# zju3dv/NeuralRecon-W

Hardware: AMD Instinct MI355X
Metric: ray-samples/sec (train step) at 1024 rays x 128 samples (higher is better)
Workload: dtype f16; 1 GPU; brandenburg_gate config (BASELINE.json configs[1]): 1024 rays/GPU x (64 coarse + 64 fine) samples, SDF 8x256 + colour 4x256 + bg NeRF 8x256, 4 outside samples, up_sample_steps 2, render+loss+backward+allreduce+clip+Adam; rays_per_gpu=1024, samples_per_ray=128, global_rays=1024, parallelism=dp1, world_size=1, submission=eager, streams=2, skipped_steps=0

## Files before the change

include/neuconw_hip.h:

```cpp
#ifndef NEUCONW_HIP_H
#define NEUCONW_HIP_H
#include <stdint.h>

#ifdef __cplusplus
extern "C" {
#endif

#define NCW_PREC_F32 0
#define NCW_PREC_BF16 1
#define NCW_PREC_F16 2
#define NCW_MAX_LAYERS 12
#define NCW_MAX_SEGS 4

#define NCW_E_BADARG (-1)
#define NCW_E_UNSUPPORTED (-2)

int ncw_abi_version(void);
const char* ncw_source_hash(void);
int ncw_device_info(char* buf, int buflen);

typedef struct NcwSeg {
    int32_t col0;
    int32_t ncols;
    int32_t dcol0;
// ... 23 lines not shown
                     void* stream);

typedef struct NcwUnpackDesc {
    const float* dw;
    const float* db;
    const float* src;
    const float* g;
    float* d_src;
    float* d_g;
    float* d_bias;
    int32_t ld, ldw;
    int32_t row0, nrows, drow0;
    float scale;
    float grad_mul;
    int32_t accumulate;
    int32_t nseg;
    NcwSeg seg[NCW_MAX_SEGS];
    const float* grad_mul_dev;
} NcwUnpackDesc;
int ncw_unpack_grads(const NcwUnpackDesc* descs, const int32_t* row_prefix, int n, int total_rows,
                     void* stream);

typedef struct NcwSdfNet {
    const void* w[NCW_MAX_LAYERS];
    const float* b[NCW_MAX_LAYERS];
    const void* wt[NCW_MAX_LAYERS];
    const void* w_feat;
    const float* b_feat;
    const void* wt_feat;
    int32_t n_layers;
    int32_t skip_layer;
    int32_t rb;
    int32_t multires;
    float scale;
    int32_t adj_mode;
    const void* w_lo[NCW_MAX_LAYERS];
    const void* wt_lo[NCW_MAX_LAYERS];
} NcwSdfNet;

int ncw_sdf_infer(const NcwSdfNet* net, int prec, const float* x, int64_t n, float* sdf, void* stream);

int ncw_sdf_infer_rays(const NcwSdfNet* net, int prec, const float* rays_o, const float* rays_d, const float* z,
                       int R, int n, float* sdf, void* stream);

typedef struct NcwPoints {
    const float* x;
    const float* rays_o;
    const float* rays_d;
    const float* z;
    const float* sample_dist;
    int32_t per_ray;
    int32_t mode;
    float gmin[3], gmax[3], gorigin[3], gradius;
    int32_t gdim;
    int32_t _gpad;
    int64_t gstart;
    const int32_t* idx;
    const int32_t* count;
} NcwPoints;

int ncw_sdf_infer_points(const NcwSdfNet* net, int prec, const NcwPoints* pts, int64_t count, float* sdf, void* stream);


typedef struct NcwSdfStash {
    void* gamma;
    void* h[NCW_MAX_LAYERS];
    void* s[NCW_MAX_LAYERS];
    void* t[NCW_MAX_LAYERS];
    void* feat;
    void* dfeat;
    void* qbar[NCW_MAX_LAYERS];
    void* zbar[NCW_MAX_LAYERS];
    void* zsdf;
    void* one;
} NcwSdfStash;

int ncw_sdf_fwd(const NcwSdfNet* net, int prec, const NcwPoints* pts, int64_t n, float* sdf, float* grad,
                const NcwSdfStash* stash, void* stream);
int ncw_sdf_bwd(const NcwSdfNet* net, int prec, const NcwPoints* pts, int64_t n, const float* d_sdf,
                const float* d_grad, const NcwSdfStash* stash, void* stream);

typedef struct NcwColorNet {
    const void* w_f; const void* wt_f; const float* b_f;
    const void* w_e[4]; const void* wt_e[4]; const float* b_e[4];
    const void* w_l[8]; const void* wt_l[8]; const float* b_l[8];
    int32_t n_head;
    int32_t n_lin;
    int32_t rbf, rbh, rbc, n_a;
    const void* w_f_lo; const void* w_e_lo[4]; const void* w_l_lo[8];
    int32_t act_split;
    int32_t _pad;
} NcwColorNet;

typedef struct NcwColorStash {
    void* aux1;
    void* aux2;
    void* f;
    void* e[4];
    void* x[8];
    void* zf;
    void* ze[4];
    void* zx[8];
    void* zo;
    const float* aux_bias;
} NcwColorStash;

int ncw_color_fwd(const NcwColorNet* net, int prec, const NcwPoints* pts, int64_t n, const float* normals,
                  const float* a, const void* feat_stash, float* rgb, const NcwColorStash* stash, void* stream);
int ncw_color_bwd(const NcwColorNet* net, int prec, const NcwPoints* pts, int64_t n, const float* rgb,
                  const float* d_rgb, float* d_grad, float* d_a, float* d_a_rows, void* dfeat_stash,
                  const NcwColorStash* stash, void* stream);

typedef struct NcwNerfNet {
    const void* w_p[8]; const void* wt_p[8]; const float* b_p[8];
    const void* w_alpha; const void* wt_alpha; const float* b_alpha;
    const void* w_feat; const void* wt_feat; const float* b_feat;
    const void* w_a[4]; const void* wt_a[4]; const float* b_a[4];
    const void* w_rgb; const void* wt_rgb; const float* b_rgb;
    int32_t D;
    int32_t skip;
    int32_t rbn, rbh, n_head, n_a;
    const void* w_p_lo[8]; const void* w_alpha_lo; const void* w_feat_lo; const void* w_a_lo[4]; const void* w_rgb_lo;
} NcwNerfNet;

typedef struct NcwNerfStash {
    void* gp;
    void* aux1;
    void* h[9];
    void* featn;
    void* e[4];
    void* zp[8];
    void* zalpha;
    void* zfeat;
    void* ze[4];
    void* zrgb;
    const float* aux_bias;
} NcwNerfStash;

int ncw_nerf_fwd(const NcwNerfNet* net, int prec, const NcwPoints* pts, const float* x4, int64_t n, const float* a,
                 float* density, float* rgb, const NcwNerfStash* stash, void* stream);
int ncw_nerf_bwd(const NcwNerfNet* net, int prec, const NcwPoints* pts, int64_t n, const float* d_density,
                 const float* d_rgb, float* d_a, float* d_a_rows, const NcwNerfStash* stash, void* stream);
int ncw_nerf_refine(const NcwNerfNet* net, int prec, const NcwPoints* pts, int64_t n, const float* aux_bias, float* density,
                    float* rgb, void* stream);
int ncw_batch_assemble(const float* all_rays, int ncols, const float* all_rgbs, const int64_t* idx, int64_t n_rows,
                       int64_t B, int with_semantics, float* rays, int64_t* ts, int64_t* label, float* rgbs,
                       const int* mask_ids, int n_ids, uint8_t* keep, void* stream);
int ncw_aux_ray_bias(const float* w, int ldw, int col0, int n_out, const float* rays_d, const float* a, int n_a, int64_t R,
                     float* out, int ldo, void* stream);
int ncw_ray_prologue(const float* rays, int ncols, int64_t R, const float* origin_host, float radius, float* rays_o,
                     float* rays_d, float* near, float* far, float* depth_gt, float* depth_weight, void* stream);
int ncw_inv_s_fwd(const float* variance, float* inv_s, float* s_val, void* stream);
int ncw_inv_s_bwd(const float* d_inv_s_rays, int64_t R, const float* inv_s, float* d_variance, void* stream);
int ncw_loss_fwd(const float* color, const float* rgbs, int64_t R, const float* gradient_error, const float* mask_error,
                 int64_t n_mask, const float* sfm, int64_t n_sfm, float coef, float igr_w, float mask_w, float depth_w,
                 float* loss, void* stream);
int ncw_loss_bwd(const float* d_loss, const float* color, const float* rgbs, int64_t R, int64_t n_mask, int64_t n_sfm,
                 float coef, float igr_w, float mask_w, float depth_w, float* d_color, float* d_gradient_error,
                 float* d_mask_error, float* d_sfm, void* stream);
int ncw_scatter_add_rows(const float* rows, const int64_t* idx, int64_t R, int n_cols, int64_t n_out, float* out,
                         void* stream);
int ncw_ray_sum_rows(const float* rows, int64_t R, int per_ray, int n_cols, float* out, int accumulate, void* stream);

typedef struct NcwWgradDesc {
    const void* x;
    const void* y;
    float* dense;
    float* dbias;
    int32_t rbx, rby, ld;
    int32_t ksplit;
    int64_t n_points;
    const int32_t* n_points_dev;
} NcwWgradDesc;
int ncw_wgrad(const NcwWgradDesc* descs, const int32_t* wg_prefix, int n_desc, int total_wgs, int ksplit,
              int prec, int64_t n_points, void* stream);
int64_t ncw_wgrad_ordered_scratch_floats(int total_wgs);
int ncw_wgrad_ordered(const NcwWgradDesc* descs, const int32_t* wg_prefix, int n_desc, int total_wgs, int ksplit,
                      int prec, int64_t n_points, float* partials, void* stream);
int ncw_wgrad_tiled(const NcwWgradDesc* descs, const int32_t* wg_prefix, int n_desc, int total_wgs, int ksplit,
                    int tile, int64_t n_points, void* stream);
int ncw_wgrad_tiled_f16(const NcwWgradDesc* descs, const int32_t* wg_prefix, int n_desc, int total_wgs, int ksplit,
                        int tile, int64_t n_points, void* stream);

int ncw_adam_step(float* param, float* grad, float* exp_avg, float* exp_avg_sq, int64_t n, float step_size,
                  float beta1, float beta2, float eps, float bias_correction2_sqrt, const float* total_norm,
                  float max_norm, void* stream);

int64_t ncw_grad_norm_scratch_floats(void);
int ncw_grad_norm(const float* grad, int64_t n, float* scratch, float* norm, void* stream);

typedef struct NcwAdamState {
    int32_t step;
    int32_t good;
    int32_t skipped;
    int32_t skip_now;
    float coef, step_size, bc2_sqrt, last_norm;
} NcwAdamState;
int ncw_adam_step_dev(float* param, float* grad, float* exp_avg, float* exp_avg_sq, int64_t n, NcwAdamState* state,
                      const float* total_norm, float lr, const float* lr_dev, float beta1, float beta2, float eps,
                      float max_norm, float* loss_scale, int growth_interval, float scale_min, float scale_max,
                      void* stream);

int ncw_stash_from_rows(int prec, const float* rows, int64_t n, int F, int rb, void* stash, void* stream);
int ncw_stash_to_rows(int prec, const void* stash, int64_t n, int F, int rb, float* rows, void* stream);

int ncw_sample_coarse(const float* near, const float* far, const float* s_near, const float* s_far, int R,
                      int n_samples, int n_outside, const float* rand_shift, const float* rand_out,
                      float* z, float* z_out, float* sample_dist, void* stream);
int ncw_upsample(const float* rays_o, const float* rays_d, const float* z, const float* sdf, int R, int n,
                 float inv_s, int n_new, float* z_new, void* stream);
int ncw_sort_merge(const float* a, int na, const float* b, int nb, const float* pa, const float* pb, int R,
                   float* out, float* pout, void* stream);
int ncw_boundary(const float* near, const float* far, const float* z, int n, int R, int nb, float* zb,
                 void* stream);

int ncw_voxel_build(const float* pts_normalised, int64_t n, int level, uint32_t* occ, uint32_t* brick, void* stream);
int ncw_ray_voxel_near_far(const float* rays_o_sfm, const float* rays_d, int R, const float* scene_origin_host,
                           float scale, int level, const uint32_t* occ, const uint32_t* brick, float* near_sfm,
                           float* far_sfm, void* stream);
int ncw_ray_voxel_trace(const float* rays_o_norm, const float* rays_d, int R, int level, const uint32_t* occ,
                        const uint32_t* brick, const int32_t* offsets, int32_t* counts, int32_t* nug_ray,
                        int32_t* nug_voxel, float* nug_depth, void* stream);

typedef struct NcwCompositeIn {
    const float* rays_o;
    const float* rays_d;
    const float* z;
    const float* z_feed;
    const float* sample_dist;
    const float* sdf;
    const float* grad;
    const float* rgb;
    const float* density;
    const float* bg_rgb;
    const float* inv_s;
    const float* background_rgb;
    const float* cos_anneal_dev;
    float cos_anneal;
    int32_t R, S, O, has_bg, trim_sphere;
} NcwCompositeIn;

typedef struct NcwCompositeOut {
    float* color;
    float* color_sphere;
    float* color_bg;
    float* weights;
    float* weights_sum;
    float* cdf;
    float* inside;
    float* depth;
    float* normals;
    float* eik;
    float* mid_z;
    float* dists;
    float* bg_alpha;
    float* weights_max;
} NcwCompositeOut;

typedef struct NcwCompositeGrad {
    const float* d_color;
    const float* d_weights_sum;
    const float* d_depth;
    const float* d_eik_num;
    float* d_sdf;
    float* d_grad;
    float* d_rgb;
    float* d_density;
    float* d_bg_rgb;
    float* d_inv_s;
    float grad_scale;
    const float* grad_scale_dev;
    const float* d_normals;
} NcwCompositeGrad;

int ncw_bg_select(const float* rays_o, const float* rays_d, const float* z, const float* sample_dist, int R, int S,
                  int O, int32_t* idx, int32_t* ray_offsets, int32_t* count, void* stream);

int ncw_composite_fwd(const NcwCompositeIn* in, const NcwCompositeOut* out, void* stream);
int ncw_composite_bwd(const NcwCompositeIn* in, const NcwCompositeGrad* g, void* stream);

int ncw_ray_tail_fwd(const float* weights_sum, const int64_t* label, const int* mask_ids, int n_ids,
                     const float* depth, const float* depth_gt, const float* depth_weight, const float* eik_num,
                     const float* eik_den, int R, float* mask_error, float* sfm_depth_loss, float* scalars,
                     void* stream);
int ncw_ray_tail_bwd(const float* weights_sum, const int64_t* label, const int* mask_ids, int n_ids,
                     const float* depth, const float* depth_gt, const float* depth_weight, int R,
                     const float* scalars, const float* d_mask_error, const float* d_sfm_depth_loss,
                     const float* d_gradient_error, float* d_weights_sum, float* d_depth, float* d_eik_num,
                     void* stream);

int ncw_ray_floor_fwd(const float* normals, const int64_t* label, const int* floor_ids, int n_ids, const float n_gt[3],
                      const float* rays_o, const float* rays_d, const float* depth, int R, int scaled,
                      float* floor_error , float* scalars , void* stream);
int ncw_ray_floor_bwd(const float* normals, const int64_t* label, const int* floor_ids, int n_ids, const float n_gt[3],
                      int R, int scaled, const float* scalars, const float* d_floor_error ,
                      float* d_normals , void* stream);

int ncw_mc_count(const float* sdf, const uint8_t* mask, int Dx, int Dy, int Dz, float level, const int32_t* ntri,
                 int32_t* counts, void* stream);
int ncw_mc_emit(const float* sdf, const uint8_t* mask, int Dx, int Dy, int Dz, float level, const int8_t* tri,
                const int32_t* ntri, const int32_t* edges, const int64_t* offsets, float* tri_pos, int64_t* tri_key,
                void* stream);

int ncw_mcs_neighbors(const int32_t* bricks, int64_t n, int G, int32_t* nbr, void* stream);
int ncw_mcs_count(const float* values, int64_t n_values, const int32_t* bricks, const int32_t* nbr, int64_t n, int up, int G,
                  float level, const int32_t* ntri, uint8_t* counts, void* stream);
int ncw_mcs_cube_ids(const int32_t* bricks, int64_t n, int up, int G, const int64_t* sub, int64_t M, int64_t* ids, void* stream);
int ncw_mcs_emit(const float* values, int64_t n_values, const int32_t* bricks, const int32_t* nbr, int64_t n, int up, int G,
                 float level, const int8_t* tri, const int32_t* ntri, const int32_t* edges, const int64_t* sub,
                 const int64_t* offsets, int64_t M, int64_t T, float* tri_pos, int64_t* tri_key, void* stream);


typedef struct NcwNnGrid {
    float lo[3];
    float h, inv_h;
    int32_t dim[3];
} NcwNnGrid;

int ncw_nn_cell_keys(const float* pts, int64_t n, const NcwNnGrid* grid, int32_t* keys, void* stream);
int ncw_nn_cell_ranges(const float* pts, const int32_t* sorted_keys, const int64_t* order, int64_t m, int32_t* cell_range,
                       float* pts_sorted, void* stream);
int ncw_nn_query(const float* pts_sorted, const int32_t* cell_range, const float* q, const int64_t* q_order, int64_t n,
                 const NcwNnGrid* grid, int max_shell, float margin, float* dist, int64_t* idx, int32_t* escaped,
                 int32_t* n_escaped, void* stream);
int ncw_nn_brute(const float* pts_sorted, int64_t m, const float* q, const int32_t* escaped, int64_t n_esc, uint64_t* scratch,
                 float* dist, int64_t* idx, void* stream);
int ncw_nn_coarse(const int32_t* cell_range, const NcwNnGrid* grid, int B, int32_t* coarse, void* stream);
int ncw_nn_query_within(const float* pts_sorted, const int32_t* cell_range, const int32_t* coarse, int B, const float* q,
                        const int64_t* q_order, int64_t n, const NcwNnGrid* grid, float margin, float max_dist, float* dist,
                        int64_t* idx, void* stream);


int ncw_knn_query(const float* pts_sorted, const int32_t* cell_range, const int32_t* coarse, int B, const float* q,
                  const int64_t* q_order, const int32_t* exclude, int64_t n, const NcwNnGrid* grid, float margin, float max_dist,
                  int k, int wg, int32_t* idx, float* dist, int32_t* count, int32_t* work, void* stream);
int ncw_knn_pca(const float* pts, const float* ref, int64_t m, const int32_t* idx, const int32_t* count, int64_t n, int k,
                int with_query, const float* toward, float* normal, double* eig, float* curvature, uint8_t* valid, void* stream);


typedef struct NcwRasterView {
    float view[12];
    float fx, fy, cx, cy;
    float znear, zfar;
    int32_t height, width;
    int32_t cull;
    int32_t small_max;
} NcwRasterView;

int ncw_raster_small(const float* verts, int64_t n_verts, const int32_t* faces, int64_t n_faces, const NcwRasterView* view,
                     uint64_t* zbuf, int32_t* large, int32_t* n_large, void* stream);
int ncw_raster_large(const float* verts, int64_t n_verts, const int32_t* faces, const NcwRasterView* view, const int32_t* large,
                     const int32_t* n_large, int64_t max_large, uint64_t* zbuf, void* stream);
int ncw_raster_resolve(const uint64_t* zbuf, int64_t n_pix, float* depth, int32_t* face, void* stream);
int ncw_raster_backproject(const float* depth, const int64_t* pix, int64_t n, int32_t width, const float* M, float* pts,
                           void* stream);
int ncw_raster_mark(const float* dist, const int64_t* idx, int64_t n, float thr, int64_t m, uint8_t* flags, void* stream);


typedef struct NcwViewCamera {
    float fx, fy, cx, cy;
    float c2w[12];
    int32_t width, height;
    float near, far;
} NcwViewCamera;

// ... 200 lines not shown
```

neuralrecon-w_amd/appfit.py:

```python
import ctypes as C
import json
import os

import numpy as np
import torch

from . import lib as L
from . import rayops
from .neuconw import points_struct
from .packing import pack_many
from .stash import StashArena, StashCache

DEFAULT_STEPS = 200
DEFAULT_LR = 0.02
DEFAULT_N_RAYS = 8192


def half_pixel_indices(width, height):
    width, height = int(width), int(height)
    idx = np.arange(width * height, dtype=np.int64).reshape(height, width)
    return idx[:, : width // 2].reshape(-1), idx[:, width // 2:].reshape(-1)


def ray_subset(width, height, n_rays, seed=0):
    left, _ = half_pixel_indices(width, height)
    if n_rays is None or int(n_rays) >= left.size:
        return left
    pick = np.random.default_rng(int(seed)).choice(left.size, int(n_rays), replace=False)
    return left[np.sort(pick)]


def held_out_rows(root_dir):
    from . import colmap

    _, rows = colmap.split_rows(root_dir)
    return [r["filename"] for r in rows if r.get("split") == "test"]


class FrozenRays:

    def release(self):
        StashCache.release(self.__dict__.pop("sdf_lease", None))

    def __del__(self):
        try:
            self.release()
        except Exception:
            pass


def _use_bg(rdr):
    return bool(rdr.render_bg and rdr.n_outside > 0)


def _bg_choice(rdr, z, n_out):
    select = refine = None
    if rdr.trim_sphere:
        refine = (z, n_out)
        if not rdr.bg_dense:
            select = refine
    return select, refine


@torch.no_grad()
def freeze_rays(rdr, rays, background_rgb=None, chunk=1024, cos_anneal_ratio=0.0, far_override=None):
    if not (torch.is_tensor(rays) and rays.is_cuda):
        raise L.NeuconwHipError("appfit.freeze_rays: rays are not on a GPU; the hot path has no CPU fallback")
    dev, prec, lib = rays.device, rdr.prec, L.get_lib()
    neuconw, nerf = rdr.neuconw, rdr.nerf
    if rdr.origin.device != dev:
        rdr.origin = rdr.origin.to(dev).float()
        rdr.sfm_to_gt = rdr.sfm_to_gt.to(dev).float()
    use_bg = _use_bg(rdr)
    if rdr.__dict__.get("sampler_prec") is None:
        pack_many([(m, m.plan(prec)) for m in [neuconw.sdf_net, neuconw.color_net] + ([nerf] if use_bg else [])])
    origin = (C.c_float * 3)(*[float(v) for v in rdr.origin.reshape(-1).tolist()])
    n_a = int(neuconw.color_net.n_a)
    bgc = None
    if background_rgb is not None:
        if background_rgb.numel() != 3:
            raise ValueError("background_rgb must hold ONE colour (3 values): got shape %s" % (tuple(background_rgb.shape),))
        bgc = background_rgb.detach().to(dev).reshape(3).float().contiguous()
    variance = neuconw.deviation_network.variance
    inv_s, s_val = torch.empty(1, device=dev), torch.empty(1, device=dev)
    L.check(lib.ncw_inv_s_fwd(L.ptr(variance.detach().reshape(1).float().contiguous()), L.ptr(inv_s), L.ptr(s_val),
                              L.stream_ptr(dev)), "ncw_inv_s_fwd")
    rays = rays.contiguous().float()
    out = []
    for r0 in range(0, rays.shape[0], max(1, int(chunk))):
        rc = rays[r0:r0 + max(1, int(chunk))].contiguous()
        R = rc.shape[0]
        rays_o, rays_d = torch.empty(R, 3, device=dev), torch.empty(R, 3, device=dev)
        near, far = torch.empty(R, 1, device=dev), torch.empty(R, 1, device=dev)
        dgt, dw = torch.empty(R, device=dev), torch.empty(R, device=dev)
        L.check(lib.ncw_ray_prologue(L.ptr(rc), rc.shape[1], R, origin, float(rdr.radius), L.ptr(rays_o), L.ptr(rays_d),
                                     L.ptr(near), L.ptr(far), L.ptr(dgt), L.ptr(dw), L.stream_ptr(dev)), "ncw_ray_prologue")
        _, z, z_out, sample_dist = rdr.sparse_sampler(rays_o, rays_d, near, far, 0, None, far_override)
        S = z.shape[1]
        g = FrozenRays()
        g.R, g.S, g.use_bg, g.background_rgb = R, S, bool(use_bg and z_out is not None), bgc
        a0 = torch.zeros(R, n_a, device=dev)
        z_feed = density = bg_rgb = None
        g.O = 0
        if g.use_bg:
            g.O = z_out.shape[1]
            g.select, g.refine = _bg_choice(rdr, z, g.O)
            z_feed, _ = rayops.sort_merge(z, z_out)
            g.pts_bg = points_struct(rays_o=rays_o, rays_d=rays_d, z=z_feed, sample_dist=sample_dist, mode=2)
            density, bg_rgb, nctx = nerf.fwd_stash(g.pts_bg, R * (S + g.O), prec, a0, select=g.select, train=False, refine=g.refine)
            StashCache.release(nctx["lease"])
            density, bg_rgb = density.view(R, S + g.O), bg_rgb.view(R, S + g.O, 3)
        g.M = S + g.O
        g.pts_in = points_struct(rays_o=rays_o, rays_d=rays_d, z=z, sample_dist=sample_dist, mode=2)
        sdf, grad, sctx = neuconw.sdf_net.fwd_stash(g.pts_in, R * S, prec, train=False)
        g.sdf_lease, g.sdf_arena = sctx["lease"], sctx["arena"]
        g.feat_ptr = sctx["arena"].ptr(sctx["ids"]["feat"])
        g.grad = grad
        comp = rayops.CompositeCtx(rays_o, rays_d, z, sample_dist, sdf.view(R, S), grad.view(R, S, 3),
                                   torch.zeros(R, S, 3, device=dev), inv_s, cos_anneal_ratio, z_feed, density, bg_rgb, bgc,
                                   rdr.trim_sphere)
        o = comp.forward()
        g.weights, g.inside, g.weights_sum, g.z_feed, g.z = o["weights"], o["inside"], o["weights_sum"], z_feed, z
        out.append(g)
    return out


def release_contexts(contexts):
    for g in contexts:
        g.release()


def dead_sample_share(contexts):
    dead = sum(int((g.weights == 0).sum()) for g in contexts)
    return dead / float(max(1, sum(g.weights.numel() for g in contexts)))


class AppearanceFit:

    def __init__(self, rdr, contexts, targets, init, lr=DEFAULT_LR, betas=(0.9, 0.999), eps=1e-7):
        if not contexts:
            raise ValueError("AppearanceFit: no frozen rays")
        if not (torch.is_tensor(targets) and targets.is_cuda and torch.is_tensor(init) and init.is_cuda):
            raise L.NeuconwHipError("AppearanceFit: targets / init are not on a GPU; the hot path has no CPU fallback")
        self.rdr, self.ctxs = rdr, list(contexts)
        dev = targets.device
        self.dev, self.prec = dev, rdr.prec
        self.n_a = n_a = int(rdr.neuconw.color_net.n_a)
        self.R_total = sum(g.R for g in self.ctxs)
        self.targets = targets.detach().reshape(-1, 3).float().contiguous()
        if self.targets.shape[0] != self.R_total:
            raise ValueError("AppearanceFit: %d targets for %d frozen rays" % (self.targets.shape[0], self.R_total))
        if init.numel() != n_a:
            raise ValueError("AppearanceFit: the code holds %d values, the networks take %d" % (init.numel(), n_a))
        self.lr, self.betas, self.eps = float(lr), (float(betas[0]), float(betas[1])), float(eps)
        self.inv_denom = 1.0 / (self.R_total + 1e-5)
        self.code = init.detach().reshape(n_a).float().clone().contiguous()
        self.exp_avg, self.exp_avg_sq = torch.zeros(n_a, device=dev), torch.zeros(n_a, device=dev)
        self.grad_acc = torch.zeros(n_a, device=dev)
        self.state = torch.zeros(8, device=dev, dtype=torch.int32)
        self.scale = None
        if self.prec == L.PREC_F16:
            s0 = float(rdr.loss_scale.init)
            self.scale = torch.tensor([s0, 1.0 / s0], device=dev, dtype=torch.float32)
        Rm = max(g.R for g in self.ctxs)
        nS, nM = max(g.R * g.S for g in self.ctxs), max(g.R * g.M for g in self.ctxs)
        any_bg = any(g.use_bg for g in self.ctxs)
        self.a_rows = self.code.reshape(1, n_a).expand(Rm, n_a).contiguous()
        self.color = torch.empty(self.R_total, 3, device=dev)
        self.ray_loss = torch.zeros(self.R_total, device=dev)
        self.d_rgb, self.rows = torch.empty(nS, 3, device=dev), torch.empty(nS, n_a, device=dev)
        self.d_grad = torch.zeros(nS, 3, device=dev)
        rbf = int(rdr.neuconw.color_net.d_feature) // 32
        self.dfeat = StashArena(dev, self.prec, nS)
        self.dfeat.new(rbf)
        self.dfeat.allocate()
        if any_bg:
            self.d_bg_rgb, self.rows_bg = torch.empty(nM, 3, device=dev), torch.empty(nM, n_a, device=dev)
            self.d_density = torch.zeros(nM, device=dev)
        lib = L.get_lib()
        self.scratch = torch.empty(max(1, int(lib.ncw_appfit_step_scratch_floats(max(nS, nM), n_a))), device=dev)

    def _step_call(self, rows, n, accumulate, final):
        dev = self.dev
        L.check(L.get_lib().ncw_appfit_step(L.ptr(rows), int(n), self.n_a, L.ptr(self.scratch), L.ptr(self.grad_acc),
                                            int(accumulate), int(final), L.ptr(self.code), L.ptr(self.exp_avg),
                                            L.ptr(self.exp_avg_sq), L.ptr(self.state), self.lr, self.betas[0], self.betas[1],
                                            self.eps, L.ptr(self.scale), 1.0, L.ptr(self.a_rows), self.a_rows.shape[0],
                                            L.stream_ptr(dev)), "ncw_appfit_step")

    def _pass(self, backward):
        rdr, prec, lib, dev, n_a = self.rdr, self.prec, L.get_lib(), self.dev, self.n_a
        color_net, nerf = rdr.neuconw.color_net, rdr.nerf
        r0, first = 0, True
        for g in self.ctxs:
            R, S, M = g.R, g.S, g.M
            a = self.a_rows[:R]
            leases = []
            try:
                rgb, cctx = color_net.fwd_stash(g.pts_in, R * S, prec, g.grad, a, g.feat_ptr, train=backward)
                leases.append(cctx["lease"])
                bg_rgb = nctx = None
                if g.use_bg:
                    _, bg_rgb, nctx = nerf.fwd_stash(g.pts_bg, R * M, prec, a, select=g.select, train=backward, refine=g.refine)
                    leases.append(nctx["lease"])
                d_bg = self.d_bg_rgb[:R * M] if g.use_bg else None
                L.check(lib.ncw_appfit_loss(L.ptr(g.weights), L.ptr(g.inside), L.ptr(g.weights_sum), L.ptr(rgb), L.ptr(bg_rgb),
                                            L.ptr(g.background_rgb), L.ptr(self.targets[r0:r0 + R]), R, S, g.O, self.inv_denom,
                                            L.ptr(self.scale), L.ptr(self.color[r0:r0 + R]), L.ptr(self.ray_loss[r0:r0 + R]),
                                            L.ptr(self.d_rgb[:R * S]), L.ptr(d_bg), L.stream_ptr(dev)), "ncw_appfit_loss")
                if backward:
                    rows = self.rows[:R * S]
                    color_net.bwd_stash(cctx, self.d_rgb[:R * S], self.d_grad[:R * S], None, self.dfeat.ptr(0), d_a_rows=rows)
                    self._step_call(rows, R * S, not first, False)
                    first = False
                    if g.use_bg:
                        rows_bg = self.rows_bg[:R * M]
                        if nctx.get("sel_count") is not None:
                            rows_bg.zero_()
                        nerf.bwd_stash(nctx, self.d_density[:R * M], d_bg, None, d_a_rows=rows_bg)
                        self._step_call(rows_bg, R * M, True, False)
            finally:
                for l in leases:
                    StashCache.release(l)
            r0 += R
        return self.ray_loss.sum() * self.inv_denom

    def loss_and_grad(self):
        with torch.no_grad():
            return self._pass(True)

    def loss(self):
        with torch.no_grad():
            return self._pass(False)

    def step(self):
        self._step_call(None, 0, True, True)

    @property
    def grad(self):
        return self.grad_acc * self.scale[1] if self.scale is not None else self.grad_acc.clone()

    def colors(self):
        return self.color

    @property
    def skipped_steps(self):
        return int(self.state[2])

    @property
    def applied_steps(self):
        return int(self.state[0])


def _planar(gt, H, W, dev):
    g = gt.to(dev).float()
    if g.dim() == 2:
        g = g.reshape(H, W, 3).permute(2, 0, 1)
    return g.reshape(3, H, W).contiguous()


# ... 115 lines not shown
```

neuralrecon-w_amd/csrc/ncw_glue.hip:

```cpp
#include "../../include/neuconw_hip.h"
#include "ncw_common.h"

namespace {

__global__ __launch_bounds__(256) void ray_prologue_kernel(const float* __restrict__ rays, int ncols, int64_t R, float ox, float oy,
                                                           float oz, float radius, float* __restrict__ rays_o,
                                                           float* __restrict__ rays_d, float* __restrict__ near,
                                                           float* __restrict__ far, float* __restrict__ depth_gt,
                                                           float* __restrict__ depth_w) {
    const int64_t r = (int64_t)blockIdx.x * 256 + threadIdx.x;
    if (r >= R) return;
    const float* s = rays + r * ncols;
    const float inv = 1.0f / radius;
    rays_o[r * 3 + 0] = (s[0] - ox) * inv;
    rays_o[r * 3 + 1] = (s[1] - oy) * inv;
    rays_o[r * 3 + 2] = (s[2] - oz) * inv;
    rays_d[r * 3 + 0] = s[3]; rays_d[r * 3 + 1] = s[4]; rays_d[r * 3 + 2] = s[5];
    near[r] = s[6] * inv;
    far[r] = s[7] * inv;
    depth_gt[r] = ncols >= 10 ? s[8] * inv : 0.f;
    depth_w[r] = ncols >= 10 ? s[9] : 0.f;
}

__global__ void inv_s_fwd_kernel(const float* __restrict__ variance, float* __restrict__ inv_s, float* __restrict__ s_val) {
    const float v = fminf(fmaxf(expf(variance[0] * 10.0f), 1e-6f), 1e6f);
    inv_s[0] = v;
    if (s_val) s_val[0] = 1.0f / v;
}

__device__ __forceinline__ float block_sum_fixed(float v, float* sm) {
    sm[threadIdx.x] = v;
    __syncthreads();
    for (int o = 128; o > 0; o >>= 1) {
        if ((int)threadIdx.x < o) sm[threadIdx.x] += sm[threadIdx.x + o];
        __syncthreads();
    }
    const float t = sm[0];
    __syncthreads();
    return t;
}

__global__ __launch_bounds__(256) void inv_s_bwd_kernel(const float* __restrict__ d, int64_t R, const float* __restrict__ inv_s,
                                                        float* __restrict__ d_var) {
    __shared__ float sm[256];
    float a = 0.f;
    for (int64_t i = threadIdx.x; i < R; i += 256) a += d[i];
    const float tot = block_sum_fixed(a, sm);
    if (threadIdx.x == 0) {
        const float v = inv_s[0];
        d_var[0] = (v > 1e-6f && v < 1e6f) ? tot * 10.0f * v : 0.f;
    }
}

__global__ __launch_bounds__(256) void loss_fwd_kernel(const float* __restrict__ color, const float* __restrict__ rgbs, int64_t R,
                                                       const float* __restrict__ ge, const float* __restrict__ me, int64_t n_mask,
                                                       const float* __restrict__ sfm, int64_t n_sfm, float coef, float igr_w,
                                                       float mask_w, float depth_w, float* __restrict__ loss) {
    __shared__ float sm[256];
    float a = 0.f, b = 0.f, c = 0.f;
    for (int64_t i = threadIdx.x; i < R * 3; i += 256) a += fabsf(color[i] - rgbs[i]);
    for (int64_t i = threadIdx.x; i < n_mask; i += 256) b += me[i];
    for (int64_t i = threadIdx.x; i < n_sfm; i += 256) c += sfm[i];
    const float sa = block_sum_fixed(a, sm), sb = block_sum_fixed(b, sm), sc = block_sum_fixed(c, sm);
    if (threadIdx.x == 0) {
        float l = coef * (sa / ((float)R + 1e-5f));
        if (ge) l += coef * (igr_w * ge[0]);
        if (n_mask > 0) l += coef * (mask_w * (sb / (float)n_mask));
        if (n_sfm > 0) l += coef * (depth_w * (sc / (float)n_sfm));
        loss[0] = l;
    }
}

__global__ __launch_bounds__(256) void loss_bwd_kernel(const float* __restrict__ d_loss, const float* __restrict__ color,
                                                       const float* __restrict__ rgbs, int64_t R, int64_t n_mask, int64_t n_sfm,
                                                       float coef, float igr_w, float mask_w, float depth_w,
                                                       float* __restrict__ d_color, float* __restrict__ d_ge,
                                                       float* __restrict__ d_me, float* __restrict__ d_sfm) {
    const float g = d_loss[0] * coef;
    const int64_t i = (int64_t)blockIdx.x * 256 + threadIdx.x;
    if (i < R * 3) {
        const float e = color[i] - rgbs[i];
        d_color[i] = (e > 0.f ? 1.f : (e < 0.f ? -1.f : 0.f)) * g / ((float)R + 1e-5f);
    }
    if (d_me && i < n_mask) d_me[i] = g * mask_w / (float)n_mask;
    if (d_sfm && i < n_sfm) d_sfm[i] = g * depth_w / (float)n_sfm;
    if (d_ge && i == 0) d_ge[0] = g * igr_w;
}

__global__ __launch_bounds__(128) void aux_ray_bias_kernel(const float* __restrict__ w, int ldw, int col0, int n_out,
                                                          const float* __restrict__ rays_d, const float* __restrict__ a, int n_a,
                                                          float* __restrict__ out, int ldo) {
    __shared__ float x[96];
    const int64_t ray = blockIdx.x;
    const int t = threadIdx.x;
    const int K = 27 + n_a;
    if (t < K) {
        float v;
        if (t < 27) {
            const float d[3] = {rays_d[ray * 3 + 0], rays_d[ray * 3 + 1], rays_d[ray * 3 + 2]};
            if (t < 3) v = d[t];
            else {
                const int j = t - 3, k = j / 6, rem = j - 6 * k;
                const float arg = d[rem % 3] * (float)(1 << k);
                v = rem >= 3 ? cosf(arg) : sinf(arg);
            }
        } else {
            v = a[ray * n_a + (t - 27)];
        }
        x[t] = v;
    }
    __syncthreads();
    for (int j = t; j < n_out; j += 128) {
        const float* wr = w + (size_t)j * ldw + col0;
        float acc = 0.f;
        for (int k = 0; k < K; ++k) acc = fmaf(wr[k], x[k], acc);
        out[ray * ldo + j] = acc;
    }
}

}

extern "C" int ncw_aux_ray_bias(const float* w, int ldw, int col0, int n_out, const float* rays_d, const float* a, int n_a,
                                int64_t R, float* out, int ldo, void* stream) {
    if (R <= 0) return 0;
    if (!w || !rays_d || !a || !out || n_a < 0 || n_a > 69 || n_out <= 0 || ldo < n_out || col0 < 0 || col0 + 27 + n_a > ldw)
        return NCW_E_BADARG;
    hipLaunchKernelGGL(aux_ray_bias_kernel, dim3((unsigned)R), dim3(128), 0, (hipStream_t)stream, w, ldw, col0, n_out, rays_d, a,
                       n_a, out, ldo);
    NCW_CHECK_LAUNCH();
    return 0;
}

extern "C" int ncw_ray_prologue(const float* rays, int ncols, int64_t R, const float* origin_host, float radius, float* rays_o,
                                float* rays_d, float* near, float* far, float* depth_gt, float* depth_weight, void* stream) {
    if (R <= 0) return 0;
    if (!rays || ncols < 8 || !origin_host || !rays_o || !rays_d || !near || !far || !depth_gt || !depth_weight || radius == 0.f)
        return NCW_E_BADARG;
    hipLaunchKernelGGL(ray_prologue_kernel, dim3((unsigned)((R + 255) / 256)), dim3(256), 0, (hipStream_t)stream, rays, ncols, R,
                       origin_host[0], origin_host[1], origin_host[2], radius, rays_o, rays_d, near, far, depth_gt, depth_weight);
    NCW_CHECK_LAUNCH();
    return 0;
}

extern "C" int ncw_inv_s_fwd(const float* variance, float* inv_s, float* s_val, void* stream) {
    if (!variance || !inv_s) return NCW_E_BADARG;
    hipLaunchKernelGGL(inv_s_fwd_kernel, dim3(1), dim3(1), 0, (hipStream_t)stream, variance, inv_s, s_val);
    NCW_CHECK_LAUNCH();
    return 0;
}

extern "C" int ncw_inv_s_bwd(const float* d_inv_s_rays, int64_t R, const float* inv_s, float* d_variance, void* stream) {
    if (!d_inv_s_rays || !inv_s || !d_variance || R < 0) return NCW_E_BADARG;
    hipLaunchKernelGGL(inv_s_bwd_kernel, dim3(1), dim3(256), 0, (hipStream_t)stream, d_inv_s_rays, R, inv_s, d_variance);
    NCW_CHECK_LAUNCH();
    return 0;
}

extern "C" int ncw_loss_fwd(const float* color, const float* rgbs, int64_t R, const float* gradient_error, const float* mask_error,
                            int64_t n_mask, const float* sfm, int64_t n_sfm, float coef, float igr_w, float mask_w, float depth_w,
                            float* loss, void* stream) {
    if (!color || !rgbs || !loss || R <= 0 || n_mask < 0 || n_sfm < 0 || (n_mask > 0 && !mask_error) || (n_sfm > 0 && !sfm))
        return NCW_E_BADARG;
    hipLaunchKernelGGL(loss_fwd_kernel, dim3(1), dim3(256), 0, (hipStream_t)stream, color, rgbs, R, gradient_error, mask_error,
                       n_mask, sfm, n_sfm, coef, igr_w, mask_w, depth_w, loss);
    NCW_CHECK_LAUNCH();
    return 0;
}

extern "C" int ncw_loss_bwd(const float* d_loss, const float* color, const float* rgbs, int64_t R, int64_t n_mask, int64_t n_sfm,
                            float coef, float igr_w, float mask_w, float depth_w, float* d_color, float* d_gradient_error,
                            float* d_mask_error, float* d_sfm, void* stream) {
    if (!d_loss || !color || !rgbs || !d_color || R <= 0 || n_mask < 0 || n_sfm < 0) return NCW_E_BADARG;
    int64_t n = R * 3;
    if (n_mask > n) n = n_mask;
    if (n_sfm > n) n = n_sfm;
    hipLaunchKernelGGL(loss_bwd_kernel, dim3((unsigned)((n + 255) / 256)), dim3(256), 0, (hipStream_t)stream, d_loss, color, rgbs, R,
                       n_mask, n_sfm, coef, igr_w, mask_w, depth_w, d_color, d_gradient_error, d_mask_error, d_sfm);
    NCW_CHECK_LAUNCH();
    return 0;
}
```

neuralrecon-w_amd/csrc/ncw_optim.hip:

```cpp
#include "../../include/neuconw_hip.h"
#include "ncw_common.h"

__global__ __launch_bounds__(256) void adam_clip_kernel(float* __restrict__ p, float* __restrict__ g, float* __restrict__ m,
                                                        float* __restrict__ v, int64_t n, float step_size, float beta1,
                                                        float beta2, float eps, float bc2_sqrt,
                                                        const float* __restrict__ total_norm, float max_norm) {
    float coef = 1.f;
    if (total_norm != nullptr) {
        const float tn = total_norm[0];
        if (!(tn < __builtin_inff())) return;
        coef = fminf(max_norm / (tn + 1e-6f), 1.f);
    }
    const int64_t i4 = ((int64_t)blockIdx.x * blockDim.x + threadIdx.x) * 4;
    if (i4 >= n) return;
    const float w1 = 1.f - beta1, w2 = 1.f - beta2;
    if (i4 + 4 <= n) {
        f32x4 pp = *reinterpret_cast<f32x4*>(p + i4), gg = *reinterpret_cast<f32x4*>(g + i4);
        f32x4 mm = *reinterpret_cast<f32x4*>(m + i4), vv = *reinterpret_cast<f32x4*>(v + i4);
#pragma unroll
        for (int c = 0; c < 4; ++c) {
            const float gc = gg[c] * coef;
            gg[c] = gc;
            mm[c] = mm[c] + w1 * (gc - mm[c]);
            vv[c] = vv[c] * beta2 + w2 * gc * gc;
            const float denom = sqrtf(vv[c]) / bc2_sqrt + eps;
            pp[c] = pp[c] - step_size * (mm[c] / denom);
        }
        *reinterpret_cast<f32x4*>(p + i4) = pp;
        *reinterpret_cast<f32x4*>(g + i4) = gg;
        *reinterpret_cast<f32x4*>(m + i4) = mm;
        *reinterpret_cast<f32x4*>(v + i4) = vv;
    } else {
        for (int64_t i = i4; i < n; ++i) {
            const float gc = g[i] * coef;
            g[i] = gc;
            const float mi = m[i] + w1 * (gc - m[i]);
            const float vi = v[i] * beta2 + w2 * gc * gc;
            m[i] = mi;
            v[i] = vi;
            p[i] = p[i] - step_size * (mi / (sqrtf(vi) / bc2_sqrt + eps));
        }
    }
}

__global__ void adam_prep_kernel(NcwAdamState* __restrict__ st, const float* __restrict__ total_norm, float lr,
                                 const float* __restrict__ lr_dev, float beta1, float beta2, float max_norm,
                                 float* __restrict__ loss_scale, int growth_interval, float scale_min, float scale_max) {
    if (threadIdx.x != 0 || blockIdx.x != 0) return;
    const float tn = total_norm ? total_norm[0] : 0.f;
    const bool finite = tn < __builtin_inff() && tn == tn;
    if (!finite) {
        st->skip_now = 1;
        st->skipped += 1;
        st->good = 0;
        if (loss_scale) {
            const float s = fmaxf(loss_scale[0] * 0.5f, scale_min);
            loss_scale[0] = s;
            loss_scale[1] = 1.f / s;
        }
        return;
    }
    st->skip_now = 0;
    const int t = st->step + 1;
    st->step = t;
    st->good += 1;
    if (loss_scale && growth_interval > 0 && st->good >= growth_interval) {
        const float s = fminf(loss_scale[0] * 2.f, scale_max);
        loss_scale[0] = s;
        loss_scale[1] = 1.f / s;
        st->good = 0;
    }
    const double l = lr_dev ? (double)lr_dev[0] : (double)lr;
    const double bc1 = 1.0 - pow((double)beta1, (double)t);
    const double bc2 = 1.0 - pow((double)beta2, (double)t);
    st->step_size = (float)(l / bc1);
    st->bc2_sqrt = (float)sqrt(bc2);
    st->coef = (total_norm && max_norm > 0.f) ? fminf(max_norm / (tn + 1e-6f), 1.f) : 1.f;
    st->last_norm = tn;
}

__global__ __launch_bounds__(256) void adam_dev_kernel(float* __restrict__ p, float* __restrict__ g, float* __restrict__ m,
                                                       float* __restrict__ v, int64_t n, float beta1, float beta2, float eps,
                                                       const NcwAdamState* __restrict__ st) {
    if (st->skip_now) return;
    const float coef = st->coef, step_size = st->step_size, bc2_sqrt = st->bc2_sqrt;
    const int64_t i4 = ((int64_t)blockIdx.x * blockDim.x + threadIdx.x) * 4;
    if (i4 >= n) return;
    const float w1 = 1.f - beta1, w2 = 1.f - beta2;
    if (i4 + 4 <= n) {
        f32x4 pp = *reinterpret_cast<f32x4*>(p + i4), gg = *reinterpret_cast<f32x4*>(g + i4);
        f32x4 mm = *reinterpret_cast<f32x4*>(m + i4), vv = *reinterpret_cast<f32x4*>(v + i4);
#pragma unroll
        for (int c = 0; c < 4; ++c) {
            const float gc = gg[c] * coef;
            gg[c] = gc;
            mm[c] = mm[c] + w1 * (gc - mm[c]);
            vv[c] = vv[c] * beta2 + w2 * gc * gc;
            const float denom = sqrtf(vv[c]) / bc2_sqrt + eps;
            pp[c] = pp[c] - step_size * (mm[c] / denom);
        }
        *reinterpret_cast<f32x4*>(p + i4) = pp;
        *reinterpret_cast<f32x4*>(g + i4) = gg;
        *reinterpret_cast<f32x4*>(m + i4) = mm;
        *reinterpret_cast<f32x4*>(v + i4) = vv;
    } else {
        for (int64_t i = i4; i < n; ++i) {
            const float gc = g[i] * coef;
            g[i] = gc;
            const float mi = m[i] + w1 * (gc - m[i]);
            const float vi = v[i] * beta2 + w2 * gc * gc;
            m[i] = mi;
            v[i] = vi;
            p[i] = p[i] - step_size * (mi / (sqrtf(vi) / bc2_sqrt + eps));
        }
    }
}

constexpr int NORM_BLOCKS = 256;

__global__ __launch_bounds__(256) void grad_norm_kernel(const float* __restrict__ g, int64_t n, float* __restrict__ scratch,
                                                        float* __restrict__ norm) {
    __shared__ float wsum[4];
    __shared__ int last;
    const int64_t quads = (n + 3) / 4;
    const int64_t per = (quads + NORM_BLOCKS - 1) / NORM_BLOCKS;
    const int64_t q0 = (int64_t)blockIdx.x * per, q1 = q0 + per < quads ? q0 + per : quads;
    float acc = 0.f;
    for (int64_t q = q0 + threadIdx.x; q < q1; q += 256) {
        const int64_t i = q * 4;
        if (i + 4 <= n) {
            const f32x4 v = *reinterpret_cast<const f32x4*>(g + i);
            acc += v[0] * v[0] + v[1] * v[1] + v[2] * v[2] + v[3] * v[3];
        } else {
            for (int64_t j = i; j < n; ++j) acc += g[j] * g[j];
        }
    }
#pragma unroll
    for (int o = 32; o >= 1; o >>= 1) acc += __shfl_xor(acc, o, 64);
    if ((threadIdx.x & 63) == 0) wsum[threadIdx.x >> 6] = acc;
    __syncthreads();
    if (threadIdx.x == 0) {
        scratch[blockIdx.x] = (wsum[0] + wsum[1]) + (wsum[2] + wsum[3]);
        __threadfence();
        unsigned* ticket = reinterpret_cast<unsigned*>(scratch + NORM_BLOCKS);
        last = (atomicAdd(ticket, 1u) == NORM_BLOCKS - 1) ? 1 : 0;
    }
    __syncthreads();
    if (!last) return;
    __threadfence();
    float t = __builtin_nontemporal_load(scratch + threadIdx.x);
#pragma unroll
    for (int o = 32; o >= 1; o >>= 1) t += __shfl_xor(t, o, 64);
    if ((threadIdx.x & 63) == 0) wsum[threadIdx.x >> 6] = t;
    __syncthreads();
    if (threadIdx.x == 0) {
        norm[0] = sqrtf((wsum[0] + wsum[1]) + (wsum[2] + wsum[3]));
    }
}

extern "C" int64_t ncw_grad_norm_scratch_floats(void) { return NORM_BLOCKS + 4; }

extern "C" int ncw_grad_norm(const float* grad, int64_t n, float* scratch, float* norm, void* stream) {
    if (!grad || !scratch || !norm || n < 0 || ((uintptr_t)grad & 15) != 0) return NCW_E_BADARG;
    if (hipMemsetAsync(scratch + NORM_BLOCKS, 0, sizeof(unsigned), (hipStream_t)stream) != hipSuccess) return NCW_E_BADARG;
    hipLaunchKernelGGL(grad_norm_kernel, dim3(NORM_BLOCKS), dim3(256), 0, (hipStream_t)stream, grad, n, scratch, norm);
    NCW_CHECK_LAUNCH();
    return 0;
}

extern "C" int ncw_adam_step_dev(float* param, float* grad, float* exp_avg, float* exp_avg_sq, int64_t n, NcwAdamState* state,
                                 const float* total_norm, float lr, const float* lr_dev, float beta1, float beta2, float eps,
                                 float max_norm, float* loss_scale, int growth_interval, float scale_min, float scale_max,
                                 void* stream) {
    if (n <= 0) return 0;
    if (!param || !grad || !exp_avg || !exp_avg_sq || !state) return NCW_E_BADARG;
    if ((((uintptr_t)param | (uintptr_t)grad | (uintptr_t)exp_avg | (uintptr_t)exp_avg_sq) & 15) != 0) return NCW_E_BADARG;
    hipLaunchKernelGGL(adam_prep_kernel, dim3(1), dim3(64), 0, (hipStream_t)stream, state, total_norm, lr, lr_dev, beta1, beta2,
                       max_norm, loss_scale, growth_interval, scale_min, scale_max);
    NCW_CHECK_LAUNCH();
    const int64_t quads = (n + 3) / 4;
    hipLaunchKernelGGL(adam_dev_kernel, dim3((unsigned)((quads + 255) / 256)), dim3(256), 0, (hipStream_t)stream, param, grad,
                       exp_avg, exp_avg_sq, n, beta1, beta2, eps, state);
    NCW_CHECK_LAUNCH();
    return 0;
}

extern "C" int ncw_adam_step(float* param, float* grad, float* exp_avg, float* exp_avg_sq, int64_t n, float step_size,
                             float beta1, float beta2, float eps, float bias_correction2_sqrt, const float* total_norm,
                             float max_norm, void* stream) {
    if (n <= 0) return 0;
    if (!param || !grad || !exp_avg || !exp_avg_sq || !(bias_correction2_sqrt > 0.f)) return NCW_E_BADARG;
    if ((((uintptr_t)param | (uintptr_t)grad | (uintptr_t)exp_avg | (uintptr_t)exp_avg_sq) & 15) != 0) return NCW_E_BADARG;
    const int64_t quads = (n + 3) / 4;
    hipLaunchKernelGGL(adam_clip_kernel, dim3((unsigned)((quads + 255) / 256)), dim3(256), 0, (hipStream_t)stream, param,
                       grad, exp_avg, exp_avg_sq, n, step_size, beta1, beta2, eps, bias_correction2_sqrt, total_norm,
                       max_norm);
    NCW_CHECK_LAUNCH();
    return 0;
}
```

neuralrecon-w_amd/csrc/ncw_pack.hip:

```cpp
#include "../../include/neuconw_hip.h"
#include "ncw_common.h"

__device__ __forceinline__ size_t packed_index(int o, int k, int rb_out, int prec) {
    const int ro = o >> 5, i = o & 31;
    const int rb = k >> 5, kk = k & 31;
    const int h = (kk >> 2) & 1;
    const int r = (kk & 3) + 4 * (kk >> 3);
    const int lane = i + 32 * h;
    if (prec == NCW_PREC_F32) return ((size_t)(rb * 16 + r) * rb_out + ro) * 64 + lane;
    const int t = r >> 3, e = r & 7;
    return (((size_t)(2 * rb + t) * rb_out + ro) * 64 + lane) * 8 + e;
}

__device__ __forceinline__ int find_desc(const int32_t* __restrict__ prefix, int n, int row) {
    int lo = 0, hi = n;
    while (hi - lo > 1) {
        int mid = (lo + hi) >> 1;
        if (prefix[mid] <= row) lo = mid; else hi = mid;
    }
    return lo;
}

__device__ __forceinline__ float wave_sum(float v) {
#pragma unroll
// ... 28 lines not shown
            const float v = srow[sg.col0 + c] * coef;
            const int k_log = sg.dcol0 + c;
            const int o = transpose ? k_log : o_log;
            const int k = transpose ? o_log : k_log;
            const size_t idx = packed_index(o, k, rb_out, prec);
            if (prec == NCW_PREC_F32) reinterpret_cast<float*>(dst_w)[idx] = v;
            else if (prec == NCW_PREC_F16) {
                const _Float16 hi = (_Float16)v;
                reinterpret_cast<_Float16*>(dst_w)[idx] = D.residual ? (_Float16)(v - (float)hi) : hi;
            } else {
                const __bf16 hi = (__bf16)v;
                reinterpret_cast<__bf16*>(dst_w)[idx] = D.residual ? (__bf16)(v - (float)hi) : hi;
            }
        }
    }
    if (D.dst_b != nullptr && D.bias != nullptr && lane == 0) {
        const int f = o_log, rb = f >> 5, kk = f & 31;
        const int h = (kk >> 2) & 1, r = (kk & 3) + 4 * (kk >> 3);
        D.dst_b[(rb * 2 + h) * 16 + r] = D.bias[row];
    }
}

__global__ __launch_bounds__(256) void unpack_kernel(const NcwUnpackDesc* __restrict__ descs,
                                                     const int32_t* __restrict__ prefix, int n, int total_rows) {
    const int grow = blockIdx.x * 4 + (threadIdx.x >> 6);
    if (grow >= total_rows) return;
    const int lane = threadIdx.x & 63;
    const int d = find_desc(prefix, n, grow);
    const NcwUnpackDesc& D = descs[d];
    const int i = grow - prefix[d];
    const int row = D.row0 + i;
    const float* drow = D.dw + (size_t)(D.drow0 + i) * D.ldw;
    const float* vrow = D.src + (size_t)row * D.ld;
    float* out = D.d_src + (size_t)row * D.ld;
    const float gm = (D.grad_mul != 0.f ? D.grad_mul : 1.0f) * (D.grad_mul_dev ? D.grad_mul_dev[0] : 1.0f);
    const float scale = D.scale * gm;
    const int accumulate = D.accumulate;
    if (D.g == nullptr) {
        for (int s = 0; s < D.nseg; ++s) {
            const NcwSeg sg = D.seg[s];
            for (int c = lane; c < sg.ncols; c += 64) {
                const float gval = drow[sg.dcol0 + c] * scale;
                float* o = out + sg.col0 + c;
                *o = accumulate ? *o + gval : gval;
            }
        }
    } else {
        float ss = 0.f, dot = 0.f;
        for (int s = 0; s < D.nseg; ++s) {
            const NcwSeg sg = D.seg[s];
            for (int c = lane; c < sg.ncols; c += 64) {
                const float v = vrow[sg.col0 + c];
                ss += v * v;
                dot += drow[sg.dcol0 + c] * scale * v;
            }
        }
        ss = wave_sum(ss);
        dot = wave_sum(dot);
        const float inv = 1.f / sqrtf(ss);
        const float gbar = dot * inv;
        const float gg = D.g[row];
        for (int s = 0; s < D.nseg; ++s) {
            const NcwSeg sg = D.seg[s];
            for (int c = lane; c < sg.ncols; c += 64) {
                const float v = vrow[sg.col0 + c];
                const float gval = gg * inv * (drow[sg.dcol0 + c] * scale - gbar * v * inv);
                float* o = out + sg.col0 + c;
                *o = accumulate ? *o + gval : gval;
            }
        }
        if (lane == 0 && D.d_g != nullptr) D.d_g[row] = accumulate ? D.d_g[row] + gbar : gbar;
    }
    if (lane == 0 && D.d_bias != nullptr && D.db != nullptr) {
        const float b = D.db[D.drow0 + i] * gm;
        D.d_bias[row] = accumulate ? D.d_bias[row] + b : b;
    }
}

extern "C" int ncw_pack_weights(const NcwPackDesc* descs, const int32_t* row_prefix, int n, int total_rows,
                                void* stream) {
    if (n <= 0 || total_rows <= 0) return 0;
    hipLaunchKernelGGL(pack_kernel, dim3((total_rows + 3) / 4), dim3(256), 0, (hipStream_t)stream, descs, row_prefix, n,
                       total_rows);
    NCW_CHECK_LAUNCH();
    return 0;
}

extern "C" int ncw_unpack_grads(const NcwUnpackDesc* descs, const int32_t* row_prefix, int n, int total_rows,
                                void* stream) {
    if (n <= 0 || total_rows <= 0) return 0;
    hipLaunchKernelGGL(unpack_kernel, dim3((total_rows + 3) / 4), dim3(256), 0, (hipStream_t)stream, descs, row_prefix, n,
                       total_rows);
    NCW_CHECK_LAUNCH();
    return 0;
}

template <class SE, bool TO_ROWS>
__global__ void stash_rows_kernel(SE* stash, float* rows, int64_t n, int F, int rb) {
    const int lane = threadIdx.x & 63;
    const int64_t tile = (int64_t)blockIdx.x * (blockDim.x >> 6) + (threadIdx.x >> 6);
    if (tile * 32 >= n) return;
    const int64_t p = tile * 32 + (lane & 31);
    const int h = lane >> 5;
    for (int b = 0; b < rb; ++b)
        for (int g = 0; g < 4; ++g) {
            SE* s = stash + ((((size_t)tile * rb + b) * 4 + g) * 64 + lane) * 4;
            for (int c = 0; c < 4; ++c) {
                const int f = b * 32 + 8 * g + 4 * h + c;
                if (TO_ROWS) {
                    if (p < n && f < F) rows[p * F + f] = (float)s[c];
                } else {
                    s[c] = (p < n && f < F) ? (SE)rows[p * F + f] : (SE)0.f;
                }
            }
        }
}

extern "C" int ncw_stash_from_rows(int prec, const float* rows, int64_t n, int F, int rb, void* stash, void* stream) {
    if (n <= 0) return 0;
    if (F > 32 * rb) return NCW_E_BADARG;
    const int64_t tiles = (n + 31) / 32;
    dim3 grid((unsigned)((tiles + 3) / 4));
    if (prec == NCW_PREC_F32)
        hipLaunchKernelGGL((stash_rows_kernel<float, false>), grid, dim3(256), 0, (hipStream_t)stream, (float*)stash,
                           const_cast<float*>(rows), n, F, rb);
    else if (prec == NCW_PREC_F16)
        hipLaunchKernelGGL((stash_rows_kernel<_Float16, false>), grid, dim3(256), 0, (hipStream_t)stream, (_Float16*)stash,
                           const_cast<float*>(rows), n, F, rb);
    else
        hipLaunchKernelGGL((stash_rows_kernel<__bf16, false>), grid, dim3(256), 0, (hipStream_t)stream, (__bf16*)stash,
                           const_cast<float*>(rows), n, F, rb);
    NCW_CHECK_LAUNCH();
    return 0;
}

extern "C" int ncw_stash_to_rows(int prec, const void* stash, int64_t n, int F, int rb, float* rows, void* stream) {
    if (n <= 0) return 0;
    if (F > 32 * rb) return NCW_E_BADARG;
    const int64_t tiles = (n + 31) / 32;
    dim3 grid((unsigned)((tiles + 3) / 4));
    if (prec == NCW_PREC_F32)
        hipLaunchKernelGGL((stash_rows_kernel<float, true>), grid, dim3(256), 0, (hipStream_t)stream,
                           (float*)const_cast<void*>(stash), rows, n, F, rb);
    else if (prec == NCW_PREC_F16)
        hipLaunchKernelGGL((stash_rows_kernel<_Float16, true>), grid, dim3(256), 0, (hipStream_t)stream,
                           (_Float16*)const_cast<void*>(stash), rows, n, F, rb);
    else
        hipLaunchKernelGGL((stash_rows_kernel<__bf16, true>), grid, dim3(256), 0, (hipStream_t)stream,
                           (__bf16*)const_cast<void*>(stash), rows, n, F, rb);
    NCW_CHECK_LAUNCH();
    return 0;
}

extern "C" int ncw_abi_version(void) { return 38; }

extern "C" int ncw_device_info(char* buf, int buflen) {
    int cnt = 0;
    if (hipGetDeviceCount(&cnt) != hipSuccess || cnt == 0) {
        if (buf && buflen > 0) buf[0] = 0;
        return 0;
    }
    hipDeviceProp_t p;
    if (hipGetDeviceProperties(&p, 0) != hipSuccess) return 0;
    if (buf && buflen > 0) {
        int i = 0;
        for (; i < buflen - 1 && p.gcnArchName[i]; ++i) buf[i] = p.gcnArchName[i];
        buf[i] = 0;
    }
    return p.multiProcessorCount;
}
```

neuralrecon-w_amd/csrc/ncw_rays.hip:

```cpp
#include "../../include/neuconw_hip.h"
#include "ncw_common.h"

constexpr int RAY_CAP_SMALL = 512, RAY_CAP_LARGE = 1088;

NCW_DEV float sigmoid_acc(float x) { return 1.f / (1.f + expf(-x)); }

NCW_DEV float torch_linspace(float start, float end, int steps, int i) {
    if (steps == 1) return start;
    const float step = (end - start) / (float)(steps - 1);
    return (i < steps / 2) ? start + step * (float)i : end - step * (float)(steps - 1 - i);
}

template <bool MUL, int CH>
NCW_DEV float wave_excl_scan(const float* a, float* out, int m, int lane) {
    const int per = (m + 63) >> 6;
    const int b = lane * per;
    float loc[CH];
    float tot = MUL ? 1.f : 0.f;
#pragma unroll
    for (int k = 0; k < CH; ++k) {
        if (k < per) {
            const int i = b + k;
            loc[k] = (i < m) ? a[i] : (MUL ? 1.f : 0.f);
            tot = MUL ? tot * loc[k] : tot + loc[k];
// ... 53 lines not shown

struct NeusAlpha { float ep, en, pc, nc, raw; };

NCW_DEV NeusAlpha neus_alpha(float sdf, float cs, float dist, float inv_s) {
    NeusAlpha a;
    a.ep = sdf - cs * dist * 0.5f;
    a.en = sdf + cs * dist * 0.5f;
    a.pc = sigmoid_acc(a.ep * inv_s);
    a.nc = sigmoid_acc(a.en * inv_s);
    a.raw = (a.pc - a.nc + 1e-5f) / (a.pc + 1e-5f);
    return a;
}

NCW_DEV float clamp01(float x) { return fminf(fmaxf(x, 0.f), 1.f); }

NCW_DEV float bg_alpha_of(float den, float dist) {
    const float sp = den > 20.f ? den : log1pf(expf(den));
    return 1.0f - expf(-sp * dist);
}
NCW_DEV float bg_alpha_bwd(float dalpha, float alpha, float den, float dist) {
    const float sg = den > 20.f ? 1.f : sigmoid_acc(den);
    return dalpha * (1.0f - alpha) * dist * sg;
}

__global__ void sample_coarse_kernel(const float* __restrict__ near, const float* __restrict__ far,
                                     const float* __restrict__ s_near, const float* __restrict__ s_far, int R,
                                     int n_samples, int n_out, const float* __restrict__ rand_shift,
                                     const float* __restrict__ rand_out, float* __restrict__ z,
                                     float* __restrict__ z_out, float* __restrict__ sample_dist) {
    const int r = blockIdx.x * blockDim.y + threadIdx.y;
    if (r >= R) return;
    const float sn = s_near[r], sf = s_far[r], fr = far[r];
    for (int i = threadIdx.x; i < n_samples; i += blockDim.x) {
        float v = sn + (sf - sn) * torch_linspace(0.f, 1.f, n_samples, i);
        if (rand_shift) v = v + (sf - sn) * (rand_shift[r] - 0.5f) * 2.0f / (float)n_samples;
        z[(size_t)r * n_samples + i] = v;
    }
    if (threadIdx.x == 0) sample_dist[r] = (sf - sn) / (float)n_samples;
    const float oe = 1.0f - 1.0f / ((float)n_out + 1.0f);
    for (int j = threadIdx.x; j < n_out; j += blockDim.x) {
        const int q = n_out - 1 - j;
        float zo = torch_linspace(1e-3f, oe, n_out, q);
        if (rand_out) {
            const float cur = zo;
            const float nxt = (q + 1 < n_out) ? torch_linspace(1e-3f, oe, n_out, q + 1) : cur;
            const float prv = (q > 0) ? torch_linspace(1e-3f, oe, n_out, q - 1) : cur;
            const float upper = (q + 1 < n_out) ? 0.5f * (nxt + cur) : cur;
            const float lower = (q > 0) ? 0.5f * (cur + prv) : cur;
            zo = lower + (upper - lower) * rand_out[(size_t)r * n_out + q];
        }
        z_out[(size_t)r * n_out + j] = fr / zo + 1.0f / (float)n_samples;
    }
}

template <int MAXN>
__global__ __launch_bounds__(256) void upsample_kernel(const float* __restrict__ rays_o, const float* __restrict__ rays_d,
                                                       const float* __restrict__ z, const float* __restrict__ sdf,
                                                       int R, int n, float inv_s, int n_new,
                                                       float* __restrict__ z_new) {
    constexpr int CH = MAXN / 64;
    __shared__ float sm[4][4][MAXN];
    const int wv = threadIdx.x >> 6, lane = threadIdx.x & 63;
    const int r = blockIdx.x * 4 + wv;
    if (r >= R) return;
    float* zs = sm[wv][0];
    float* sd = sm[wv][1];
    float* t0 = sm[wv][2];
    float* t1 = sm[wv][3];
    const Ray y = load_ray(rays_o, rays_d, r);
    const int m = n - 1;
    for (int i = lane; i < n; i += 64) {
        const float zz = z[(size_t)r * n + i];
        zs[i] = zz;
        sd[i] = sdf[(size_t)r * n + i];
        t0[i] = ray_radius(y, zz);
    }
    __builtin_amdgcn_wave_barrier();
    for (int i = lane; i < m; i += 64) t1[i] = (sd[i + 1] - sd[i]) / (zs[i + 1] - zs[i] + 1e-5f);
    __builtin_amdgcn_wave_barrier();
    float alpha_l[CH];
#pragma unroll
    for (int k = 0; k < CH; ++k) {
        const int i = lane + 64 * k;
        alpha_l[k] = 0.f;
        if (i < m) {
            const float pc0 = (i > 0) ? t1[i - 1] : 0.f;
            float cv = fminf(pc0, t1[i]);
            cv = fminf(fmaxf(cv, -1e3f), 0.f);
            const bool inside = (t0[i] < 1.0f) || (t0[i + 1] < 1.0f);
            cv = inside ? cv : 0.f;
            alpha_l[k] = neus_alpha((sd[i] + sd[i + 1]) * 0.5f, cv, zs[i + 1] - zs[i], inv_s).raw;
        }
    }
    __builtin_amdgcn_wave_barrier();
#pragma unroll
    for (int k = 0; k < CH; ++k) {
        const int i = lane + 64 * k;
        if (i < m) t0[i] = 1.0f - alpha_l[k] + 1e-7f;
    }
    __builtin_amdgcn_wave_barrier();
    wave_excl_scan<true, CH>(t0, t0, m, lane);
    float wsum = 0.f;
#pragma unroll
    for (int k = 0; k < CH; ++k) {
        const int i = lane + 64 * k;
        if (i < m) {
            const float w = alpha_l[k] * t0[i] + 1e-5f;
            t1[i] = w;
            wsum += w;
        }
    }
    wsum = wave_sum(wsum);
    __builtin_amdgcn_wave_barrier();
    for (int i = lane; i < m; i += 64) t1[i] = t1[i] / wsum;
    __builtin_amdgcn_wave_barrier();
    if (lane == 0) t1[m] = 0.f;
    __builtin_amdgcn_wave_barrier();
    wave_excl_scan<false, CH>(t1, t0, m + 1, lane);
    for (int j = lane; j < n_new; j += 64) {
        const float u = torch_linspace(0.5f / (float)n_new, 1.0f - 0.5f / (float)n_new, n_new, j);
        int lo = 0, hi = n;
        while (lo < hi) {
            const int mid = (lo + hi) >> 1;
            if (t0[mid] <= u) lo = mid + 1; else hi = mid;
        }
        const int below = max(lo - 1, 0), above = min(lo, n - 1);
        const float cb = t0[below], ca = t0[above];
        float denom = ca - cb;
        denom = (denom < 1e-5f) ? 1.0f : denom;
        const float t = (u - cb) / denom;
        z_new[(size_t)r * n_new + j] = zs[below] + t * (zs[above] - zs[below]);
    }
}

template <int MAXN>
__global__ __launch_bounds__(256) void sort_merge_kernel(const float* __restrict__ a, int na, const float* __restrict__ b,
                                                         int nb, const float* __restrict__ pa,
                                                         const float* __restrict__ pb, int R, float* __restrict__ out,
                                                         float* __restrict__ pout) {
    __shared__ float sm[4][MAXN];
    const int wv = threadIdx.x >> 6, lane = threadIdx.x & 63;
    const int r = blockIdx.x * 4 + wv;
    if (r >= R) return;
    const int n = na + nb;
    float* c = sm[wv];
    for (int i = lane; i < n; i += 64) c[i] = (i < na) ? a[(size_t)r * na + i] : b[(size_t)r * nb + (i - na)];
    __builtin_amdgcn_wave_barrier();
    for (int i = lane; i < n; i += 64) {
        const float v = c[i];
        int rank = 0;
        for (int j = 0; j < n; ++j) {
            const float w = c[j];
            rank += (w < v || (w == v && j < i)) ? 1 : 0;
        }
        out[(size_t)r * n + rank] = v;
        if (pout) pout[(size_t)r * n + rank] = (i < na) ? pa[(size_t)r * na + i] : pb[(size_t)r * nb + (i - na)];
    }
}

__global__ void boundary_kernel(const float* __restrict__ near, const float* __restrict__ far,
                                const float* __restrict__ z, int n, int R, int nb, float* __restrict__ zb) {
    const int r = blockIdx.x * blockDim.y + threadIdx.y;
    if (r >= R) return;
    const int n_near = nb / 2, n_far = nb - n_near;
    const float nr = near[r], fr = far[r], z0 = z[(size_t)r * n], z1 = z[(size_t)r * n + n - 1];
    for (int j = threadIdx.x; j < nb; j += blockDim.x) {
        float v;
        if (j < n_near) v = nr + (z0 - nr) * torch_linspace(0.f, 1.f, n_near + 1, j);
        else v = z1 + (fr - z1) * torch_linspace(0.f, 1.f, n_far + 1, j - n_near + 1);
        zb[(size_t)r * nb + j] = v;
    }
}

NCW_DEV float iter_cos_of(float tc, float c) {
    return -(fmaxf(-tc * 0.5f + 0.5f, 0.f) * (1.0f - c) + fmaxf(-tc, 0.f) * c);
}

template <int MAXN>
__global__ __launch_bounds__(256) void composite_fwd_kernel(NcwCompositeIn A, NcwCompositeOut Q) {
    constexpr int CH = MAXN / 64;
    __shared__ float sm[4][4][MAXN];
    const int wv = threadIdx.x >> 6, lane = threadIdx.x & 63;
    const int r = blockIdx.x * 4 + wv;
    if (r >= A.R) return;
    const int S = A.S, M = A.has_bg ? A.S + A.O : A.S;
    float* al0 = sm[wv][0];
    float* alm = sm[wv][1];
    float* tA = sm[wv][2];
    float* tB = sm[wv][3];
    const Ray y = load_ray(A.rays_o, A.rays_d, r);
    const float inv_s = A.inv_s[0], sdist = A.sample_dist[r];
    const float* zr = A.z + (size_t)r * S;
    float eik_num = 0.f, eik_den = 0.f;
    for (int i = lane; i < S; i += 64) {
        const Section sec = section_of(zr, i, S, sdist);
        const float pn = ray_radius(y, sec.mid);
        const size_t q = (size_t)r * S + i;
        const float gx = A.grad[q * 3], gy = A.grad[q * 3 + 1], gz = A.grad[q * 3 + 2];
        const float tc = y.dx * gx + y.dy * gy + y.dz * gz;
        const float ic = iter_cos_of(tc, A.cos_anneal_dev ? A.cos_anneal_dev[0] : A.cos_anneal);
        const NeusAlpha na = neus_alpha(A.sdf[q], ic, sec.dist, inv_s);
        const float relax = pn < 1.2f ? 1.f : 0.f;
        al0[i] = clamp01(na.raw);
        Q.cdf[q] = na.pc;
        Q.inside[q] = inside_sphere(pn) ? 1.f : 0.f;
        Q.mid_z[q] = sec.mid;
        Q.dists[q] = sec.dist;
        const float gn = sqrtf(gx * gx + gy * gy + gz * gz);
        eik_num += relax * (gn - 1.0f) * (gn - 1.0f);
        eik_den += relax;
    }
    if (A.has_bg) {
        const float* zf = A.z_feed + (size_t)r * M;
        for (int j = lane; j < M; j += 64) {
            const float ba = bg_alpha_of(A.density[(size_t)r * M + j], section_of(zf, j, M, sdist).dist);
            tB[j] = ba;
            Q.bg_alpha[(size_t)r * M + j] = ba;
        }
    }
    __builtin_amdgcn_wave_barrier();
    for (int i = lane; i < S; i += 64) tA[i] = 1.0f - al0[i] + 1e-7f;
    __builtin_amdgcn_wave_barrier();
    wave_excl_scan<true, CH>(tA, tA, S, lane);
    float depth = 0.f;
    for (int i = lane; i < S; i += 64) depth += al0[i] * tA[i] * Q.mid_z[(size_t)r * S + i];
    depth = wave_sum(depth);
    for (int j = lane; j < M; j += 64) {
        float a;
        if (j < S) {
            const float ins = Q.inside[(size_t)r * S + j];
            a = ins > 0.f ? al0[j] : (A.has_bg ? tB[j] : 0.f);
        } else a = tB[j];
        alm[j] = a;
    }
    __builtin_amdgcn_wave_barrier();
    for (int j = lane; j < M; j += 64) tA[j] = 1.0f - alm[j] + 1e-7f;
    __builtin_amdgcn_wave_barrier();
    wave_excl_scan<true, CH>(tA, tA, M, lane);
    float cr = 0.f, cg = 0.f, cb = 0.f, wsum = 0.f, nx = 0.f, ny = 0.f, nz = 0.f, wmax = -3.4e38f;
    for (int j = lane; j < M; j += 64) {
        const float w = alm[j] * tA[j];
        Q.weights[(size_t)r * M + j] = w;
        wmax = fmaxf(wmax, w);
        float rr, gg, bb;
        bool ins = false;
        if (j < S) ins = Q.inside[(size_t)r * S + j] > 0.f;
        if (ins) {
            const size_t q = ((size_t)r * S + j) * 3;
            rr = A.rgb[q]; gg = A.rgb[q + 1]; bb = A.rgb[q + 2];
        } else if (A.has_bg) {
            const size_t q = ((size_t)r * M + j) * 3;
            rr = A.bg_rgb[q]; gg = A.bg_rgb[q + 1]; bb = A.bg_rgb[q + 2];
        } else rr = gg = bb = 0.f;
        cr += rr * w; cg += gg * w; cb += bb * w;
        if (j < S) {
            if (ins) wsum += w;
            const size_t q = ((size_t)r * S + j) * 3;
            nx += A.grad[q] * w; ny += A.grad[q + 1] * w; nz += A.grad[q + 2] * w;
        }
    }
    cr = wave_sum(cr); cg = wave_sum(cg); cb = wave_sum(cb); wsum = wave_sum(wsum);
#pragma unroll
    for (int o = 32; o > 0; o >>= 1) wmax = fmaxf(wmax, __shfl_xor(wmax, o, 64));
    nx = wave_sum(nx); ny = wave_sum(ny); nz = wave_sum(nz);
    if (A.background_rgb) {
        cr += A.background_rgb[0] * (1.0f - wsum);
        cg += A.background_rgb[1] * (1.0f - wsum);
        cb += A.background_rgb[2] * (1.0f - wsum);
    }
    __builtin_amdgcn_wave_barrier();
    for (int i = lane; i < S; i += 64) tA[i] = 1.0f - al0[i] * Q.inside[(size_t)r * S + i] + 1e-7f;
    __builtin_amdgcn_wave_barrier();
    wave_excl_scan<true, CH>(tA, tA, S, lane);
    float sr = 0.f, sg = 0.f, sb = 0.f;
    for (int i = lane; i < S; i += 64) {
        const float ins = Q.inside[(size_t)r * S + i];
        const float w = al0[i] * ins * tA[i];
        const size_t q = ((size_t)r * S + i) * 3;
        sr += A.rgb[q] * ins * w; sg += A.rgb[q + 1] * ins * w; sb += A.rgb[q + 2] * ins * w;
    }
    sr = wave_sum(sr); sg = wave_sum(sg); sb = wave_sum(sb);
    float br = 0.f, bgc = 0.f, bb2 = 0.f;
    if (A.has_bg) {
        __builtin_amdgcn_wave_barrier();
        for (int j = lane; j < M; j += 64) {
            float a = tB[j];
            if (A.trim_sphere && j < S && Q.inside[(size_t)r * S + j] > 0.f) a = 0.f;
            alm[j] = a;
            tA[j] = 1.0f - a + 1e-7f;
        }
        __builtin_amdgcn_wave_barrier();
        wave_excl_scan<true, CH>(tA, tA, M, lane);
        for (int j = lane; j < M; j += 64) {
            const float w = alm[j] * tA[j];
            const size_t q = ((size_t)r * M + j) * 3;
            br += A.bg_rgb[q] * w; bgc += A.bg_rgb[q + 1] * w; bb2 += A.bg_rgb[q + 2] * w;
        }
        br = wave_sum(br); bgc = wave_sum(bgc); bb2 = wave_sum(bb2);
    }
    eik_num = wave_sum(eik_num);
    eik_den = wave_sum(eik_den);
    if (lane == 0) {
        Q.color[r * 3] = cr; Q.color[r * 3 + 1] = cg; Q.color[r * 3 + 2] = cb;
        Q.color_sphere[r * 3] = sr; Q.color_sphere[r * 3 + 1] = sg; Q.color_sphere[r * 3 + 2] = sb;
        Q.color_bg[r * 3] = br; Q.color_bg[r * 3 + 1] = bgc; Q.color_bg[r * 3 + 2] = bb2;
        Q.weights_sum[r] = wsum;
// ... 63 lines not shown
        dnx = G.d_normals[r * 3] * gs; dny = G.d_normals[r * 3 + 1] * gs; dnz = G.d_normals[r * 3 + 2] * gs;
    }
    for (int i = lane; i < S; i += 64) {
        const size_t q = (size_t)r * S + i;
        const float tc = y.dx * A.grad[q * 3] + y.dy * A.grad[q * 3 + 1] + y.dz * A.grad[q * 3 + 2];
        al0[i] = clamp01(neus_alpha(A.sdf[q], iter_cos_of(tc, c), section_of(zr, i, S, sdist).dist, inv_s).raw);
        dal0[i] = 0.f;
    }
    __builtin_amdgcn_wave_barrier();
    for (int i = lane; i < S; i += 64) T[i] = 1.0f - al0[i] + 1e-7f;
    __builtin_amdgcn_wave_barrier();
    wave_excl_scan<true, CH>(T, T, S, lane);
    for (int i = lane; i < S; i += 64) {
        const float wb = ddep * section_of(zr, i, S, sdist).mid;
        wk[i] = al0[i] * T[i] * wb;
    }
    __builtin_amdgcn_wave_barrier();
    wave_suffix_excl_sum<CH>(wk, wk, S, lane);
    for (int i = lane; i < S; i += 64) {
        const float mid = section_of(zr, i, S, sdist).mid;
        dal0[i] += T[i] * ddep * mid - wk[i] / (1.0f - al0[i] + 1e-7f);
    }
    __builtin_amdgcn_wave_barrier();
    __shared__ float smb[4][2][MAXN];
    float* ba = smb[wv][0];
    float* wbar = smb[wv][1];
    if (A.has_bg) {
        const float* zf = A.z_feed + (size_t)r * M;
        for (int j = lane; j < M; j += 64) ba[j] = bg_alpha_of(A.density[(size_t)r * M + j], section_of(zf, j, M, sdist).dist);
    }
    __builtin_amdgcn_wave_barrier();
    for (int j = lane; j < M; j += 64) {
        const bool ins = j < S && section_inside(y, zr, j, S, sdist);
        const float a = ins ? al0[j] : (A.has_bg ? ba[j] : 0.f);
        alm[j] = a;
        T[j] = 1.0f - a + 1e-7f;
        float rr, gg, bb;
        if (ins) {
            const size_t q = ((size_t)r * S + j) * 3;
            rr = A.rgb[q]; gg = A.rgb[q + 1]; bb = A.rgb[q + 2];
        } else if (A.has_bg) {
            const size_t q = ((size_t)r * M + j) * 3;
            rr = A.bg_rgb[q]; gg = A.bg_rgb[q + 1]; bb = A.bg_rgb[q + 2];
        } else rr = gg = bb = 0.f;
        float wb = dcr * rr + dcg * gg + dcb * bb + (ins ? dws : 0.f);
        if constexpr (NRM) {
            if (j < S) {
                const size_t q = ((size_t)r * S + j) * 3;
                wb += dnx * A.grad[q] + dny * A.grad[q + 1] + dnz * A.grad[q + 2];
            }
        }
        wbar[j] = wb;
    }
    __builtin_amdgcn_wave_barrier();
    wave_excl_scan<true, CH>(T, T, M, lane);
    for (int j = lane; j < M; j += 64) wk[j] = alm[j] * T[j] * wbar[j];
    __builtin_amdgcn_wave_barrier();
    float* suf = wk;
    wave_suffix_excl_sum<CH>(wk, suf, M, lane);
    for (int j = lane; j < M; j += 64) {
        const float w = alm[j] * T[j];
        const float dalpha = T[j] * wbar[j] - suf[j] / (1.0f - alm[j] + 1e-7f);
        const bool ins = j < S && section_inside(y, zr, j, S, sdist);
        if (j < S) {
            const size_t q = ((size_t)r * S + j) * 3;
            G.d_rgb[q] = ins ? dcr * w : 0.f;
            G.d_rgb[q + 1] = ins ? dcg * w : 0.f;
            G.d_rgb[q + 2] = ins ? dcb * w : 0.f;
            if (ins) dal0[j] += dalpha;
        }
        if (A.has_bg) {
            const size_t q = ((size_t)r * M + j) * 3;
            G.d_bg_rgb[q] = ins ? 0.f : dcr * w;
            G.d_bg_rgb[q + 1] = ins ? 0.f : dcg * w;
            G.d_bg_rgb[q + 2] = ins ? 0.f : dcb * w;
            const float* zf = A.z_feed + (size_t)r * M;
            G.d_density[(size_t)r * M + j] =
                bg_alpha_bwd(ins ? 0.f : dalpha, ba[j], A.density[(size_t)r * M + j], section_of(zf, j, M, sdist).dist);
        }
    }
    __builtin_amdgcn_wave_barrier();
    float ds_acc = 0.f;
    for (int i = lane; i < S; i += 64) {
        const Section sec = section_of(zr, i, S, sdist);
        const float dist = sec.dist;
        const float relax = ray_radius(y, sec.mid) < 1.2f ? 1.f : 0.f;
        const size_t q = (size_t)r * S + i;
        const float gx = A.grad[q * 3], gy = A.grad[q * 3 + 1], gz = A.grad[q * 3 + 2];
        const float tc = y.dx * gx + y.dy * gy + y.dz * gz;
        const NeusAlpha na = neus_alpha(A.sdf[q], iter_cos_of(tc, c), dist, inv_s);
        const float ep = na.ep, en = na.en, pc = na.pc, nc = na.nc;
        const float draw = (na.raw >= 0.f && na.raw <= 1.f) ? dal0[i] : 0.f;
        const float dpc = draw * (nc / ((pc + 1e-5f) * (pc + 1e-5f)));
        const float dnc = -draw / (pc + 1e-5f);
        const float dep_ = dpc * pc * (1.0f - pc), den_ = dnc * nc * (1.0f - nc);
        ds_acc += dep_ * ep + den_ * en;
        const float dep = dep_ * inv_s, dne = den_ * inv_s;
        const float dic = (dne - dep) * dist * 0.5f;
        const float dtc = dic * (0.5f * (1.0f - c) * (tc < 1.0f ? 1.f : 0.f) + c * (tc < 0.f ? 1.f : 0.f));
        const float gn = sqrtf(gx * gx + gy * gy + gz * gz);
        const float ek = (gn > 0.f) ? deik * relax * 2.0f * (gn - 1.0f) / gn : 0.f;
        G.d_sdf[q] = dep + dne;
        if constexpr (NRM) {
            const float w = alm[i] * T[i];
            G.d_grad[q * 3] = dtc * y.dx + ek * gx + w * dnx;
            G.d_grad[q * 3 + 1] = dtc * y.dy + ek * gy + w * dny;
            G.d_grad[q * 3 + 2] = dtc * y.dz + ek * gz + w * dnz;
        } else {
            G.d_grad[q * 3] = dtc * y.dx + ek * gx;
            G.d_grad[q * 3 + 1] = dtc * y.dy + ek * gy;
            G.d_grad[q * 3 + 2] = dtc * y.dz + ek * gz;
        }
    }
    ds_acc = wave_sum(ds_acc);
    if (lane == 0) G.d_inv_s[r] = ds_acc;
}

static int ray_capacity(int slots) { return slots <= RAY_CAP_SMALL ? RAY_CAP_SMALL : slots <= RAY_CAP_LARGE ? RAY_CAP_LARGE : 0; }

extern "C" int ncw_sample_coarse(const float* near, const float* far, const float* s_near, const float* s_far, int R,
                                 int n_samples, int n_outside, const float* rand_shift, const float* rand_out,
                                 float* z, float* z_out, float* sample_dist, void* stream) {
    if (R <= 0) return 0;
    if (n_samples < 1 || n_samples > RAY_CAP_LARGE) return NCW_E_BADARG;
    dim3 blk(64, 4);
    hipLaunchKernelGGL(sample_coarse_kernel, dim3((R + 3) / 4), blk, 0, (hipStream_t)stream, near, far, s_near, s_far, R,
                       n_samples, n_outside, rand_shift, rand_out, z, z_out, sample_dist);
    NCW_CHECK_LAUNCH();
    return 0;
}

extern "C" int ncw_upsample(const float* rays_o, const float* rays_d, const float* z, const float* sdf, int R, int n,
                            float inv_s, int n_new, float* z_new, void* stream) {
    if (R <= 0 || n_new <= 0) return 0;
    const int cap = ray_capacity(n + 1);
    if (n < 2 || !cap) return NCW_E_BADARG;
    hipLaunchKernelGGL(cap == RAY_CAP_SMALL ? upsample_kernel<RAY_CAP_SMALL> : upsample_kernel<RAY_CAP_LARGE>, dim3((R + 3) / 4),
                       dim3(256), 0, (hipStream_t)stream, rays_o, rays_d, z, sdf, R, n, inv_s, n_new, z_new);
    NCW_CHECK_LAUNCH();
    return 0;
}

extern "C" int ncw_sort_merge(const float* a, int na, const float* b, int nb, const float* pa, const float* pb, int R,
                              float* out, float* pout, void* stream) {
    if (R <= 0 || na + nb <= 0) return 0;
    const int cap = ray_capacity(na + nb);
    if (!cap) return NCW_E_BADARG;
    hipLaunchKernelGGL(cap == RAY_CAP_SMALL ? sort_merge_kernel<RAY_CAP_SMALL> : sort_merge_kernel<RAY_CAP_LARGE>, dim3((R + 3) / 4),
                       dim3(256), 0, (hipStream_t)stream, a, na, b, nb, pa, pb, R, out, pout);
    NCW_CHECK_LAUNCH();
    return 0;
}

extern "C" int ncw_boundary(const float* near, const float* far, const float* z, int n, int R, int nb, float* zb,
                            void* stream) {
    if (R <= 0 || nb <= 0) return 0;
    dim3 blk(64, 4);
    hipLaunchKernelGGL(boundary_kernel, dim3((R + 3) / 4), blk, 0, (hipStream_t)stream, near, far, z, n, R, nb, zb);
    NCW_CHECK_LAUNCH();
    return 0;
}

extern "C" int ncw_composite_fwd(const NcwCompositeIn* in, const NcwCompositeOut* out, void* stream) {
    if (!in || !out) return NCW_E_BADARG;
    if (in->R <= 0) return 0;
    const int M = in->has_bg ? in->S + in->O : in->S;
    const int cap = ray_capacity(M);
    if (in->S < 1 || !cap) return NCW_E_BADARG;
    hipLaunchKernelGGL(cap == RAY_CAP_SMALL ? composite_fwd_kernel<RAY_CAP_SMALL> : composite_fwd_kernel<RAY_CAP_LARGE>, dim3((in->R + 3) / 4), dim3(256), 0, (hipStream_t)stream, *in, *out);
    NCW_CHECK_LAUNCH();
    return 0;
}

extern "C" int ncw_composite_bwd(const NcwCompositeIn* in, const NcwCompositeGrad* g, void* stream) {
    if (!in || !g) return NCW_E_BADARG;
    if (in->R <= 0) return 0;
    const int M = in->has_bg ? in->S + in->O : in->S;
    const int cap = ray_capacity(M);
    if (in->S < 1 || !cap) return NCW_E_BADARG;
    NcwCompositeGrad G = *g;
    if (G.grad_scale == 0.f) G.grad_scale = 1.0f;
    auto kernel = cap == RAY_CAP_SMALL ? composite_bwd_kernel<RAY_CAP_SMALL, false> : composite_bwd_kernel<RAY_CAP_LARGE, false>;
    if (G.d_normals) kernel = cap == RAY_CAP_SMALL ? composite_bwd_kernel<RAY_CAP_SMALL, true> : composite_bwd_kernel<RAY_CAP_LARGE, true>;
    hipLaunchKernelGGL(kernel, dim3((in->R + 3) / 4), dim3(256), 0, (hipStream_t)stream, *in, G);
    NCW_CHECK_LAUNCH();
    return 0;
}

__global__ __launch_bounds__(256) void ray_sum_rows_kernel(const float* __restrict__ rows, int64_t R, int per_ray, int n_cols,
                                                           float* __restrict__ out, int accumulate) {
    const int64_t e = (int64_t)blockIdx.x * 256 + threadIdx.x;
    if (e >= R * n_cols) return;
    const int64_t r = e / n_cols;
    const int j = (int)(e - r * n_cols);
    const float* src = rows + (size_t)r * per_ray * n_cols + j;
    float s = 0.f;
    for (int i = 0; i < per_ray; ++i) s += src[(size_t)i * n_cols];
    out[e] = accumulate ? out[e] + s : s;
}

__global__ __launch_bounds__(256) void scatter_add_rows_kernel(const float* __restrict__ rows, const int64_t* __restrict__ idx,
                                                               int64_t R, int n_cols, int64_t n_out, float* __restrict__ out) {
    const int64_t e = (int64_t)blockIdx.x * 256 + threadIdx.x;
    if (e >= R * n_cols) return;
    const int64_t r = e / n_cols;
    const int j = (int)(e - r * n_cols);
    const int64_t t = idx[r];
    if (t >= 0 && t < n_out) atomicAdd(out + t * n_cols + j, rows[e]);
}

extern "C" int ncw_scatter_add_rows(const float* rows, const int64_t* idx, int64_t R, int n_cols, int64_t n_out, float* out,
                                    void* stream) {
    if (R <= 0 || n_cols <= 0) return 0;
    if (!rows || !idx || !out || n_out <= 0) return NCW_E_BADARG;
    hipLaunchKernelGGL(scatter_add_rows_kernel, dim3((unsigned)((R * n_cols + 255) / 256)), dim3(256), 0, (hipStream_t)stream,
                       rows, idx, R, n_cols, n_out, out);
    NCW_CHECK_LAUNCH();
    return 0;
}

extern "C" int ncw_ray_sum_rows(const float* rows, int64_t R, int per_ray, int n_cols, float* out, int accumulate,
                                void* stream) {
    if (R <= 0 || n_cols <= 0) return 0;
    if (!rows || !out || per_ray < 1) return NCW_E_BADARG;
    hipLaunchKernelGGL(ray_sum_rows_kernel, dim3((unsigned)((R * n_cols + 255) / 256)), dim3(256), 0, (hipStream_t)stream,
                       rows, R, per_ray, n_cols, out, accumulate);
    NCW_CHECK_LAUNCH();
    return 0;
}

__global__ __launch_bounds__(256) void batch_assemble_kernel(const float* __restrict__ all_rays, int ncols,
                                                             const float* __restrict__ all_rgbs,
                                                             const int64_t* __restrict__ idx, int64_t n_rows, int64_t B,
                                                             int with_semantics, float* __restrict__ rays,
                                                             int64_t* __restrict__ ts, int64_t* __restrict__ label,
                                                             float* __restrict__ rgbs, int4 ids, int n_ids,
                                                             uint8_t* __restrict__ keep) {
    const int64_t b = (int64_t)blockIdx.x * 256 + threadIdx.x;
    if (b >= B) return;
    int64_t r = idx ? idx[b] : b;
    r = r < 0 ? 0 : (r >= n_rows ? n_rows - 1 : r);
    const float* src = all_rays + r * ncols;
    float* dst = rays + b * 11;
#pragma unroll
    for (int c = 0; c < 8; ++c) dst[c] = src[c];
    const int tail = with_semantics ? 10 : 9;
#pragma unroll
    for (int c = 0; c < 3; ++c) dst[8 + c] = src[tail + c];
    ts[b] = (int64_t)src[8];
    const int64_t lab = with_semantics ? (int64_t)src[9] : 0;
    if (label) label[b] = lab;
    if (rgbs) {
        rgbs[b * 3] = all_rgbs[r * 3]; rgbs[b * 3 + 1] = all_rgbs[r * 3 + 1]; rgbs[b * 3 + 2] = all_rgbs[r * 3 + 2];
    }
    if (keep) {
        bool k = true;
        if (with_semantics) {
            if (n_ids > 0 && lab == ids.x) k = false;
            if (n_ids > 1 && lab == ids.y) k = false;
            if (n_ids > 2 && lab == ids.z) k = false;
            if (n_ids > 3 && lab == ids.w) k = false;
        }
        keep[b] = k ? 1 : 0;
    }
}

extern "C" int ncw_batch_assemble(const float* all_rays, int ncols, const float* all_rgbs, const int64_t* idx, int64_t n_rows,
                                  int64_t B, int with_semantics, float* rays, int64_t* ts, int64_t* label, float* rgbs,
                                  const int* mask_ids, int n_ids, uint8_t* keep, void* stream) {
    if (B <= 0) return 0;
    if (!all_rays || !rays || !ts || n_rows <= 0 || n_ids < 0 || n_ids > 4) return NCW_E_BADARG;
    if (ncols != (with_semantics ? 13 : 12) || (rgbs && !all_rgbs)) return NCW_E_BADARG;
    int4 ids = make_int4(n_ids > 0 ? mask_ids[0] : -1, n_ids > 1 ? mask_ids[1] : -1, n_ids > 2 ? mask_ids[2] : -1,
                         n_ids > 3 ? mask_ids[3] : -1);
    hipLaunchKernelGGL(batch_assemble_kernel, dim3((unsigned)((B + 255) / 256)), dim3(256), 0, (hipStream_t)stream, all_rays,
                       ncols, all_rgbs, idx, n_rows, B, with_semantics, rays, ts, label, rgbs, ids, n_ids, keep);
    NCW_CHECK_LAUNCH();
    return 0;
}

__device__ __forceinline__ float block_sum256(float v, float* sm) {
#pragma unroll
    for (int o = 32; o > 0; o >>= 1) v += __shfl_xor(v, o, 64);
    __syncthreads();
    if ((threadIdx.x & 63) == 0) sm[threadIdx.x >> 6] = v;
    __syncthreads();
    return sm[0] + sm[1] + sm[2] + sm[3];
}

__device__ __forceinline__ float tail_mask(const int64_t* label, int r, int n_ids, const int* ids) {
    if (label == nullptr) return 1.f;
    const int64_t l = label[r];
    for (int i = 0; i < n_ids; ++i)
        if (l == ids[i]) return 0.f;
    return 1.f;
}

struct TailIds { int v[4]; };

__global__ __launch_bounds__(256) void ray_tail_fwd_kernel(const float* __restrict__ wsum, const int64_t* __restrict__ label,
                                                           const float* __restrict__ depth, const float* __restrict__ depth_gt,
                                                           const float* __restrict__ depth_w, const float* __restrict__ eik_num,
                                                           const float* __restrict__ eik_den, int R, int n_ids, TailIds ids,
                                                           float* __restrict__ mask_error, float* __restrict__ sfm,
                                                           float* __restrict__ scal) {
    __shared__ float sm[4];
// ... 272 lines not shown
```

neuralrecon-w_amd/lib.py:

```python
import ctypes as C
import os

HERE = os.path.dirname(os.path.abspath(__file__))
LIB_PATH = os.environ.get("NEUCONW_HIP_LIB") or os.path.join(HERE, "libneuconw_hip.so")

PREC_F32 = 0
PREC_BF16 = 1
PREC_F16 = 2
MAX_LAYERS = 12
MAX_SEGS = 4
ABI_VERSION = 38


class NcwSeg(C.Structure):
    _fields_ = [("col0", C.c_int32), ("ncols", C.c_int32), ("dcol0", C.c_int32), ("_pad", C.c_int32)]


class NcwPackDesc(C.Structure):
    _fields_ = [
        ("src", C.c_void_p), ("g", C.c_void_p), ("bias", C.c_void_p), ("dst_w", C.c_void_p), ("dst_b", C.c_void_p),
        ("ld", C.c_int32), ("row0", C.c_int32), ("nrows", C.c_int32), ("drow0", C.c_int32),
        ("rb_out", C.c_int32), ("rb_in", C.c_int32), ("transpose", C.c_int32), ("prec", C.c_int32),
        ("scale", C.c_float), ("nseg", C.c_int32), ("seg", NcwSeg * MAX_SEGS), ("residual", C.c_int32), ("_pad", C.c_int32),
    ]


class NcwUnpackDesc(C.Structure):
    _fields_ = [
        ("dw", C.c_void_p), ("db", C.c_void_p), ("src", C.c_void_p), ("g", C.c_void_p),
        ("d_src", C.c_void_p), ("d_g", C.c_void_p), ("d_bias", C.c_void_p),
        ("ld", C.c_int32), ("ldw", C.c_int32), ("row0", C.c_int32), ("nrows", C.c_int32), ("drow0", C.c_int32),
        ("scale", C.c_float), ("grad_mul", C.c_float), ("accumulate", C.c_int32), ("nseg", C.c_int32),
        ("seg", NcwSeg * MAX_SEGS), ("grad_mul_dev", C.c_void_p),
    ]


class NcwAdamState(C.Structure):
    _fields_ = [("step", C.c_int32), ("good", C.c_int32), ("skipped", C.c_int32), ("skip_now", C.c_int32),
                ("coef", C.c_float), ("step_size", C.c_float), ("bc2_sqrt", C.c_float), ("last_norm", C.c_float)]


class NcwSdfNet(C.Structure):
    _fields_ = [
        ("w", C.c_void_p * MAX_LAYERS), ("b", C.c_void_p * MAX_LAYERS), ("wt", C.c_void_p * MAX_LAYERS),
        ("w_feat", C.c_void_p), ("b_feat", C.c_void_p), ("wt_feat", C.c_void_p),
        ("n_layers", C.c_int32), ("skip_layer", C.c_int32), ("rb", C.c_int32), ("multires", C.c_int32),
        ("scale", C.c_float), ("adj_mode", C.c_int32), ("w_lo", C.c_void_p * MAX_LAYERS),
        ("wt_lo", C.c_void_p * MAX_LAYERS),
    ]


class NcwPoints(C.Structure):
    _fields_ = [("x", C.c_void_p), ("rays_o", C.c_void_p), ("rays_d", C.c_void_p), ("z", C.c_void_p),
                ("sample_dist", C.c_void_p), ("per_ray", C.c_int32), ("mode", C.c_int32),
                ("gmin", C.c_float * 3), ("gmax", C.c_float * 3), ("gorigin", C.c_float * 3), ("gradius", C.c_float),
                ("gdim", C.c_int32), ("_gpad", C.c_int32), ("gstart", C.c_int64),
                ("idx", C.c_void_p), ("count", C.c_void_p)]


class NcwNnGrid(C.Structure):
    _fields_ = [("lo", C.c_float * 3), ("h", C.c_float), ("inv_h", C.c_float), ("dim", C.c_int32 * 3)]


class NcwPtmGrid(C.Structure):
    _fields_ = [("lo", C.c_double * 3), ("h", C.c_double), ("inv_h", C.c_double), ("dim", C.c_int32 * 3)]


class NcwRasterView(C.Structure):
    _fields_ = [("view", C.c_float * 12), ("fx", C.c_float), ("fy", C.c_float), ("cx", C.c_float), ("cy", C.c_float),
                ("znear", C.c_float), ("zfar", C.c_float), ("height", C.c_int32), ("width", C.c_int32), ("cull", C.c_int32),
                ("small_max", C.c_int32)]


class NcwViewCamera(C.Structure):
    _fields_ = [("fx", C.c_float), ("fy", C.c_float), ("cx", C.c_float), ("cy", C.c_float), ("c2w", C.c_float * 12),
                ("width", C.c_int32), ("height", C.c_int32), ("near", C.c_float), ("far", C.c_float)]


class NcwCacheOctree(C.Structure):
    _fields_ = [("origin", C.c_float * 3), ("scale", C.c_float), ("level", C.c_int32), ("_pad", C.c_int32),
                ("occ", C.c_void_p), ("brick", C.c_void_p)]


class NcwSourceRec(C.Structure):
    _fields_ = [("pix", C.c_uint32), ("r", C.c_uint8), ("g", C.c_uint8), ("b", C.c_uint8), ("label", C.c_uint8)]


class NcwSourceImage(C.Structure):
    _fields_ = [("cam", NcwViewCamera), ("ts", C.c_int32), ("_pad", C.c_int32)]


class NcwVoxelView(C.Structure):
    _fields_ = [("fx", C.c_float), ("fy", C.c_float), ("cx", C.c_float), ("cy", C.c_float), ("pose", C.c_float * 9),
                ("o_norm", C.c_float * 3), ("width", C.c_int32), ("height", C.c_int32)]


class NcwPixelQuery(C.Structure):
    _fields_ = [("w2c", C.c_float * 12), ("fx", C.c_float), ("fy", C.c_float), ("cx", C.c_float), ("cy", C.c_float),
                ("qx", C.c_float), ("qy", C.c_float)]


class NcwFuseGrid(C.Structure):
    _fields_ = [("lo", C.c_double * 3), ("h", C.c_double), ("dims", C.c_int64 * 3), ("scale", C.c_double),
                ("off", C.c_double * 3), ("cos_min", C.c_double), ("facing", C.c_int32), ("_pad", C.c_int32)]


class NcwFuseTable(C.Structure):
    _fields_ = [("keys", C.c_void_p), ("acc", C.c_void_p), ("stamp", C.c_void_p), ("views", C.c_void_p),
                ("counters", C.c_void_p), ("capacity", C.c_int64)]


FUSE_ACC = 10
FUSE_COUNTERS = 4
FUSE_EMPTY = -1
FUSE_MAX_DIM = 1 << 20
FUSE_MAX_CAPACITY = 1 << 36
FUSE_MAX_SERIAL = 0x7ffffffe
PIXNN_WG_POINTS = 2048
PIXNN_QUERY_TILE = 256
ALIGN_LANES = 256
ALIGN_BLOCK = 1024
ALIGN_SUMS = 20


class NcwSdfStash(C.Structure):
    _fields_ = [("gamma", C.c_void_p), ("h", C.c_void_p * MAX_LAYERS), ("s", C.c_void_p * MAX_LAYERS),
                ("t", C.c_void_p * MAX_LAYERS), ("feat", C.c_void_p), ("dfeat", C.c_void_p),
                ("qbar", C.c_void_p * MAX_LAYERS), ("zbar", C.c_void_p * MAX_LAYERS), ("zsdf", C.c_void_p),
                ("one", C.c_void_p)]


class NcwWgradDesc(C.Structure):
    _fields_ = [("x", C.c_void_p), ("y", C.c_void_p), ("dense", C.c_void_p), ("dbias", C.c_void_p),
                ("rbx", C.c_int32), ("rby", C.c_int32), ("ld", C.c_int32), ("ksplit", C.c_int32),
                ("n_points", C.c_int64), ("n_points_dev", C.c_void_p)]


class NcwColorNet(C.Structure):
    _fields_ = [("w_f", C.c_void_p), ("wt_f", C.c_void_p), ("b_f", C.c_void_p),
                ("w_e", C.c_void_p * 4), ("wt_e", C.c_void_p * 4), ("b_e", C.c_void_p * 4),
                ("w_l", C.c_void_p * 8), ("wt_l", C.c_void_p * 8), ("b_l", C.c_void_p * 8),
                ("n_head", C.c_int32), ("n_lin", C.c_int32), ("rbf", C.c_int32), ("rbh", C.c_int32),
                ("rbc", C.c_int32), ("n_a", C.c_int32),
                ("w_f_lo", C.c_void_p), ("w_e_lo", C.c_void_p * 4), ("w_l_lo", C.c_void_p * 8),
                ("act_split", C.c_int32), ("_pad", C.c_int32)]


class NcwColorStash(C.Structure):
    _fields_ = [("aux1", C.c_void_p), ("aux2", C.c_void_p), ("f", C.c_void_p), ("e", C.c_void_p * 4),
                ("x", C.c_void_p * 8), ("zf", C.c_void_p), ("ze", C.c_void_p * 4), ("zx", C.c_void_p * 8),
                ("zo", C.c_void_p), ("aux_bias", C.c_void_p)]


class NcwNerfNet(C.Structure):
    _fields_ = [("w_p", C.c_void_p * 8), ("wt_p", C.c_void_p * 8), ("b_p", C.c_void_p * 8),
                ("w_alpha", C.c_void_p), ("wt_alpha", C.c_void_p), ("b_alpha", C.c_void_p),
                ("w_feat", C.c_void_p), ("wt_feat", C.c_void_p), ("b_feat", C.c_void_p),
                ("w_a", C.c_void_p * 4), ("wt_a", C.c_void_p * 4), ("b_a", C.c_void_p * 4),
                ("w_rgb", C.c_void_p), ("wt_rgb", C.c_void_p), ("b_rgb", C.c_void_p),
                ("D", C.c_int32), ("skip", C.c_int32), ("rbn", C.c_int32), ("rbh", C.c_int32),
                ("n_head", C.c_int32), ("n_a", C.c_int32),
                ("w_p_lo", C.c_void_p * 8), ("w_alpha_lo", C.c_void_p), ("w_feat_lo", C.c_void_p), ("w_a_lo", C.c_void_p * 4),
                ("w_rgb_lo", C.c_void_p)]


class NcwNerfStash(C.Structure):
    _fields_ = [("gp", C.c_void_p), ("aux1", C.c_void_p), ("h", C.c_void_p * 9), ("featn", C.c_void_p),
                ("e", C.c_void_p * 4), ("zp", C.c_void_p * 8), ("zalpha", C.c_void_p), ("zfeat", C.c_void_p),
                ("ze", C.c_void_p * 4), ("zrgb", C.c_void_p), ("aux_bias", C.c_void_p)]


def _ptr_struct(name, fields_ptr, fields_other=()):
    return type(name, (C.Structure,), {"_fields_": [(f, C.c_void_p) for f in fields_ptr] + list(fields_other)})


NcwCompositeIn = _ptr_struct(
    "NcwCompositeIn",
    ["rays_o", "rays_d", "z", "z_feed", "sample_dist", "sdf", "grad", "rgb", "density", "bg_rgb", "inv_s",
     "background_rgb", "cos_anneal_dev"],
    [("cos_anneal", C.c_float), ("R", C.c_int32), ("S", C.c_int32), ("O", C.c_int32), ("has_bg", C.c_int32),
     ("trim_sphere", C.c_int32)],
)
NcwCompositeOut = _ptr_struct(
    "NcwCompositeOut",
    ["color", "color_sphere", "color_bg", "weights", "weights_sum", "cdf", "inside", "depth", "normals", "eik",
     "mid_z", "dists", "bg_alpha", "weights_max"],
)
NcwCompositeGrad = _ptr_struct(
    "NcwCompositeGrad",
    ["d_color", "d_weights_sum", "d_depth", "d_eik_num", "d_sdf", "d_grad", "d_rgb", "d_density", "d_bg_rgb",
     "d_inv_s"],
    [("grad_scale", C.c_float), ("grad_scale_dev", C.c_void_p), ("d_normals", C.c_void_p)],
)

_VP = C.c_void_p
_PROTOS = {
    "ncw_mc_count": (C.c_int, [C.c_void_p, C.c_void_p, C.c_int, C.c_int, C.c_int, C.c_float, C.c_void_p, C.c_void_p, C.c_void_p]),
    "ncw_mc_emit": (C.c_int, [C.c_void_p, C.c_void_p, C.c_int, C.c_int, C.c_int, C.c_float, C.c_void_p, C.c_void_p, C.c_void_p,
                              C.c_void_p, C.c_void_p, C.c_void_p, C.c_void_p]),
    "ncw_ray_tail_fwd": (C.c_int, [C.c_void_p, C.c_void_p, C.c_void_p, C.c_int, C.c_void_p, C.c_void_p, C.c_void_p,
                                   C.c_void_p, C.c_void_p, C.c_int, C.c_void_p, C.c_void_p, C.c_void_p, C.c_void_p]),
    "ncw_ray_tail_bwd": (C.c_int, [C.c_void_p, C.c_void_p, C.c_void_p, C.c_int, C.c_void_p, C.c_void_p, C.c_void_p,
                                   C.c_int, C.c_void_p, C.c_void_p, C.c_void_p, C.c_void_p, C.c_void_p, C.c_void_p,
                                   C.c_void_p, C.c_void_p]),
    "ncw_ray_floor_fwd": (C.c_int, [_VP, _VP, _VP, C.c_int, C.POINTER(C.c_float), _VP, _VP, _VP, C.c_int, C.c_int, _VP, _VP, _VP]),
    "ncw_ray_floor_bwd": (C.c_int, [_VP, _VP, _VP, C.c_int, C.POINTER(C.c_float), C.c_int, C.c_int, _VP, _VP, _VP, _VP]),
    "ncw_adam_step": (C.c_int, [C.c_void_p, C.c_void_p, C.c_void_p, C.c_void_p, C.c_int64, C.c_float, C.c_float,
                                C.c_float, C.c_float, C.c_float, C.c_void_p, C.c_float, C.c_void_p]),
    "ncw_adam_step_dev": (C.c_int, [C.c_void_p, C.c_void_p, C.c_void_p, C.c_void_p, C.c_int64, C.c_void_p, C.c_void_p,
                                    C.c_float, C.c_void_p, C.c_float, C.c_float, C.c_float, C.c_float, C.c_void_p, C.c_int,
                                    C.c_float, C.c_float, C.c_void_p]),
    "ncw_wgrad_tiled": (C.c_int, [C.c_void_p, C.c_void_p, C.c_int, C.c_int, C.c_int, C.c_int, C.c_int64, C.c_void_p]),
    "ncw_wgrad_tiled_f16": (C.c_int, [C.c_void_p, C.c_void_p, C.c_int, C.c_int, C.c_int, C.c_int, C.c_int64, C.c_void_p]),
    "ncw_sdf_infer_points": (C.c_int, [C.POINTER(NcwSdfNet), C.c_int, C.POINTER(NcwPoints), C.c_int64, C.c_void_p,
                                       C.c_void_p]),
    "ncw_nn_cell_keys": (C.c_int, [_VP, C.c_int64, C.POINTER(NcwNnGrid), _VP, _VP]),
    "ncw_nn_cell_ranges": (C.c_int, [_VP, _VP, _VP, C.c_int64, _VP, _VP, _VP]),
    "ncw_nn_query": (C.c_int, [_VP, _VP, _VP, _VP, C.c_int64, C.POINTER(NcwNnGrid), C.c_int, C.c_float, _VP, _VP, _VP, _VP, _VP]),
    "ncw_nn_brute": (C.c_int, [_VP, C.c_int64, _VP, _VP, C.c_int64, _VP, _VP, _VP, _VP]),
    "ncw_nn_coarse": (C.c_int, [_VP, C.POINTER(NcwNnGrid), C.c_int, _VP, _VP]),
    "ncw_nn_query_within": (C.c_int, [_VP, _VP, _VP, C.c_int, _VP, _VP, C.c_int64, C.POINTER(NcwNnGrid), C.c_float, C.c_float, _VP, _VP, _VP]),
    "ncw_knn_query": (C.c_int, [_VP, _VP, _VP, C.c_int, _VP, _VP, _VP, C.c_int64, C.POINTER(NcwNnGrid), C.c_float, C.c_float, C.c_int, C.c_int, _VP, _VP, _VP, _VP, _VP]),
    "ncw_knn_pca": (C.c_int, [_VP, _VP, C.c_int64, _VP, _VP, C.c_int64, C.c_int, C.c_int, C.POINTER(C.c_float), _VP, _VP, _VP, _VP, _VP]),
    "ncw_raster_small": (C.c_int, [_VP, C.c_int64, _VP, C.c_int64, C.POINTER(NcwRasterView), _VP, _VP, _VP, _VP]),
    "ncw_raster_large": (C.c_int, [_VP, C.c_int64, _VP, C.POINTER(NcwRasterView), _VP, _VP, C.c_int64, _VP, _VP]),
    "ncw_raster_resolve": (C.c_int, [_VP, C.c_int64, _VP, _VP, _VP]),
    "ncw_raster_backproject": (C.c_int, [_VP, _VP, C.c_int64, C.c_int32, C.POINTER(C.c_float), _VP, _VP]),
    "ncw_raster_mark": (C.c_int, [_VP, _VP, C.c_int64, C.c_float, C.c_int64, _VP, _VP]),
    "ncw_view_rays": (C.c_int, [C.POINTER(NcwViewCamera), C.c_int64, C.c_int64, _VP, _VP]),
    "ncw_view_store": (C.c_int, [_VP, _VP, _VP, C.c_int64, C.c_int64, C.c_int64, _VP, _VP, _VP, _VP]),
    "ncw_image_reduce_scratch_bytes": (C.c_int64, []),
    "ncw_image_minmax": (C.c_int, [_VP, C.c_int64, _VP, _VP, _VP]),
    "ncw_depth_colormap": (C.c_int, [_VP, C.c_int64, _VP, _VP, _VP, _VP, _VP, _VP]),
    "ncw_image_sqerr": (C.c_int, [_VP, _VP, _VP, C.c_int64, C.c_int, _VP, _VP, _VP, _VP]),
    "ncw_image_ssim_scratch_floats": (C.c_int64, [C.c_int, C.c_int, C.c_int]),
    "ncw_image_ssim": (C.c_int, [_VP, _VP, C.c_int, C.c_int, C.c_int, C.c_int, _VP, _VP, _VP]),
    "ncw_trace_scratch_bytes": (C.c_int64, [C.c_int64]),
    "ncw_trace_begin": (C.c_int, [_VP, _VP, _VP, _VP, C.c_int64, _VP, _VP, _VP, _VP, _VP, _VP]),
    "ncw_trace_step": (C.c_int, [_VP, _VP, _VP, C.c_int64, _VP, _VP, _VP, C.c_int64, C.c_float, C.c_float, C.c_int, _VP, _VP, _VP,
                                 _VP, _VP, _VP]),
    "ncw_trace_finish": (C.c_int, [_VP, _VP, _VP, C.c_int64, _VP, _VP, _VP, _VP, _VP]),
    "ncw_trace_store": (C.c_int, [_VP, _VP, _VP, _VP, _VP, _VP, C.c_int64, C.POINTER(C.c_float), C.c_int64, C.c_int64, C.c_int64,
                                  _VP, _VP, _VP, _VP, _VP, _VP]),
    "ncw_sfm_depth_splat": (C.c_int, [_VP, _VP, _VP, C.c_int64, C.c_double, C.POINTER(C.c_float), C.c_int, C.c_int, _VP, _VP, _VP,
                                      _VP]),
    "ncw_cache_rows": (C.c_int, [C.POINTER(NcwViewCamera), _VP, _VP, C.c_int, C.c_int, _VP, _VP, C.c_int, C.c_float,
                                 C.POINTER(NcwCacheOctree), C.POINTER(NcwCacheOctree), C.c_int64, C.c_int64, C.c_int, _VP, _VP,
                                 _VP, _VP]),
    "ncw_source_batch": (C.c_int, [_VP, C.c_int64, _VP, _VP, _VP, C.c_int, _VP, _VP, _VP, C.POINTER(NcwCacheOctree), C.c_float, _VP,
                                   C.c_int64, C.c_int, _VP, _VP, _VP, _VP, C.POINTER(C.c_int), C.c_int, _VP, _VP]),
    "ncw_surf_weights": (C.c_int, [_VP, C.c_int64, _VP, C.c_int64, C.POINTER(C.c_double), _VP, _VP]),
    "ncw_surf_pick": (C.c_int, [_VP, C.c_int64, _VP, C.c_int64, _VP, _VP]),
    "ncw_surf_sample": (C.c_int, [_VP, _VP, _VP, C.c_int64, C.c_uint64, C.c_int64, C.c_int64, C.c_int64, C.c_int, _VP, _VP, _VP,
                                  _VP]),
    "ncw_ptm_pack": (C.c_int, [_VP, C.c_int64, _VP, C.c_int64, C.POINTER(C.c_double), C.POINTER(C.c_double), _VP, _VP, _VP]),
    "ncw_ptm_count": (C.c_int, [_VP, _VP, C.c_int64, C.POINTER(NcwPtmGrid), C.c_int64, _VP, _VP, _VP]),
    "ncw_ptm_emit": (C.c_int, [_VP, _VP, _VP, C.c_int64, C.POINTER(NcwPtmGrid), C.c_int64, _VP, _VP, _VP]),
    "ncw_ptm_ranges": (C.c_int, [_VP, _VP, _VP, C.c_int64, C.c_int64, _VP, _VP, _VP]),
    "ncw_ptm_cell_keys": (C.c_int, [_VP, C.c_int64, C.POINTER(NcwPtmGrid), _VP, _VP]),
    "ncw_ptm_query": (C.c_int, [_VP, C.c_int64, _VP, _VP, _VP, C.c_int64, _VP, _VP, C.c_int64, C.POINTER(NcwPtmGrid), C.c_int,
                                C.c_double, _VP, _VP, _VP, _VP, _VP, _VP]),
    "ncw_ptm_brute": (C.c_int, [_VP, _VP, C.c_int64, _VP, C.c_int64, _VP, C.c_int64, _VP, _VP, _VP, _VP, _VP]),
    "ncw_voxel_view_seen": (C.c_int, [C.POINTER(NcwVoxelView), C.POINTER(NcwCacheOctree), C.c_int64, C.c_int64, _VP, _VP, _VP, _VP]),
    "ncw_voxel_points_seen": (C.c_int, [_VP, C.c_int64, C.c_int, _VP, _VP, _VP]),
    "ncw_views_roi": (C.c_int, [_VP, _VP, C.c_int, C.POINTER(C.c_float), C.c_float, _VP, _VP, _VP]),
    "ncw_pixel_nearest": (C.c_int, [_VP, C.c_int, _VP, C.c_int64, C.c_int64, C.c_int, _VP, _VP]),
    "ncw_reproj_errors": (C.c_int, [_VP, C.c_int, _VP, C.c_int64, _VP, _VP, _VP, C.c_int64, _VP, C.c_int64, _VP, _VP, _VP]),
    "ncw_voxel_build": (C.c_int, [C.c_void_p, C.c_int64, C.c_int, C.c_void_p, C.c_void_p, C.c_void_p]),
    "ncw_ray_voxel_near_far": (C.c_int, [C.c_void_p, C.c_void_p, C.c_int, C.POINTER(C.c_float), C.c_float, C.c_int,
                                         C.c_void_p, C.c_void_p, C.c_void_p, C.c_void_p, C.c_void_p]),
    "ncw_ray_voxel_trace": (C.c_int, [C.c_void_p, C.c_void_p, C.c_int, C.c_int, C.c_void_p, C.c_void_p, C.c_void_p, C.c_void_p,
                                      C.c_void_p, C.c_void_p, C.c_void_p, C.c_void_p]),
    "ncw_color_fwd": (C.c_int, [C.POINTER(NcwColorNet), C.c_int, C.POINTER(NcwPoints), C.c_int64, C.c_void_p,
                                C.c_void_p, C.c_void_p, C.c_void_p, C.POINTER(NcwColorStash), C.c_void_p]),
    "ncw_color_bwd": (C.c_int, [C.POINTER(NcwColorNet), C.c_int, C.POINTER(NcwPoints), C.c_int64, C.c_void_p,
                                C.c_void_p, C.c_void_p, C.c_void_p, C.c_void_p, C.c_void_p, C.POINTER(NcwColorStash),
                                C.c_void_p]),
    "ncw_batch_assemble": (C.c_int, [C.c_void_p, C.c_int, C.c_void_p, C.c_void_p, C.c_int64, C.c_int64, C.c_int, C.c_void_p,
                                     C.c_void_p, C.c_void_p, C.c_void_p, C.c_void_p, C.c_int, C.c_void_p, C.c_void_p]),
    "ncw_ray_prologue": (C.c_int, [_VP, C.c_int, C.c_int64, C.POINTER(C.c_float), C.c_float, _VP, _VP, _VP, _VP, _VP, _VP, _VP]),
    "ncw_aux_ray_bias": (C.c_int, [_VP, C.c_int, C.c_int, C.c_int, _VP, _VP, C.c_int, C.c_int64, _VP, C.c_int, _VP]),
    "ncw_inv_s_fwd": (C.c_int, [_VP, _VP, _VP, _VP]),
    "ncw_inv_s_bwd": (C.c_int, [_VP, C.c_int64, _VP, _VP, _VP]),
    "ncw_loss_fwd": (C.c_int, [_VP, _VP, C.c_int64, _VP, _VP, C.c_int64, _VP, C.c_int64, C.c_float, C.c_float, C.c_float,
                               C.c_float, _VP, _VP]),
    "ncw_loss_bwd": (C.c_int, [_VP, _VP, _VP, C.c_int64, C.c_int64, C.c_int64, C.c_float, C.c_float, C.c_float, C.c_float,
                               _VP, _VP, _VP, _VP, _VP]),
    "ncw_scatter_add_rows": (C.c_int, [C.c_void_p, C.c_void_p, C.c_int64, C.c_int, C.c_int64, C.c_void_p, C.c_void_p]),
    "ncw_ray_sum_rows": (C.c_int, [C.c_void_p, C.c_int64, C.c_int, C.c_int, C.c_void_p, C.c_int, C.c_void_p]),
    "ncw_nerf_fwd": (C.c_int, [C.POINTER(NcwNerfNet), C.c_int, C.POINTER(NcwPoints), C.c_void_p, C.c_int64,
                               C.c_void_p, C.c_void_p, C.c_void_p, C.POINTER(NcwNerfStash), C.c_void_p]),
    "ncw_nerf_bwd": (C.c_int, [C.POINTER(NcwNerfNet), C.c_int, C.POINTER(NcwPoints), C.c_int64, C.c_void_p,
                               C.c_void_p, C.c_void_p, C.c_void_p, C.POINTER(NcwNerfStash), C.c_void_p]),
    "ncw_nerf_refine": (C.c_int, [C.POINTER(NcwNerfNet), C.c_int, C.POINTER(NcwPoints), C.c_int64, C.c_void_p, C.c_void_p,
                                  C.c_void_p, C.c_void_p]),
    "ncw_sdf_fwd": (C.c_int, [C.POINTER(NcwSdfNet), C.c_int, C.POINTER(NcwPoints), C.c_int64, C.c_void_p, C.c_void_p,
                              C.POINTER(NcwSdfStash), C.c_void_p]),
    "ncw_sdf_bwd": (C.c_int, [C.POINTER(NcwSdfNet), C.c_int, C.POINTER(NcwPoints), C.c_int64, C.c_void_p, C.c_void_p,
                              C.POINTER(NcwSdfStash), C.c_void_p]),
    "ncw_wgrad": (C.c_int, [C.c_void_p, C.c_void_p, C.c_int, C.c_int, C.c_int, C.c_int, C.c_int64, C.c_void_p]),
    "ncw_wgrad_ordered": (C.c_int, [C.c_void_p, C.c_void_p, C.c_int, C.c_int, C.c_int, C.c_int, C.c_int64, C.c_void_p,
                                    C.c_void_p]),
    "ncw_wgrad_ordered_scratch_floats": (C.c_int64, [C.c_int]),
    "ncw_stash_from_rows": (C.c_int, [C.c_int, C.c_void_p, C.c_int64, C.c_int, C.c_int, C.c_void_p, C.c_void_p]),
    "ncw_stash_to_rows": (C.c_int, [C.c_int, C.c_void_p, C.c_int64, C.c_int, C.c_int, C.c_void_p, C.c_void_p]),
    "ncw_sdf_infer_rays": (C.c_int, [C.POINTER(NcwSdfNet), C.c_int, _VP, _VP, _VP, C.c_int, C.c_int, _VP, _VP]),
    "ncw_sample_coarse": (C.c_int, [_VP, _VP, _VP, _VP, C.c_int, C.c_int, C.c_int, _VP, _VP, _VP, _VP, _VP, _VP]),
    "ncw_upsample": (C.c_int, [_VP, _VP, _VP, _VP, C.c_int, C.c_int, C.c_float, C.c_int, _VP, _VP]),
    "ncw_sort_merge": (C.c_int, [_VP, C.c_int, _VP, C.c_int, _VP, _VP, C.c_int, _VP, _VP, _VP]),
    "ncw_boundary": (C.c_int, [_VP, _VP, _VP, C.c_int, C.c_int, C.c_int, _VP, _VP]),
    "ncw_bg_select": (C.c_int, [_VP, _VP, _VP, _VP, C.c_int, C.c_int, C.c_int, _VP, _VP, _VP, _VP]),
    "ncw_composite_fwd": (C.c_int, [C.POINTER(NcwCompositeIn), C.POINTER(NcwCompositeOut), _VP]),
    "ncw_composite_bwd": (C.c_int, [C.POINTER(NcwCompositeIn), C.POINTER(NcwCompositeGrad), _VP]),
    "ncw_appfit_loss": (C.c_int, [_VP, _VP, _VP, _VP, _VP, _VP, _VP, C.c_int, C.c_int, C.c_int, C.c_float, _VP, _VP, _VP, _VP, _VP,
                                  _VP]),
    "ncw_appfit_step_scratch_floats": (C.c_int64, [C.c_int64, C.c_int]),
    "ncw_appfit_step": (C.c_int, [_VP, C.c_int64, C.c_int, _VP, _VP, C.c_int, C.c_int, _VP, _VP, _VP, _VP, C.c_float, C.c_float,
                                  C.c_float, C.c_float, _VP, C.c_float, _VP, C.c_int64, _VP]),
    "ncw_mesh_cc_hook": (C.c_int, [_VP, _VP, C.c_int64, C.c_int64, _VP, _VP]),
    "ncw_mesh_cc_flatten": (C.c_int, [_VP, C.c_int64, _VP]),
    "ncw_mesh_cc_sizes": (C.c_int, [_VP, _VP, C.c_int64, C.c_int64, _VP, _VP, _VP]),
    "ncw_mesh_face_select": (C.c_int, [_VP, C.c_int64, C.c_int64, _VP, C.c_int, _VP, _VP, _VP, _VP]),
    "ncw_mesh_compact_mark": (C.c_int, [_VP, _VP, C.c_int64, C.c_int64, _VP, _VP]),
    "ncw_mesh_compact_faces": (C.c_int, [_VP, _VP, _VP, _VP, C.c_int64, C.c_int64, C.c_int64, _VP, _VP]),
    "ncw_mesh_sc_keys": (C.c_int, [_VP, _VP, C.c_int64, C.POINTER(C.c_double), C.c_double, C.POINTER(C.c_int64), _VP, _VP]),
    "ncw_mesh_sc_faces": (C.c_int, [_VP, C.c_int64, C.c_int64, _VP, C.c_int64, _VP, _VP, _VP, _VP]),
    "ncw_mesh_sc_place": (C.c_int, [_VP, _VP, C.c_int64, C.c_int64, _VP, C.c_int64, _VP, _VP, C.c_int64, _VP, _VP, C.c_int64,
                                    C.POINTER(C.c_double), C.c_double, C.POINTER(C.c_int64), C.c_double, _VP, _VP, _VP, _VP, _VP]),
    "ncw_align_transform": (C.c_int, [_VP, C.c_int64, C.POINTER(C.c_double), C.POINTER(C.c_double), C.POINTER(C.c_float),
                                      C.POINTER(C.c_float), C.c_float, _VP, _VP, _VP]),
    "ncw_align_sums_blocks": (C.c_int64, [C.c_int64]),
    "ncw_align_sums": (C.c_int, [_VP, C.c_int64, C.POINTER(C.c_double), _VP, C.c_int64, C.POINTER(C.c_double), _VP, _VP, C.c_float,
                                 C.POINTER(C.c_double), _VP, _VP, _VP, _VP, _VP]),
    "ncw_mcs_neighbors": (C.c_int, [_VP, C.c_int64, C.c_int, _VP, _VP]),
    "ncw_mcs_count": (C.c_int, [_VP, C.c_int64, _VP, _VP, C.c_int64, C.c_int, C.c_int, C.c_float, _VP, _VP, _VP]),
    "ncw_mcs_cube_ids": (C.c_int, [_VP, C.c_int64, C.c_int, C.c_int, _VP, C.c_int64, _VP, _VP]),
    "ncw_mcs_emit": (C.c_int, [_VP, C.c_int64, _VP, _VP, C.c_int64, C.c_int, C.c_int, C.c_float, _VP, _VP, _VP, _VP, _VP, C.c_int64,
                               C.c_int64, _VP, _VP, _VP]),
    "ncw_fuse_insert": (C.c_int, [_VP, _VP, _VP, _VP, C.c_int64, C.c_int32, C.POINTER(NcwFuseGrid), C.POINTER(NcwFuseTable), _VP]),
    "ncw_fuse_move": (C.c_int, [C.POINTER(NcwFuseTable), C.POINTER(NcwFuseTable), _VP]),
    "ncw_fuse_resolve": (C.c_int, [C.POINTER(NcwFuseTable), _VP, C.c_int64, C.POINTER(NcwFuseGrid), _VP, _VP, _VP, _VP, _VP, _VP,
                                   _VP, _VP]),
    "ncw_abi_version": (C.c_int, []),
    "ncw_source_hash": (C.c_char_p, []),
    "ncw_device_info": (C.c_int, [C.c_char_p, C.c_int]),
    "ncw_grad_norm_scratch_floats": (C.c_int64, []),
    "ncw_grad_norm": (C.c_int, [C.c_void_p, C.c_int64, C.c_void_p, C.c_void_p, C.c_void_p]),
    "ncw_pack_weights": (C.c_int, [C.c_void_p, C.c_void_p, C.c_int, C.c_int, C.c_void_p]),
    "ncw_unpack_grads": (C.c_int, [C.c_void_p, C.c_void_p, C.c_int, C.c_int, C.c_void_p]),
    "ncw_sdf_infer": (C.c_int, [C.POINTER(NcwSdfNet), C.c_int, C.c_void_p, C.c_int64, C.c_void_p, C.c_void_p]),
}

_lib = None

PROFILE = None


def _wrap_timed(name, fn):
    def call(*args):
        if PROFILE is None:
            return fn(*args)
        import torch

        e0, e1 = torch.cuda.Event(enable_timing=True), torch.cuda.Event(enable_timing=True)
        e0.record()
        r = fn(*args)
        e1.record()
        PROFILE.setdefault(name, []).append((e0, e1))
        return r

    return call



class NeuconwHipError(RuntimeError):
    pass


def exported_symbols():
    return sorted(_PROTOS)


def get_lib():
    global _lib
    if _lib is not None:
        return _lib
    if not os.path.isfile(LIB_PATH):
        raise NeuconwHipError(
            "libneuconw_hip.so not found at %s -- run `python -c 'import __graft_entry__ as g; g.build()'`. "
            "There is no CPU / PyTorch fallback for the hot path." % LIB_PATH
        )
    lib = C.CDLL(LIB_PATH)
    ns = type("NcwLib", (), {})()
    for name, (res, args) in _PROTOS.items():
        fn = getattr(lib, name)
        fn.restype = res
        fn.argtypes = args
        setattr(ns, name, _wrap_timed(name, fn))
    v = lib.ncw_abi_version()
    if v != ABI_VERSION:
        raise NeuconwHipError("libneuconw_hip.so ABI %d != binding ABI %d: rebuild" % (v, ABI_VERSION))
    if not os.environ.get("NEUCONW_HIP_LIB") and os.path.isdir(os.path.join(HERE, "csrc")):
        from . import build as _b

        built, now = lib.ncw_source_hash().decode(), _b.source_hash()
        if built != now:
            raise NeuconwHipError("libneuconw_hip.so was built from other sources (%s.. != %s..): rebuild with "
                                  "`python -c 'import __graft_entry__ as g; g.build()'`" % (built[:12], now[:12]))
    ns._cdll = lib
    _lib = ns
    return ns


def check(code, what):
    if code != 0:
        raise NeuconwHipError("%s failed with code %d" % (what, code))


def stream_ptr(device=None):
    import torch

    return C.c_void_p(torch.cuda.current_stream(device).cuda_stream)


def ptr(t):
    if t is None:
        return C.c_void_p(0)
    assert t.is_contiguous(), "non-contiguous tensor handed to the C ABI"
    return C.c_void_p(t.data_ptr())
```

neuralrecon-w_amd/rayops.py:

```python
import torch

from . import lib as L


def _f(t):
    return t.contiguous().float()


def _chk_cuda(*ts):
    for t in ts:
        if t is not None and not t.is_cuda:
            raise L.NeuconwHipError("hot-path tensors must live on the GPU (no CPU fallback)")


def sample_coarse(near, far, s_near, s_far, n_samples, n_outside, rand_shift=None, rand_out=None):
    _chk_cuda(near, far)
    R = near.shape[0]
    dev = near.device
    near, far, s_near, s_far = (_f(t).reshape(-1) for t in (near, far, s_near, s_far))
    z = torch.empty(R, n_samples, device=dev)
    zo = torch.empty(R, max(n_outside, 0), device=dev)
    sd = torch.empty(R, device=dev)
    rs = _f(rand_shift).reshape(-1) if rand_shift is not None else None
    ro = _f(rand_out) if rand_out is not None else None
    lib = L.get_lib()
    L.check(lib.ncw_sample_coarse(L.ptr(near), L.ptr(far), L.ptr(s_near), L.ptr(s_far), R, n_samples, n_outside,
                                  L.ptr(rs), L.ptr(ro), L.ptr(z), L.ptr(zo), L.ptr(sd), L.stream_ptr(dev)),
            "ncw_sample_coarse")
    return z, (zo if n_outside > 0 else None), sd.reshape(R, 1)


def upsample(rays_o, rays_d, z, sdf, n_new, inv_s):
    _chk_cuda(z, sdf)
    R, n = z.shape
    out = torch.empty(R, n_new, device=z.device)
    lib = L.get_lib()
    L.check(lib.ncw_upsample(L.ptr(_f(rays_o)), L.ptr(_f(rays_d)), L.ptr(_f(z)), L.ptr(_f(sdf)), R, n, float(inv_s),
                             n_new, L.ptr(out), L.stream_ptr(z.device)), "ncw_upsample")
    return out


def sort_merge(a, b, pa=None, pb=None):
    _chk_cuda(a, b)
    R, na = a.shape
    nb = b.shape[1]
    out = torch.empty(R, na + nb, device=a.device)
    pout = torch.empty(R, na + nb, device=a.device) if pa is not None else None
    lib = L.get_lib()
    L.check(lib.ncw_sort_merge(L.ptr(_f(a)), na, L.ptr(_f(b)), nb, L.ptr(_f(pa) if pa is not None else None),
                               L.ptr(_f(pb) if pb is not None else None), R, L.ptr(out), L.ptr(pout),
                               L.stream_ptr(a.device)), "ncw_sort_merge")
    return out, pout


def boundary(near, far, z, nb):
    _chk_cuda(z)
    R, n = z.shape
    out = torch.empty(R, nb, device=z.device)
    lib = L.get_lib()
    L.check(lib.ncw_boundary(L.ptr(_f(near).reshape(-1)), L.ptr(_f(far).reshape(-1)), L.ptr(_f(z)), n, R, nb,
                             L.ptr(out), L.stream_ptr(z.device)), "ncw_boundary")
    return out


class CompositeCtx:

    def __init__(self, rays_o, rays_d, z, sample_dist, sdf, grad, rgb, inv_s, cos_anneal, z_feed=None, density=None,
                 bg_rgb=None, background_rgb=None, trim_sphere=True):
        _chk_cuda(z, sdf, grad, rgb)
        self.dev = z.device
        self.R, self.S = z.shape
        self.has_bg = z_feed is not None
        self.O = (z_feed.shape[1] - self.S) if self.has_bg else 0
        self.t = dict(rays_o=_f(rays_o), rays_d=_f(rays_d), z=_f(z), z_feed=_f(z_feed) if self.has_bg else None,
                      sample_dist=_f(sample_dist).reshape(-1), sdf=_f(sdf), grad=_f(grad), rgb=_f(rgb),
                      density=_f(density) if self.has_bg else None, bg_rgb=_f(bg_rgb) if self.has_bg else None,
                      inv_s=_f(inv_s).reshape(1),
                      background_rgb=_f(background_rgb).reshape(3) if background_rgb is not None else None)
        self.t["cos_anneal_dev"] = _f(cos_anneal).reshape(1) if torch.is_tensor(cos_anneal) else None
        s = L.NcwCompositeIn()
        for k, v in self.t.items():
            setattr(s, k, v.data_ptr() if v is not None else 0)
        s.cos_anneal = 0.0 if torch.is_tensor(cos_anneal) else float(cos_anneal)
        s.R, s.S, s.O, s.has_bg, s.trim_sphere = self.R, self.S, self.O, int(self.has_bg), int(bool(trim_sphere))
        self.cin = s

    def forward(self):
        R, S, M, dev = self.R, self.S, self.S + self.O, self.dev
        o = dict(color=torch.empty(R, 3, device=dev), color_sphere=torch.empty(R, 3, device=dev),
                 color_bg=torch.empty(R, 3, device=dev), weights=torch.empty(R, M, device=dev),
                 weights_sum=torch.empty(R, device=dev), cdf=torch.empty(R, S, device=dev),
                 inside=torch.empty(R, S, device=dev), depth=torch.empty(R, device=dev),
                 normals=torch.empty(R, 3, device=dev), eik=torch.empty(2, R, device=dev),
                 mid_z=torch.empty(R, S, device=dev), dists=torch.empty(R, S, device=dev),
                 bg_alpha=torch.empty(R, M, device=dev) if self.has_bg else None,
                 weights_max=torch.empty(R, device=dev))
        s = L.NcwCompositeOut()
        for k, v in o.items():
            setattr(s, k, v.data_ptr() if v is not None else 0)
        lib = L.get_lib()
        L.check(lib.ncw_composite_fwd(self.cin, s, L.stream_ptr(dev)), "ncw_composite_fwd")
        return o

    def backward(self, d_color, d_weights_sum, d_depth, d_eik_num, grad_scale=1.0, grad_scale_dev=None, d_normals=None):
        R, S, M, dev = self.R, self.S, self.S + self.O, self.dev
        z = lambda t, shape: _f(t).reshape(shape) if t is not None else torch.zeros(shape, device=dev)
        ups = dict(d_color=z(d_color, (R, 3)), d_weights_sum=z(d_weights_sum, (R,)), d_depth=z(d_depth, (R,)),
                   d_eik_num=z(d_eik_num, (R,)))
        if d_normals is not None:
            _chk_cuda(d_normals)
            ups["d_normals"] = _f(d_normals).reshape(R, 3)
        g = dict(d_sdf=torch.empty(R, S, device=dev), d_grad=torch.empty(R, S, 3, device=dev),
                 d_rgb=torch.empty(R, S, 3, device=dev),
                 d_density=torch.empty(R, M, device=dev) if self.has_bg else None,
                 d_bg_rgb=torch.empty(R, M, 3, device=dev) if self.has_bg else None,
                 d_inv_s=torch.empty(R, device=dev))
        s = L.NcwCompositeGrad()
        for k, v in list(ups.items()) + list(g.items()):
            setattr(s, k, v.data_ptr() if v is not None else 0)
        s.grad_scale = float(grad_scale)
        s.grad_scale_dev = grad_scale_dev.data_ptr() if grad_scale_dev is not None else 0
        lib = L.get_lib()
        L.check(lib.ncw_composite_bwd(self.cin, s, L.stream_ptr(dev)), "ncw_composite_bwd")
        self._keep = ups
        return g
```

neuralrecon-w_amd/renderer.py:

```python
import ctypes as C
import os

import numpy as np
import torch
import yaml

from . import lib as L
from . import rayops
from .neuconw import default_infer_prec, default_prec, points_struct
from .packing import pack_many, unpack_many
from .stash import LeaseGuard, WgradBatch

from .labels import LABEL_IDS, label_id as _label_id

SKY_LABEL_ID = LABEL_IDS["sky"]


class _RenderFn(torch.autograd.Function):

    @staticmethod
    def forward(ctx, rdr, train, rays_o, rays_d, z, z_out, sample_dist, cos_anneal, background_rgb, a_embedded, variance,
                *params):
        prec = rdr.prec
        neuconw, nerf = rdr.neuconw, rdr.nerf
        R, S = z.shape
        dev = z.device
        ctx.set_materialize_grads(False)
        inv_s = torch.empty(1, device=dev, dtype=torch.float32)
        s_val = torch.empty(1, device=dev, dtype=torch.float32)
        L.check(L.get_lib().ncw_inv_s_fwd(L.ptr(variance.detach().reshape(1).float().contiguous()), L.ptr(inv_s), L.ptr(s_val),
                                          L.stream_ptr(dev)), "ncw_inv_s_fwd")
        a_det = a_embedded.detach().contiguous().float()
        use_bg = rdr.render_bg and rdr.n_outside > 0 and z_out is not None
        z_feed = density = bg_rgb = nctx = None
        if use_bg:
            M = S + z_out.shape[1]
            select = refine = None
            if rdr.trim_sphere:
                refine = (z, M - S)
                if not rdr.bg_dense:
                    select = refine
            side = rdr._bg_stream(dev) if rdr.use_bg_stream else None
            if side is not None:
                main = torch.cuda.current_stream(dev)
                side.wait_stream(main)
                with torch.cuda.stream(side):
                    z_feed, _ = rayops.sort_merge(z, z_out)
                    pts_bg = points_struct(rays_o=rays_o, rays_d=rays_d, z=z_feed, sample_dist=sample_dist, mode=2)
                    density, bg_rgb, nctx = nerf.fwd_stash(pts_bg, R * M, prec, a_det, select=select, train=train, refine=refine)
                density.record_stream(main)
                bg_rgb.record_stream(main)
                z_feed.record_stream(main)
            else:
                z_feed, _ = rayops.sort_merge(z, z_out)
                pts_bg = points_struct(rays_o=rays_o, rays_d=rays_d, z=z_feed, sample_dist=sample_dist, mode=2)
                density, bg_rgb, nctx = nerf.fwd_stash(pts_bg, R * M, prec, a_det, select=select, train=train, refine=refine)
            assert z_feed.shape[1] == M
            density, bg_rgb = density.view(R, M), bg_rgb.view(R, M, 3)
        try:
            pts_in = points_struct(rays_o=rays_o, rays_d=rays_d, z=z, sample_dist=sample_dist, mode=2)
            sdf, grad, sctx = neuconw.sdf_net.fwd_stash(pts_in, R * S, prec, train=train)
            feat_ptr = sctx["arena"].ptr(sctx["ids"]["feat"])
            rgb, cctx = neuconw.color_net.fwd_stash(pts_in, R * S, prec, grad, a_det, feat_ptr, train=train)
        finally:
            if use_bg and rdr.use_bg_stream:
                torch.cuda.current_stream(dev).wait_stream(rdr._bg_stream(dev))
        comp = rayops.CompositeCtx(rays_o, rays_d, z, sample_dist, sdf.view(R, S), grad.view(R, S, 3),
                                   rgb.view(R, S, 3), inv_s, cos_anneal, z_feed, density, bg_rgb, background_rgb,
                                   rdr.trim_sphere)
        o = comp.forward()
        ctx.rdr, ctx.comp, ctx.sctx, ctx.cctx, ctx.nctx = rdr, comp, sctx, cctx, nctx
        ctx.inv_s, ctx.n_params, ctx.use_bg = inv_s, len(params), use_bg
        ctx.a_shape = a_embedded.shape
        ctx.variance = variance
        ctx.params = params
        extras = (o["color_sphere"], o["color_bg"], o["weights"], o["cdf"], o["inside"], o["normals"],
                  sdf.view(R, S), grad.view(R, S, 3), o["mid_z"], o["dists"], o["eik"][1], inv_s, s_val,
                  o["weights_max"])
        ctx.floor_normal = bool(rdr.floor_normal)
        ctx.mark_non_differentiable(*((extras[:5] + extras[6:]) if ctx.floor_normal else extras))
        ctx.guard = LeaseGuard([c["lease"] for c in (sctx, cctx, nctx) if c is not None])
        ctx.train = train
        if not train:
            ctx.guard.release()
        return (o["color"], o["weights_sum"], o["depth"], o["eik"][0]) + extras

    @staticmethod
    def backward(ctx, d_color, d_wsum, d_depth, d_eik, *unused):
        rdr, comp, sctx, cctx, nctx = ctx.rdr, ctx.comp, ctx.sctx, ctx.cctx, ctx.nctx
        neuconw, nerf = rdr.neuconw, rdr.nerf
        prec = rdr.prec
        dev = ctx.inv_s.device
        if not ctx.train:
            raise RuntimeError("NeuconWRenderer: backward through a forward-only render (it ran under torch.no_grad(), or no "
                               "input required a gradient): nothing was stashed")
        ctx.guard.consume()
        sc = rdr.loss_scale.tensor(dev) if prec == L.PREC_F16 else None
        sc_mul, sc_inv = (sc[0:1], sc[1:2]) if sc is not None else (None, None)
        if ctx.floor_normal:
            g = comp.backward(d_color, d_wsum, d_depth, d_eik, grad_scale_dev=sc_mul, d_normals=unused[5])
        else:
            g = comp.backward(d_color, d_wsum, d_depth, d_eik, grad_scale_dev=sc_mul)
        R, S = comp.R, comp.S
        d_grad = g["d_grad"].view(R * S, 3)
        dfeat_ptr = sctx["arena"].ptr(sctx["ids"]["dfeat"])
        n_a = int(ctx.a_shape[-1])
        ordered = rdr.reproducible if rdr.reproducible is not None else (prec == L.PREC_F32)
        lib = L.get_lib()
        M = comp.S + comp.O
        side = rdr._bg_stream(dev) if (ctx.use_bg and rdr.use_bg_stream and not ordered) else None
        d_a_bg = None
        if side is not None:
            d_a_bg = torch.zeros(ctx.a_shape, device=dev, dtype=torch.float32)
            side.wait_stream(torch.cuda.current_stream(dev))
            with torch.cuda.stream(side):
                nerf.bwd_stash(nctx, g["d_density"].view(R * M), g["d_bg_rgb"].view(R * M, 3), d_a_bg)
            for t_ in (g["d_density"], g["d_bg_rgb"]):
                t_.record_stream(side)
        try:
            if ordered:
                d_a = torch.empty(ctx.a_shape, device=dev, dtype=torch.float32)
                rows = torch.empty(R * S, n_a, device=dev, dtype=torch.float32)
                neuconw.color_net.bwd_stash(cctx, g["d_rgb"].view(R * S, 3), d_grad, None, dfeat_ptr, d_a_rows=rows)
                L.check(lib.ncw_ray_sum_rows(L.ptr(rows), R, S, n_a, L.ptr(d_a), 0, L.stream_ptr(dev)), "ncw_ray_sum_rows")
            else:
                d_a = torch.zeros(ctx.a_shape, device=dev, dtype=torch.float32)
                neuconw.color_net.bwd_stash(cctx, g["d_rgb"].view(R * S, 3), d_grad, d_a, dfeat_ptr)
            neuconw.sdf_net.bwd_stash(sctx, g["d_sdf"].view(R * S), d_grad)
        finally:
            if side is not None:
                torch.cuda.current_stream(dev).wait_stream(side)
        plans = [sctx["plan"], cctx["plan"]]
        if side is not None:
            d_a.add_(d_a_bg)
            plans.append(nctx["plan"])
        elif ctx.use_bg:
            if ordered:
                rows_bg = (torch.zeros if nctx.get("sel_count") is not None else torch.empty)(R * M, n_a, device=dev,
                                                                                             dtype=torch.float32)
                nerf.bwd_stash(nctx, g["d_density"].view(R * M), g["d_bg_rgb"].view(R * M, 3), None, d_a_rows=rows_bg)
                L.check(lib.ncw_ray_sum_rows(L.ptr(rows_bg), R, M, n_a, L.ptr(d_a), 1, L.stream_ptr(dev)),
                        "ncw_ray_sum_rows")
            else:
                nerf.bwd_stash(nctx, g["d_density"].view(R * M), g["d_bg_rgb"].view(R * M, 3), d_a)
            plans.append(nctx["plan"])
        sel = nctx.get("sel_count") if ctx.use_bg else None
        sel_frac, sel_bucket = nctx["lease"].get("sel_plan", (None, None)) if sel is not None else (None, None)
        tag = (cctx["arena"].buf.data_ptr(), nctx["arena"].buf.data_ptr() if ctx.use_bg else None, prec,
               None if sel is None else sel.data_ptr(), sel_bucket)
        batch = sctx["lease"].get("wgrad_batch")
        if batch is None or batch.tag != tag:
            batch = WgradBatch(dev, prec, R * S)
            batch.tag = tag
            neuconw.sdf_net.add_wgrads(sctx, batch)
            neuconw.color_net.add_wgrads(cctx, batch)
            if ctx.use_bg:
                b_bg = WgradBatch(dev, prec, R * (comp.S + comp.O), n_dev=nctx.get("sel_count"), sel_fraction=sel_frac)
                nerf.add_wgrads(nctx, b_bg)
                batch.extend(b_bg)
            sctx["lease"]["wgrad_batch"] = batch
        torch._foreach_zero_([p.g_arena for p in plans])
        batch.run()
        out = [None] * len(ctx.params)
        direct = False
        if rdr.__dict__.get("_gv_adopted", False):
            flat, views = rdr._grad_views(ctx.params)
            direct = all(p.grad is not None and p.grad.data_ptr() == views[id(p)].data_ptr() for p in ctx.params)
        if direct:
            keep = unpack_many(plans, views, accumulate=True, grad_mul_dev=sc_inv)
        else:
            tmp = torch.zeros(sum(p.numel() for p in ctx.params), device=dev, dtype=torch.float32)
            tviews, off = {}, 0
            out = []
            for p in ctx.params:
                v = tmp[off:off + p.numel()].view(p.shape)
                tviews[id(p)] = v
                out.append(v)
                off += p.numel()
            keep = unpack_many(plans, tviews, grad_mul_dev=sc_inv)
        ctx._keep = (keep, batch)
        d_var = torch.empty(1, device=dev, dtype=torch.float32)
        L.check(lib.ncw_inv_s_bwd(L.ptr(g["d_inv_s"]), R, L.ptr(ctx.inv_s), L.ptr(d_var), L.stream_ptr(dev)), "ncw_inv_s_bwd")
        d_var = d_var.reshape(ctx.variance.shape)
        if sc_inv is not None:
            d_a.mul_(sc_inv)
            d_var = d_var * sc_inv
        ctx.guard.release()
        return (None, None, None, None, None, None, None, None, None, d_a, d_var) + tuple(out)


class _EmbedFn(torch.autograd.Function):

    @staticmethod
    def forward(ctx, weight, ts, direct_grad):
        ctx.save_for_backward(ts)
        ctx.shape, ctx.direct_grad = weight.shape, direct_grad
        return weight.detach().index_select(0, ts)

    @staticmethod
    def backward(ctx, d_a):
        (ts,) = ctx.saved_tensors
        d_a = d_a.contiguous().float()
        dw = ctx.direct_grad if ctx.direct_grad is not None else torch.zeros(ctx.shape, device=d_a.device, dtype=torch.float32)
        L.check(L.get_lib().ncw_scatter_add_rows(L.ptr(d_a), L.ptr(ts), d_a.shape[0], d_a.shape[1], dw.shape[0], L.ptr(dw),
                                                 L.stream_ptr(d_a.device)), "ncw_scatter_add_rows")
        return (None if ctx.direct_grad is not None else dw), None, None


class _RayTailFn(torch.autograd.Function):

    @staticmethod
    def forward(ctx, wsum, depth, eik_num, eik_den, label, depth_gt, depth_w, ids, has_mask, has_depth):
        R, dev = wsum.shape[0], wsum.device
        f = lambda t: t.detach().contiguous().float()
        wsum_c, depth_c, num_c, den_c = f(wsum), f(depth), f(eik_num), f(eik_den)
        label_c = label.contiguous().long() if (has_mask and label is not None) else None
        gt_c, w_c = (f(depth_gt), f(depth_w)) if has_depth else (None, None)
        mask_error = torch.empty(R, device=dev) if has_mask else None
        sfm = torch.empty(R, device=dev) if has_depth else None
        scal = torch.empty(3, device=dev)
        ids_arr = (C.c_int * 4)(*(list(ids) + [0] * (4 - len(ids))))
        L.check(L.get_lib().ncw_ray_tail_fwd(L.ptr(wsum_c), L.ptr(label_c), ids_arr, len(ids), L.ptr(depth_c),
                                             L.ptr(gt_c), L.ptr(w_c), L.ptr(num_c), L.ptr(den_c), R, L.ptr(mask_error),
                                             L.ptr(sfm), L.ptr(scal), L.stream_ptr(dev)), "ncw_ray_tail_fwd")
        ctx.keep = (wsum_c, depth_c, label_c, gt_c, w_c, scal, ids_arr, len(ids), has_mask, has_depth)
        return mask_error, sfm, scal[0:1]

    @staticmethod
    def backward(ctx, d_me, d_sfm, d_ge):
        wsum_c, depth_c, label_c, gt_c, w_c, scal, ids_arr, n_ids, has_mask, has_depth = ctx.keep
        R, dev = wsum_c.shape[0], wsum_c.device
        g = lambda t: None if t is None else t.contiguous().float()
        d_me, d_sfm, d_ge = (g(d_me) if has_mask else None), (g(d_sfm) if has_depth else None), g(d_ge)
        d_wsum, d_depth, d_num = (torch.empty(R, device=dev) for _ in range(3))
        L.check(L.get_lib().ncw_ray_tail_bwd(L.ptr(wsum_c), L.ptr(label_c), ids_arr, n_ids, L.ptr(depth_c), L.ptr(gt_c),
                                             L.ptr(w_c), R, L.ptr(scal), L.ptr(d_me), L.ptr(d_sfm), L.ptr(d_ge),
                                             L.ptr(d_wsum), L.ptr(d_depth), L.ptr(d_num), L.stream_ptr(dev)),
                "ncw_ray_tail_bwd")
        return d_wsum, d_depth, d_num, None, None, None, None, None, None, None


class _RayFloorFn(torch.autograd.Function):

    @staticmethod
    def forward(ctx, normals, label, rays_o, rays_d, depth, ids, n_gt, scaled):
        R, dev = normals.shape[0], normals.device
        f = lambda t: t.detach().contiguous().float()
        normals_c, label_c = f(normals), label.contiguous().long()
        fe, scal = torch.empty(R, 3, device=dev), torch.zeros(2, device=dev)
        ids_arr = (C.c_int * 4)(*(list(ids) + [0] * (4 - len(ids))))
        gt_arr = (C.c_float * 3)(*n_gt)
        L.check(L.get_lib().ncw_ray_floor_fwd(L.ptr(normals_c), L.ptr(label_c), ids_arr, len(ids), gt_arr, L.ptr(f(rays_o)),
                                              L.ptr(f(rays_d)), L.ptr(f(depth)), R, int(scaled), L.ptr(fe), L.ptr(scal),
                                              L.stream_ptr(dev)), "ncw_ray_floor_fwd")
        ctx.keep = (normals_c, label_c, ids_arr, len(ids), gt_arr, int(scaled), scal)
        ctx.mark_non_differentiable(scal)
        ctx.set_materialize_grads(False)
        return fe, scal

    @staticmethod
    def backward(ctx, d_fe, _d_scal):
        normals_c, label_c, ids_arr, n_ids, gt_arr, scaled, scal = ctx.keep
        if d_fe is None:
            return (None,) * 8
        R, dev = normals_c.shape[0], normals_c.device
        d_fe = d_fe.contiguous().float()
        d_normals = torch.empty(R, 3, device=dev)
        L.check(L.get_lib().ncw_ray_floor_bwd(L.ptr(normals_c), L.ptr(label_c), ids_arr, n_ids, gt_arr, R, scaled, L.ptr(scal),
                                              L.ptr(d_fe), L.ptr(d_normals), L.stream_ptr(dev)), "ncw_ray_floor_bwd")
        return (d_normals,) + (None,) * 7


class LossScale:

    def __init__(self, init):
        self.init, self.buf = float(init), None

    def tensor(self, device):
        if self.buf is None or self.buf.device != torch.device(device):
            self.buf = torch.tensor([self.init, 1.0 / self.init], device=device, dtype=torch.float32)
        return self.buf

    def set(self, value):
        self.init = float(value)
        if self.buf is not None:
            self.buf.copy_(torch.tensor([self.init, 1.0 / self.init]))

    def value(self):
        return self.init if self.buf is None else float(self.buf[0])


class NeuconWRenderer:
    @property
    def grad_scale(self):
        return self.loss_scale.value()

    @grad_scale.setter
    def grad_scale(self, v):
        self.loss_scale.set(v)

    def __init__(self, nerf, neuconw, embeddings, n_samples, n_importance, n_outside, up_sample_steps, perturb,
                 origin, radius, s_val_base=0, spc_options=None, sample_range=None, boundary_samples=None,
                 nerf_far_override=False, render_bg=True, trim_sphere=True, save_sample=False,
                 save_step_sample=False, mesh_mask_list=None, floor_normal=False, depth_loss=False,
                 floor_labels=None, prec=None, infer_prec=None):
        self.nerf, self.neuconw, self.embeddings = nerf, neuconw, embeddings
        self.n_samples, self.n_importance, self.n_outside = n_samples, n_importance, n_outside
        self.up_sample_steps, self.perturb, self.s_val_base = up_sample_steps, perturb, s_val_base
        self.boundary_samples, self.nerf_far_override = boundary_samples, nerf_far_override
        self.octree_data, self.sample_range, self.fine_octree_data = None, sample_range, None
        spc_options = spc_options or {}
        if self.nerf_far_override:
            self.recontruct_path = spc_options["recontruct_path"]
            self.min_track_length = spc_options["min_track_length"]
            self.voxel_size = spc_options["voxel_size"]
        self.sfm_to_gt = torch.eye(4)
        scene_config_path = os.path.join(spc_options.get("recontruct_path", ""), "config.yaml")
        if os.path.isfile(scene_config_path):
            with open(scene_config_path, "r") as f:
                scene_config = yaml.load(f, Loader=yaml.FullLoader)
            origin, radius = scene_config["origin"], scene_config["radius"]
            self.sfm_to_gt = torch.from_numpy(np.array(scene_config["sfm2gt"]))
        self.origin = torch.from_numpy(np.array(origin, dtype=np.float64))
        self.radius = radius
        self.render_bg, self.floor_normal, self.floor_labels = render_bg, floor_normal, floor_labels
        self.depth_loss, self.save_sample, self.trim_sphere = depth_loss, save_sample, trim_sphere
        self.mesh_mask_list = mesh_mask_list
        self.save_step_sample = save_step_sample
        if floor_normal:
            if len([_label_id(name) for name in (floor_labels or [])]) > 4:
                raise ValueError("floor_labels: at most 4 labels (ncw_ray_floor_fwd), got %d" % len(floor_labels))
        if save_sample or save_step_sample:
            raise NotImplementedError("debug PLY dumps (open3d) are out of scope")
        self.prec = default_prec() if prec is None else prec
        self.infer_prec = infer_prec
        if self.n_samples + self.n_importance + (self.boundary_samples or 0) + self.n_outside > 1088:
            raise ValueError("n_samples + n_importance + boundary_samples + n_outside = %d > 1088: the per-ray kernels keep a "
                             "ray's samples in LDS (csrc/ncw_rays.hip: 512 in the standard kernels, 1088 in the large-ray ones -- "
                             "config/defaults.py's own 512 + 512 + 32 fits)."
                             % (self.n_samples + self.n_importance + (self.boundary_samples or 0) + self.n_outside))
        self.bg_dense = os.environ.get("NEUCONW_BG_DENSE", "0") not in ("0", "")
        self.loss_scale = LossScale(float(os.environ.get("NEUCONW_F16_LOSS_SCALE", "1024")))
        self.use_bg_stream = os.environ.get("NEUCONW_BG_STREAM", "1") not in ("0", "")
        self.sync_free = False
        self.reproducible = None

    def _bg_stream(self, device):
        st = self.__dict__.get("_bg_streams")
        if st is None:
            st = self._bg_streams = {}
        key = str(device)
        if key not in st:
            st[key] = torch.cuda.Stream(device=device)
        return st[key]

    def _sdf_rays(self, rays_o, rays_d, z):
        R, n = z.shape
        out = torch.empty(R, n, device=z.device, dtype=torch.float32)
        sp = self.__dict__.get("sampler_prec")
        sp = self.prec if sp is None else sp
        plan = self.neuconw.sdf_net.packed(sp)
        L.check(L.get_lib().ncw_sdf_infer_rays(plan.net, sp, L.ptr(rays_o), L.ptr(rays_d), L.ptr(z), R, n,
                                               L.ptr(out), L.stream_ptr(z.device)), "ncw_sdf_infer_rays")
        return out

    def up_sample(self, rays_o, rays_d, z_vals, sdf, n_importance, inv_s, step=0):
        return rayops.upsample(rays_o, rays_d, z_vals, sdf, n_importance, inv_s)

    def cat_z_vals(self, rays_o, rays_d, z_vals, new_z_vals, sdf, last=False):
        if last:
            return rayops.sort_merge(z_vals, new_z_vals)[0], sdf
        new_sdf = self._sdf_rays(rays_o, rays_d, new_z_vals.contiguous())
        return rayops.sort_merge(z_vals, new_z_vals, sdf, new_sdf)

    @torch.no_grad()
    def sparse_sampler(self, rays_o, rays_d, near, far, perturb, _rand=None, far_override=None):
        dev = rays_o.device
        R = rays_o.shape[0]
        rays_o, rays_d = rays_o.contiguous().float(), rays_d.contiguous().float()
        near, far, s_near, s_far = self.ray_intervals(rays_o, rays_d, near, far, far_override)
        n_out = self.n_outside if (self.render_bg and self.n_outside > 0) else 0
        rs = ro = None
        if perturb > 0:
            if _rand is not None:
                rs, ro = _rand
            else:
                rs = torch.rand([R, 1], device=dev)
                ro = torch.rand([R, n_out], device=dev) if n_out > 0 else None
        z, z_out, sample_dist = rayops.sample_coarse(near, far, s_near, s_far, self.n_samples, n_out, rs, ro)
        n_samples = self.n_samples
        if self.n_importance > 0:
            sdf = self._sdf_rays(rays_o, rays_d, z)
            for i in range(self.up_sample_steps):
                z_new = rayops.upsample(rays_o, rays_d, z, sdf, self.n_importance // self.up_sample_steps,
                                        64 * 2 ** (self.s_val_base + i))
                z, sdf = self.cat_z_vals(rays_o, rays_d, z, z_new, sdf, last=(i + 1 == self.up_sample_steps))
            n_samples = self.n_samples + self.n_importance
        if self.fine_octree_data is not None and self.boundary_samples and self.boundary_samples > 0:
            zb = rayops.boundary(near, far, z, self.boundary_samples)
            z, _ = rayops.sort_merge(zb, z)
        return n_samples, z, z_out, sample_dist

    @torch.no_grad()
    def ray_intervals(self, rays_o, rays_d, near, far, far_override=None):
        if self.nerf_far_override if far_override is None else far_override:
            if self.octree_data is None:
                self.octree_data = self.get_octree(rays_o.device)
            near, far, _ = self.get_near_far_octree(self.octree_data, rays_o, rays_d, near, far)
        s_near, s_far = near, far
        if self.fine_octree_data is not None:
            s_near, s_far, _ = self.get_near_far_sdf(self.fine_octree_data, rays_o, rays_d, near, far)
        return near, far, s_near, s_far

    def get_octree(self, device):
        from . import voxel

        return voxel.octree_from_sfm(self.recontruct_path, self.min_track_length, self.voxel_size, device)

    def get_near_far_octree(self, octree_data, rays_o, rays_d, near, far):
        from . import voxel

        o_sfm = (rays_o * self.radius).view(-1, 3) + self.origin.to(rays_o.device).float()
        vn, vf = voxel.get_near_far(o_sfm, rays_d, octree_data)
        hit = vn > 0
        near = torch.where(hit, vn / self.radius, near)
        far = torch.where(hit, (vf + self.voxel_size) / self.radius, far)
        return near, far, hit

    def get_near_far_sdf(self, octree_data, rays_o, rays_d, near, far):
        from . import voxel

        o_sfm = (rays_o * self.radius).view(-1, 3) + self.origin.to(rays_o.device).float()
        surf, _ = voxel.get_near_far(o_sfm, rays_d, octree_data)
        miss = surf <= 0
        rng = self.sample_range * octree_data["voxel_size"]
        v_near = torch.where(miss, near, (surf - rng) / self.radius)
        v_far = torch.where(miss, far, (surf + rng) / self.radius)
        return v_near, v_far, ~miss

    def _floor_normal_gt(self):
        c = self.__dict__.get("_floor_gt")
        if c is None or c[1] is not self.sfm_to_gt:
            v = self.sfm_to_gt.detach().cpu().float()[:3, :3].T @ torch.tensor([0.0, 0.0, 1.0])
            v = v / torch.linalg.norm(v)
            self._floor_gt = c = (tuple(float(x) for x in v), self.sfm_to_gt)
        return c[0]

    def _grad_views(self, params):
        key = tuple(id(p) for p in params)
        c = self.__dict__.get("_gv")
        if c is None or c[0] != key or c[1].device != params[0].device:
            flat = torch.zeros(sum(p.numel() for p in params), device=params[0].device, dtype=torch.float32)
            views, off = {}, 0
            for p in params:
                views[id(p)] = flat[off:off + p.numel()].view(p.shape)
                off += p.numel()
            self._gv = c = (key, flat, views)
        return c[1], c[2]

    def adopt_grad_buffer(self, params, flat):
        params = list(params)
        assert [id(p) for p in params] == [id(p) for p in self._params()], "adopt_grad_buffer: parameter order"
        assert flat.numel() == sum(p.numel() for p in params) and flat.dtype == torch.float32
        views, off = {}, 0
        for p in params:
            views[id(p)] = flat[off:off + p.numel()].view(p.shape)
            off += p.numel()
        self._gv = (tuple(id(p) for p in params), flat, views)
        self._gv_adopted = True

    def flat_grad_buffer(self):
        c = self.__dict__.get("_gv")
        return None if c is None else c[1]

    def _params(self):
        ps = list(self.neuconw.sdf_net.parameters()) + list(self.neuconw.color_net.parameters())
        nf = self.nerf
        ps += [p for n, p in nf.named_parameters() if not n.startswith("views_linears")]
        return ps

    def ray_prologue(self, rays):
        device = rays.device
        if self.origin.device != device:
            self.origin = self.origin.to(device).float()
            self.sfm_to_gt = self.sfm_to_gt.to(device).float()
        R = rays.shape[0]
        rays_c = rays.contiguous().float()
        rays_o, rays_d = torch.empty(R, 3, device=device), torch.empty(R, 3, device=device)
        near, far = torch.empty(R, 1, device=device), torch.empty(R, 1, device=device)
        depth_gt, depth_weight = torch.empty(R, device=device), torch.empty(R, device=device)
        if self.__dict__.get("_origin_host") is None or self._origin_host[1] is not self.origin:
            self._origin_host = ((C.c_float * 3)(*[float(v) for v in self.origin.reshape(-1).tolist()]), self.origin)
        L.check(L.get_lib().ncw_ray_prologue(L.ptr(rays_c), rays_c.shape[1], R, self._origin_host[0], float(self.radius),
                                             L.ptr(rays_o), L.ptr(rays_d), L.ptr(near), L.ptr(far), L.ptr(depth_gt),
                                             L.ptr(depth_weight), L.stream_ptr(device)), "ncw_ray_prologue")
        return rays_o, rays_d, near, far, depth_gt, depth_weight

    def render(self, rays, ts, label, perturb_overwrite=-1, background_rgb=None, cos_anneal_ratio=0.0, _rand=None, _z_override=None):
        return self._render_with_normals(rays, ts, label, perturb_overwrite, background_rgb, cos_anneal_ratio, _rand, _z_override)[0]

    def _render_with_normals(self, rays, ts, label, perturb_overwrite=-1, background_rgb=None, cos_anneal_ratio=0.0, _rand=None,
                             _z_override=None, sfm_depth_loss=True, far_override=None, a_code=None):
        device = rays.device
        if not rays.is_cuda:
            raise L.NeuconwHipError("NeuconWRenderer.render: rays are not on a GPU; the hot path has no CPU fallback")
        if self.origin.device != device:
            self.origin = self.origin.to(device).float()
            self.sfm_to_gt = self.sfm_to_gt.to(device).float()
        if self.__dict__.get("sampler_prec") is None:
            nets = [self.neuconw.sdf_net, self.neuconw.color_net] + ([self.nerf] if (self.render_bg and self.n_outside > 0) else [])
            pack_many([(m, m.plan(self.prec)) for m in nets])
        R = rays.shape[0]
        rays_o, rays_d, near, far, depth_gt, depth_weight = self.ray_prologue(rays)
        emb_a = self.embeddings["a"]
        ordered = self.reproducible if self.reproducible is not None else (self.prec == L.PREC_F32)
        if a_code is not None:
            if not a_code.is_cuda:
                raise L.NeuconwHipError("NeuconWRenderer.render: a_code is not on a GPU; the hot path has no CPU fallback")
            a_embedded = a_code.detach().reshape(1, -1).float().expand(R, -1).contiguous()
        elif (not ordered and isinstance(emb_a, torch.nn.Embedding) and emb_a.padding_idx is None and emb_a.max_norm is None
                and not emb_a.sparse and emb_a.weight.dtype == torch.float32 and torch.is_grad_enabled()
                and emb_a.weight.requires_grad and ts.dtype == torch.int64 and ts.dim() == 1):
            g = emb_a.weight.grad
            direct = g if (self.__dict__.get("_gv_adopted", False) and g is not None and g.is_contiguous()
                           and g.dtype == torch.float32) else None
            a_embedded = _EmbedFn.apply(emb_a.weight, ts.contiguous(), direct)
# ... 67 lines not shown
```

neuralrecon-w_amd/trainer.py:

```python
import torch
import torch.distributed as dist


class FlatParams:

    def __init__(self, modules, renderer=None):
        modules = list(modules)
        seen, params = set(), []
        first = list(renderer._params()) if renderer is not None else []
        for p in first + [p for m in modules for p in m.parameters()]:
            if id(p) not in seen and p.requires_grad:
                seen.add(id(p))
                params.append(p)
        if not params:
            raise ValueError("no trainable parameters")
        dev = params[0].device
        for p in params:
            if p.device != dev or p.dtype != torch.float32:
                raise ValueError("FlatParams needs fp32 parameters on one device")
        n = sum(p.numel() for p in params)
        self.params = params
        self.flat = torch.nn.Parameter(torch.empty(n, device=dev, dtype=torch.float32))
        self.flat_grad = torch.zeros(n, device=dev, dtype=torch.float32)
        self.flat.grad = self.flat_grad
        self.slices = {}
        off = 0
        with torch.no_grad():
            for p in params:
                k = p.numel()
                view = self.flat.data[off:off + k].view(p.shape)
                view.copy_(p.data)
                p.data = view
                p.grad = self.flat_grad[off:off + k].view(p.shape)
                self.slices[id(p)] = (off, k)
                off += k
        for m in modules:
            for sub in m.modules():
                sub.__dict__["_ncw_version_srcs"] = sub.__dict__.get("_ncw_version_srcs", ()) + (self,)
        self._epoch = 0
        if renderer is not None and first:
            nr = sum(p.numel() for p in first)
            renderer.adopt_grad_buffer(first, self.flat_grad[:nr])
        self.renderer = renderer

    @property
    def _version(self):
        return (self.flat._version, self._epoch)

    def mark_updated(self):
        self._epoch += 1

    def zero_grad(self):
        self.flat_grad.zero_()
        for p in self.params:
            if p.grad is None:
                off, k = self.slices[id(p)]
                p.grad = self.flat_grad[off:off + k].view(p.shape)

    def allreduce(self, world_size=None, group=None, async_op=False, force=False):
        if not dist.is_available() or not dist.is_initialized():
            return None
        world_size = dist.get_world_size(group) if world_size is None else world_size
        if world_size == 1 and not force:
            return None
        avg = dist.get_backend(group) == "nccl"
        work = dist.all_reduce(self.flat_grad, op=dist.ReduceOp.AVG if avg else dist.ReduceOp.SUM, group=group,
                               async_op=True)
        h = _ReduceHandle(work, None if avg else (self.flat_grad, world_size))
        if async_op:
            return h
        h.wait()
        return None

    def broadcast(self, src=0, group=None):
        if dist.is_available() and dist.is_initialized() and dist.get_world_size(group) > 1:
            dist.broadcast(self.flat.data, src=src, group=group)


class _ReduceHandle:
    def __init__(self, work, div):
        self.work, self.div = work, div

    def wait(self):
        if self.work is not None:
            self.work.wait()
            self.work = None
            if self.div is not None:
                self.div[0].div_(self.div[1])


class FlatAdam:

    def __init__(self, flat_params, lr, betas=(0.9, 0.999), eps=1e-7, clip=None, loss_scale=None, growth_interval=2000,
                 scale_min=1.0, scale_max=65536.0):
        self.fp = flat_params
        self.lr_dev = torch.empty(1, device=flat_params.flat_grad.device, dtype=torch.float32)
        self.lr = float(lr)
        self.betas, self.eps, self.clip = (float(betas[0]), float(betas[1])), float(eps), clip
        self.exp_avg = torch.zeros_like(flat_params.flat_grad)
        self.exp_avg_sq = torch.zeros_like(flat_params.flat_grad)
        self.state = torch.zeros(8, device=flat_params.flat_grad.device, dtype=torch.int32)
        self.loss_scale, self.growth_interval = loss_scale, int(growth_interval)
        self.scale_min, self.scale_max = float(scale_min), float(scale_max)

    @property
    def lr(self):
        return self._lr

    @lr.setter
    def lr(self, v):
        self._lr = float(v)
        self.lr_dev.fill_(self._lr)

    @property
    def step_count(self):
        return int(self.state[0])

    @step_count.setter
    def step_count(self, v):
        self.state[0] = int(v)

    @property
    def skipped_steps(self):
        return int(self.state[2])

    def step(self):
        from . import lib as L

        fp = self.fp
        if not fp.flat_grad.is_cuda:
            raise L.NeuconwHipError("FlatAdam: parameters are not on a GPU; there is no CPU fallback")
        b1, b2 = self.betas
        need_norm = self.clip is not None or self.loss_scale is not None
        norm = None
        if need_norm:
            lib = L.get_lib()
            if self.__dict__.get("_norm_scratch") is None or self._norm_scratch.device != fp.flat_grad.device:
                self._norm_scratch = torch.zeros(int(lib.ncw_grad_norm_scratch_floats()), device=fp.flat_grad.device, dtype=torch.float32)
                self._norm = torch.empty(1, device=fp.flat_grad.device, dtype=torch.float32)
            norm = self._norm
            L.check(lib.ncw_grad_norm(L.ptr(fp.flat_grad), fp.flat_grad.numel(), L.ptr(self._norm_scratch), L.ptr(norm),
                                      L.stream_ptr(fp.flat_grad.device)), "ncw_grad_norm")
            norm = norm[0]
        L.check(L.get_lib().ncw_adam_step_dev(
            L.ptr(fp.flat.data), L.ptr(fp.flat_grad), L.ptr(self.exp_avg), L.ptr(self.exp_avg_sq), fp.flat_grad.numel(),
            L.ptr(self.state), L.ptr(norm), self.lr, L.ptr(self.lr_dev), b1, b2, self.eps,
            float(self.clip) if self.clip is not None else 0.0, L.ptr(self.loss_scale), self.growth_interval,
            self.scale_min, self.scale_max, L.stream_ptr(fp.flat_grad.device)), "ncw_adam_step_dev")
        fp.mark_updated()
        return norm.clone() if norm is not None else None

    def state_dict(self):
        return {"step": self.step_count, "exp_avg": self.exp_avg, "exp_avg_sq": self.exp_avg_sq, "lr": self.lr,
                "betas": self.betas, "eps": self.eps}

    def torch_state_dict(self, param_order):
        state, ids = {}, []
        for i, p in enumerate(param_order):
            ids.append(i)
            sl = self.fp.slices.get(id(p))
            if sl is None:
                continue
            off, k = sl
            state[i] = {"step": torch.tensor(float(self.step_count)),
                        "exp_avg": self.exp_avg[off:off + k].view(p.shape).detach().cpu().clone(),
                        "exp_avg_sq": self.exp_avg_sq[off:off + k].view(p.shape).detach().cpu().clone()}
        group = {"lr": self.lr, "betas": self.betas, "eps": self.eps, "weight_decay": 0, "amsgrad": False,
                 "maximize": False, "foreach": None, "capturable": False, "differentiable": False, "fused": None,
                 "params": ids}
        return {"state": state, "param_groups": [group]}

    def load_state_dict(self, sd, param_order=None):
        if "param_groups" in sd:
            if param_order is None:
                raise ValueError("a torch.optim.Adam state_dict needs param_order")
            step = 0
            for i, p in enumerate(param_order):
                st, sl = sd["state"].get(i), self.fp.slices.get(id(p))
                if st is None or sl is None:
                    continue
                off, k = sl
                self.exp_avg[off:off + k].copy_(st["exp_avg"].reshape(-1))
                self.exp_avg_sq[off:off + k].copy_(st["exp_avg_sq"].reshape(-1))
                step = max(step, int(float(st["step"])))
            self.step_count = step
            return
        self.step_count = int(sd["step"])
        self.exp_avg.copy_(sd["exp_avg"])
        self.exp_avg_sq.copy_(sd["exp_avg_sq"])


class TrainStep:

    def __init__(self, renderer, modules, loss_fn, lr, eps=1e-7, betas=(0.9, 0.999), clip=0.99, world_size=1,
                 group=None, capture=False, capture_warmup=3, native_optimizer=None):
        self.renderer, self.loss_fn, self.clip = renderer, loss_fn, clip
        self.world_size, self.group = world_size, group
        self.capture, self.capture_warmup = bool(capture), int(capture_warmup)
        self._n_eager, self._graphs, self._static = 0, None, None
        self.fp = FlatParams(modules, renderer)
        if world_size > 1:
            self.fp.broadcast(group=group)
        kw = dict(lr=lr, eps=eps, betas=betas)
        self.native = True if native_optimizer is None else bool(native_optimizer)
        if self.capture:
            renderer.sync_free = True
            if not self.native:
                raise ValueError("TrainStep(capture=True) needs the native optimiser (torch's path checks the gradient "
                                 "norm on the host)")
        if self.native:
            from . import lib as L

            ls = renderer.loss_scale.tensor(self.fp.flat_grad.device) if getattr(renderer, "prec", None) == L.PREC_F16 else None
            self.opt = FlatAdam(self.fp, clip=clip, loss_scale=ls, **kw)
            return
        try:
            self.opt = torch.optim.Adam([self.fp.flat], fused=True, **kw)
        except (RuntimeError, TypeError, ValueError):
            self.opt = torch.optim.Adam([self.fp.flat], **kw)

    def _fwd_bwd(self, rays, ts, label, targets, background_rgb, cos_anneal_ratio, render_kw):
        self.fp.zero_grad()
        out = self.renderer.render(rays, ts, label, background_rgb=background_rgb,
                                   cos_anneal_ratio=cos_anneal_ratio, **render_kw)
        loss = self.loss_fn(out, targets)
        loss.backward()
        return loss, out

    def _update(self):
        if self.native:
            self.last_grad_norm = self.opt.step()
            return
        norm = torch.nn.utils.clip_grad_norm_([self.fp.flat], self.clip if self.clip is not None else float("inf"))
        self.last_grad_norm = norm
        if not bool(torch.isfinite(norm)):
            self.skipped_steps = getattr(self, "skipped_steps", 0) + 1
            ls = getattr(self.renderer, "loss_scale", None)
            if ls is not None and ls.buf is not None:
                ls.set(max(ls.value() * 0.5, 1.0))
            return
        self.opt.step()
        self.fp.mark_updated()

    def eager_step(self, rays, ts, label, targets, background_rgb=None, cos_anneal_ratio=0.0, **render_kw):
        loss, out = self._fwd_bwd(rays, ts, label, targets, background_rgb, cos_anneal_ratio, render_kw)
        h = self.fp.allreduce(self.world_size, self.group, async_op=True)
        if h is not None:
            h.wait()
        self._update()
        return loss, out

    def _capture(self, rays, ts, label, targets, background_rgb, render_kw):
        dev = rays.device
        st = dict(rays=rays.clone(), ts=ts.clone(), label=label.clone(), targets=targets.clone(),
                  bg=None if background_rgb is None else background_rgb.clone(),
                  cos=torch.zeros(1, device=dev, dtype=torch.float32))
        self._render_kw = dict(render_kw)
        torch.cuda.synchronize(dev)
        g1 = torch.cuda.CUDAGraph()
        with torch.cuda.graph(g1):
            loss, out = self._fwd_bwd(st["rays"], st["ts"], st["label"], st["targets"], st["bg"], st["cos"],
                                      self._render_kw)
            if self.world_size == 1:
                self._update()
        g2 = None
        if self.world_size > 1:
            g2 = torch.cuda.CUDAGraph()
            with torch.cuda.graph(g2, pool=g1.pool()):
                self._update()
        st["loss"], st["out"] = loss.detach(), {k: (v.detach() if torch.is_tensor(v) else v) for k, v in out.items()}
        self._graphs, self._static = (g1, g2), st

    def __call__(self, rays, ts, label, targets, background_rgb=None, cos_anneal_ratio=0.0, **render_kw):
        if not self.capture:
            return self.eager_step(rays, ts, label, targets, background_rgb, cos_anneal_ratio, **render_kw)
        if self._graphs is None:
            if self._n_eager < self.capture_warmup:
                self._n_eager += 1
                loss, out = self.eager_step(rays, ts, label, targets, background_rgb, cos_anneal_ratio, **render_kw)
                return loss.detach(), {k: (v.detach() if torch.is_tensor(v) else v) for k, v in out.items()}
            import gc
            gc.collect()
            self._capture(rays, ts, label, targets, background_rgb, render_kw)
        st = self._static
        if dict(render_kw) != self._render_kw or rays.shape != st["rays"].shape:
            raise ValueError("captured TrainStep: batch shape and render keywords are fixed at capture time")
        st["rays"].copy_(rays, non_blocking=True)
        st["ts"].copy_(ts, non_blocking=True)
        st["label"].copy_(label, non_blocking=True)
        st["targets"].copy_(targets, non_blocking=True)
        if st["bg"] is not None:
            st["bg"].copy_(background_rgb, non_blocking=True)
        st["cos"].fill_(float(cos_anneal_ratio))
        g1, g2 = self._graphs
        g1.replay()
        if g2 is not None:
            self.fp.allreduce(self.world_size, self.group)
            g2.replay()
        self.fp._epoch += 1
        return st["loss"], st["out"]


def reference_param_order(embedding_a, neuconw, nerf):
# ... 64 lines not shown
```

Baseline: 33.39 million ray-samples/s.

## Fuse grad-norm with Adam prep, merge presorted samples, trim small ops

Measured after the change: 33.82 million ray-samples/s, median of 6. 1.01x the previous value.

```diff
diff --git a/include/neuconw_hip.h b/include/neuconw_hip.h
--- a/include/neuconw_hip.h
+++ b/include/neuconw_hip.h
@@ -199,6 +199,8 @@
                      float* rays_d, float* near, float* far, float* depth_gt, float* depth_weight, void* stream);
 int ncw_inv_s_fwd(const float* variance, float* inv_s, float* s_val, void* stream);
 int ncw_inv_s_bwd(const float* d_inv_s_rays, int64_t R, const float* inv_s, float* d_variance, void* stream);
+int ncw_inv_s_bwd_scaled(const float* d_inv_s_rays, int64_t R, const float* inv_s, const float* mul_dev, float* d_variance,
+                         void* stream);
 int ncw_loss_fwd(const float* color, const float* rgbs, int64_t R, const float* gradient_error, const float* mask_error,
                  int64_t n_mask, const float* sfm, int64_t n_sfm, float coef, float igr_w, float mask_w, float depth_w,
                  float* loss, void* stream);
@@ -247,6 +249,10 @@
                       const float* total_norm, float lr, const float* lr_dev, float beta1, float beta2, float eps,
                       float max_norm, float* loss_scale, int growth_interval, float scale_min, float scale_max,
                       void* stream);
+int ncw_grad_norm_adam_step(float* param, float* grad, float* exp_avg, float* exp_avg_sq, int64_t n, float* scratch, float* norm,
+                            NcwAdamState* state, float lr, const float* lr_dev, float beta1, float beta2, float eps,
+                            float max_norm, float* loss_scale, int growth_interval, float scale_min, float scale_max,
+                            void* stream);
 
 int ncw_stash_from_rows(int prec, const float* rows, int64_t n, int F, int rb, void* stash, void* stream);
 int ncw_stash_to_rows(int prec, const void* stash, int64_t n, int F, int rb, float* rows, void* stream);
@@ -258,6 +264,8 @@
                  float inv_s, int n_new, float* z_new, void* stream);
 int ncw_sort_merge(const float* a, int na, const float* b, int nb, const float* pa, const float* pb, int R,
                    float* out, float* pout, void* stream);
+int ncw_merge_sorted(const float* a, int na, const float* b, int nb, const float* pa, const float* pb, int R,
+                     float* out, float* pout, void* stream);
 int ncw_boundary(const float* near, const float* far, const float* z, int n, int R, int nb, float* zb,
                  void* stream);
 
diff --git a/neuralrecon-w_amd/appfit.py b/neuralrecon-w_amd/appfit.py
--- a/neuralrecon-w_amd/appfit.py
+++ b/neuralrecon-w_amd/appfit.py
@@ -105,7 +105,7 @@
         if g.use_bg:
             g.O = z_out.shape[1]
             g.select, g.refine = _bg_choice(rdr, z, g.O)
-            z_feed, _ = rayops.sort_merge(z, z_out)
+            z_feed, _ = rayops.merge_sorted(z, z_out)
             g.pts_bg = points_struct(rays_o=rays_o, rays_d=rays_d, z=z_feed, sample_dist=sample_dist, mode=2)
             density, bg_rgb, nctx = nerf.fwd_stash(g.pts_bg, R * (S + g.O), prec, a0, select=g.select, train=False, refine=g.refine)
             StashCache.release(nctx["lease"])
diff --git a/neuralrecon-w_amd/csrc/ncw_glue.hip b/neuralrecon-w_amd/csrc/ncw_glue.hip
--- a/neuralrecon-w_amd/csrc/ncw_glue.hip
+++ b/neuralrecon-w_amd/csrc/ncw_glue.hip
@@ -41,14 +41,15 @@
 }
 
 __global__ __launch_bounds__(256) void inv_s_bwd_kernel(const float* __restrict__ d, int64_t R, const float* __restrict__ inv_s,
-                                                        float* __restrict__ d_var) {
+                                                        const float* __restrict__ mul, float* __restrict__ d_var) {
     __shared__ float sm[256];
     float a = 0.f;
     for (int64_t i = threadIdx.x; i < R; i += 256) a += d[i];
     const float tot = block_sum_fixed(a, sm);
     if (threadIdx.x == 0) {
         const float v = inv_s[0];
-        d_var[0] = (v > 1e-6f && v < 1e6f) ? tot * 10.0f * v : 0.f;
+        const float dv = (v > 1e-6f && v < 1e6f) ? tot * 10.0f * v : 0.f;
+        d_var[0] = mul ? dv * mul[0] : dv;
     }
 }
 
@@ -151,7 +152,15 @@
 
 extern "C" int ncw_inv_s_bwd(const float* d_inv_s_rays, int64_t R, const float* inv_s, float* d_variance, void* stream) {
     if (!d_inv_s_rays || !inv_s || !d_variance || R < 0) return NCW_E_BADARG;
-    hipLaunchKernelGGL(inv_s_bwd_kernel, dim3(1), dim3(256), 0, (hipStream_t)stream, d_inv_s_rays, R, inv_s, d_variance);
+    hipLaunchKernelGGL(inv_s_bwd_kernel, dim3(1), dim3(256), 0, (hipStream_t)stream, d_inv_s_rays, R, inv_s, nullptr, d_variance);
+    NCW_CHECK_LAUNCH();
+    return 0;
+}
+
+extern "C" int ncw_inv_s_bwd_scaled(const float* d_inv_s_rays, int64_t R, const float* inv_s, const float* mul_dev,
+                                    float* d_variance, void* stream) {
+    if (!d_inv_s_rays || !inv_s || !d_variance || R < 0) return NCW_E_BADARG;
+    hipLaunchKernelGGL(inv_s_bwd_kernel, dim3(1), dim3(256), 0, (hipStream_t)stream, d_inv_s_rays, R, inv_s, mul_dev, d_variance);
     NCW_CHECK_LAUNCH();
     return 0;
 }
diff --git a/neuralrecon-w_amd/csrc/ncw_optim.hip b/neuralrecon-w_amd/csrc/ncw_optim.hip
--- a/neuralrecon-w_amd/csrc/ncw_optim.hip
+++ b/neuralrecon-w_amd/csrc/ncw_optim.hip
@@ -43,11 +43,20 @@
     }
 }
 
-__global__ void adam_prep_kernel(NcwAdamState* __restrict__ st, const float* __restrict__ total_norm, float lr,
-                                 const float* __restrict__ lr_dev, float beta1, float beta2, float max_norm,
-                                 float* __restrict__ loss_scale, int growth_interval, float scale_min, float scale_max) {
-    if (threadIdx.x != 0 || blockIdx.x != 0) return;
-    const float tn = total_norm ? total_norm[0] : 0.f;
+struct AdamPrep {
+    NcwAdamState* st;
+    const float* lr_dev;
+    float* loss_scale;
+    float lr, beta1, beta2, max_norm, scale_min, scale_max;
+    int growth_interval;
+};
+
+NCW_DEV void adam_prep(const AdamPrep& P, bool has_norm, float tn) {
+    NcwAdamState* st = P.st;
+    float* loss_scale = P.loss_scale;
+    const float lr = P.lr, beta1 = P.beta1, beta2 = P.beta2, max_norm = P.max_norm, scale_min = P.scale_min, scale_max = P.scale_max;
+    const float* lr_dev = P.lr_dev;
+    const int growth_interval = P.growth_interval;
     const bool finite = tn < __builtin_inff() && tn == tn;
     if (!finite) {
         st->skip_now = 1;
@@ -75,8 +84,13 @@
     const double bc2 = 1.0 - pow((double)beta2, (double)t);
     st->step_size = (float)(l / bc1);
     st->bc2_sqrt = (float)sqrt(bc2);
-    st->coef = (total_norm && max_norm > 0.f) ? fminf(max_norm / (tn + 1e-6f), 1.f) : 1.f;
+    st->coef = (has_norm && max_norm > 0.f) ? fminf(max_norm / (tn + 1e-6f), 1.f) : 1.f;
     st->last_norm = tn;
+}
+
+__global__ void adam_prep_kernel(AdamPrep P, const float* __restrict__ total_norm) {
+    if (threadIdx.x != 0 || blockIdx.x != 0) return;
+    adam_prep(P, total_norm != nullptr, total_norm ? total_norm[0] : 0.f);
 }
 
 __global__ __launch_bounds__(256) void adam_dev_kernel(float* __restrict__ p, float* __restrict__ g, float* __restrict__ m,
@@ -118,8 +132,9 @@
 
 constexpr int NORM_BLOCKS = 256;
 
+template <bool PREP>
 __global__ __launch_bounds__(256) void grad_norm_kernel(const float* __restrict__ g, int64_t n, float* __restrict__ scratch,
-                                                        float* __restrict__ norm) {
+                                                        float* __restrict__ norm, AdamPrep P) {
     __shared__ float wsum[4];
     __shared__ int last;
     const int64_t quads = (n + 3) / 4;
@@ -154,7 +169,9 @@
     if ((threadIdx.x & 63) == 0) wsum[threadIdx.x >> 6] = t;
     __syncthreads();
     if (threadIdx.x == 0) {
-        norm[0] = sqrtf((wsum[0] + wsum[1]) + (wsum[2] + wsum[3]));
+        const float tn = sqrtf((wsum[0] + wsum[1]) + (wsum[2] + wsum[3]));
+        norm[0] = tn;
+        if constexpr (PREP) adam_prep(P, true, tn);
     }
 }
 
@@ -163,7 +180,31 @@
 extern "C" int ncw_grad_norm(const float* grad, int64_t n, float* scratch, float* norm, void* stream) {
     if (!grad || !scratch || !norm || n < 0 || ((uintptr_t)grad & 15) != 0) return NCW_E_BADARG;
     if (hipMemsetAsync(scratch + NORM_BLOCKS, 0, sizeof(unsigned), (hipStream_t)stream) != hipSuccess) return NCW_E_BADARG;
-    hipLaunchKernelGGL(grad_norm_kernel, dim3(NORM_BLOCKS), dim3(256), 0, (hipStream_t)stream, grad, n, scratch, norm);
+    hipLaunchKernelGGL(grad_norm_kernel<false>, dim3(NORM_BLOCKS), dim3(256), 0, (hipStream_t)stream, grad, n, scratch, norm,
+                       AdamPrep{});
+    NCW_CHECK_LAUNCH();
+    return 0;
+}
+
+static bool adam_args_ok(const float* param, const float* grad, const float* exp_avg, const float* exp_avg_sq, const void* state) {
+    if (!param || !grad || !exp_avg || !exp_avg_sq || !state) return false;
+    return (((uintptr_t)param | (uintptr_t)grad | (uintptr_t)exp_avg | (uintptr_t)exp_avg_sq) & 15) == 0;
+}
+
+extern "C" int ncw_grad_norm_adam_step(float* param, float* grad, float* exp_avg, float* exp_avg_sq, int64_t n, float* scratch,
+                                       float* norm, NcwAdamState* state, float lr, const float* lr_dev, float beta1, float beta2,
+                                       float eps, float max_norm, float* loss_scale, int growth_interval, float scale_min,
+                                       float scale_max, void* stream) {
+    if (!scratch || !norm || n < 0) return NCW_E_BADARG;
+    if (n == 0) return ncw_grad_norm(grad, n, scratch, norm, stream);
+    if (!adam_args_ok(param, grad, exp_avg, exp_avg_sq, state)) return NCW_E_BADARG;
+    if (hipMemsetAsync(scratch + NORM_BLOCKS, 0, sizeof(unsigned), (hipStream_t)stream) != hipSuccess) return NCW_E_BADARG;
+    const AdamPrep P{state, lr_dev, loss_scale, lr, beta1, beta2, max_norm, scale_min, scale_max, growth_interval};
+    hipLaunchKernelGGL(grad_norm_kernel<true>, dim3(NORM_BLOCKS), dim3(256), 0, (hipStream_t)stream, grad, n, scratch, norm, P);
+    NCW_CHECK_LAUNCH();
+    const int64_t quads = (n + 3) / 4;
+    hipLaunchKernelGGL(adam_dev_kernel, dim3((unsigned)((quads + 255) / 256)), dim3(256), 0, (hipStream_t)stream, param, grad,
+                       exp_avg, exp_avg_sq, n, beta1, beta2, eps, state);
     NCW_CHECK_LAUNCH();
     return 0;
 }
@@ -175,8 +216,8 @@
     if (n <= 0) return 0;
     if (!param || !grad || !exp_avg || !exp_avg_sq || !state) return NCW_E_BADARG;
     if ((((uintptr_t)param | (uintptr_t)grad | (uintptr_t)exp_avg | (uintptr_t)exp_avg_sq) & 15) != 0) return NCW_E_BADARG;
-    hipLaunchKernelGGL(adam_prep_kernel, dim3(1), dim3(64), 0, (hipStream_t)stream, state, total_norm, lr, lr_dev, beta1, beta2,
-                       max_norm, loss_scale, growth_interval, scale_min, scale_max);
+    const AdamPrep P{state, lr_dev, loss_scale, lr, beta1, beta2, max_norm, scale_min, scale_max, growth_interval};
+    hipLaunchKernelGGL(adam_prep_kernel, dim3(1), dim3(64), 0, (hipStream_t)stream, P, total_norm);
     NCW_CHECK_LAUNCH();
     const int64_t quads = (n + 3) / 4;
     hipLaunchKernelGGL(adam_dev_kernel, dim3((unsigned)((quads + 255) / 256)), dim3(256), 0, (hipStream_t)stream, param, grad,
diff --git a/neuralrecon-w_amd/csrc/ncw_pack.hip b/neuralrecon-w_amd/csrc/ncw_pack.hip
--- a/neuralrecon-w_amd/csrc/ncw_pack.hip
+++ b/neuralrecon-w_amd/csrc/ncw_pack.hip
@@ -204,7 +204,7 @@
     return 0;
 }
 
-extern "C" int ncw_abi_version(void) { return 38; }
+extern "C" int ncw_abi_version(void) { return 39; }
 
 extern "C" int ncw_device_info(char* buf, int buflen) {
     int cnt = 0;
diff --git a/neuralrecon-w_amd/csrc/ncw_rays.hip b/neuralrecon-w_amd/csrc/ncw_rays.hip
--- a/neuralrecon-w_amd/csrc/ncw_rays.hip
+++ b/neuralrecon-w_amd/csrc/ncw_rays.hip
@@ -229,6 +229,52 @@
         for (int j = 0; j < n; ++j) {
             const float w = c[j];
             rank += (w < v || (w == v && j < i)) ? 1 : 0;
+        }
+        out[(size_t)r * n + rank] = v;
+        if (pout) pout[(size_t)r * n + rank] = (i < na) ? pa[(size_t)r * na + i] : pb[(size_t)r * nb + (i - na)];
+    }
+}
+
+template <int MAXN>
+__global__ __launch_bounds__(256) void merge_sorted_kernel(const float* __restrict__ a, int na, const float* __restrict__ b,
+                                                           int nb, const float* __restrict__ pa,
+                                                           const float* __restrict__ pb, int R, float* __restrict__ out,
+                                                           float* __restrict__ pout) {
+    __shared__ float sm[4][MAXN];
+    const int wv = threadIdx.x >> 6, lane = threadIdx.x & 63;
+    const int r = blockIdx.x * 4 + wv;
+    if (r >= R) return;
+    const int n = na + nb;
+    float* c = sm[wv];
+    for (int i = lane; i < n; i += 64) c[i] = (i < na) ? a[(size_t)r * na + i] : b[(size_t)r * nb + (i - na)];
+    __builtin_amdgcn_wave_barrier();
+    int unsorted = 0;
+    for (int i = lane; i + 1 < n; i += 64)
+        if (i + 1 != na && !(c[i] <= c[i + 1])) unsorted = 1;
+    const bool counting = __any(unsorted) != 0;
+    const float* cb = c + na;
+    for (int i = lane; i < n; i += 64) {
+        const float v = c[i];
+        int rank = 0;
+        if (counting) {
+            for (int j = 0; j < n; ++j) {
+                const float w = c[j];
+                rank += (w < v || (w == v && j < i)) ? 1 : 0;
+            }
+        } else if (i < na) {
+            int hi = nb;
+            while (rank < hi) {
+                const int mid = (rank + hi) >> 1;
+                if (cb[mid] < v) rank = mid + 1; else hi = mid;
+            }
+            rank += i;
+        } else {
+            int hi = na;
+            while (rank < hi) {
+                const int mid = (rank + hi) >> 1;
+                if (c[mid] <= v) rank = mid + 1; else hi = mid;
+            }
+            rank += i - na;
         }
         out[(size_t)r * n + rank] = v;
         if (pout) pout[(size_t)r * n + rank] = (i < na) ? pa[(size_t)r * na + i] : pb[(size_t)r * nb + (i - na)];
@@ -598,6 +644,17 @@
     return 0;
 }
 
+extern "C" int ncw_merge_sorted(const float* a, int na, const float* b, int nb, const float* pa, const float* pb, int R,
+                                float* out, float* pout, void* stream) {
+    if (R <= 0 || na + nb <= 0) return 0;
+    const int cap = ray_capacity(na + nb);
+    if (!cap || na < 0 || nb < 0) return NCW_E_BADARG;
+    hipLaunchKernelGGL(cap == RAY_CAP_SMALL ? merge_sorted_kernel<RAY_CAP_SMALL> : merge_sorted_kernel<RAY_CAP_LARGE>,
+                       dim3((R + 3) / 4), dim3(256), 0, (hipStream_t)stream, a, na, b, nb, pa, pb, R, out, pout);
+    NCW_CHECK_LAUNCH();
+    return 0;
+}
+
 extern "C" int ncw_boundary(const float* near, const float* far, const float* z, int n, int R, int nb, float* zb,
                             void* stream) {
     if (R <= 0 || nb <= 0) return 0;
diff --git a/neuralrecon-w_amd/lib.py b/neuralrecon-w_amd/lib.py
--- a/neuralrecon-w_amd/lib.py
+++ b/neuralrecon-w_amd/lib.py
@@ -9,7 +9,7 @@
 PREC_F16 = 2
 MAX_LAYERS = 12
 MAX_SEGS = 4
-ABI_VERSION = 38
+ABI_VERSION = 39
 
 
 class NcwSeg(C.Structure):
@@ -210,6 +210,9 @@
     "ncw_adam_step_dev": (C.c_int, [C.c_void_p, C.c_void_p, C.c_void_p, C.c_void_p, C.c_int64, C.c_void_p, C.c_void_p,
                                     C.c_float, C.c_void_p, C.c_float, C.c_float, C.c_float, C.c_float, C.c_void_p, C.c_int,
                                     C.c_float, C.c_float, C.c_void_p]),
+    "ncw_grad_norm_adam_step": (C.c_int, [C.c_void_p, C.c_void_p, C.c_void_p, C.c_void_p, C.c_int64, C.c_void_p, C.c_void_p,
+                                          C.c_void_p, C.c_float, C.c_void_p, C.c_float, C.c_float, C.c_float, C.c_float,
+                                          C.c_void_p, C.c_int, C.c_float, C.c_float, C.c_void_p]),
     "ncw_wgrad_tiled": (C.c_int, [C.c_void_p, C.c_void_p, C.c_int, C.c_int, C.c_int, C.c_int, C.c_int64, C.c_void_p]),
     "ncw_wgrad_tiled_f16": (C.c_int, [C.c_void_p, C.c_void_p, C.c_int, C.c_int, C.c_int, C.c_int, C.c_int64, C.c_void_p]),
     "ncw_sdf_infer_points": (C.c_int, [C.POINTER(NcwSdfNet), C.c_int, C.POINTER(NcwPoints), C.c_int64, C.c_void_p,
@@ -282,6 +285,7 @@
     "ncw_aux_ray_bias": (C.c_int, [_VP, C.c_int, C.c_int, C.c_int, _VP, _VP, C.c_int, C.c_int64, _VP, C.c_int, _VP]),
     "ncw_inv_s_fwd": (C.c_int, [_VP, _VP, _VP, _VP]),
     "ncw_inv_s_bwd": (C.c_int, [_VP, C.c_int64, _VP, _VP, _VP]),
+    "ncw_inv_s_bwd_scaled": (C.c_int, [_VP, C.c_int64, _VP, _VP, _VP, _VP]),
     "ncw_loss_fwd": (C.c_int, [_VP, _VP, C.c_int64, _VP, _VP, C.c_int64, _VP, C.c_int64, C.c_float, C.c_float, C.c_float,
                                C.c_float, _VP, _VP]),
     "ncw_loss_bwd": (C.c_int, [_VP, _VP, _VP, C.c_int64, C.c_int64, C.c_int64, C.c_float, C.c_float, C.c_float, C.c_float,
@@ -308,6 +312,7 @@
     "ncw_sample_coarse": (C.c_int, [_VP, _VP, _VP, _VP, C.c_int, C.c_int, C.c_int, _VP, _VP, _VP, _VP, _VP, _VP]),
     "ncw_upsample": (C.c_int, [_VP, _VP, _VP, _VP, C.c_int, C.c_int, C.c_float, C.c_int, _VP, _VP]),
     "ncw_sort_merge": (C.c_int, [_VP, C.c_int, _VP, C.c_int, _VP, _VP, C.c_int, _VP, _VP, _VP]),
+    "ncw_merge_sorted": (C.c_int, [_VP, C.c_int, _VP, C.c_int, _VP, _VP, C.c_int, _VP, _VP, _VP]),
     "ncw_boundary": (C.c_int, [_VP, _VP, _VP, C.c_int, C.c_int, C.c_int, _VP, _VP]),
     "ncw_bg_select": (C.c_int, [_VP, _VP, _VP, _VP, C.c_int, C.c_int, C.c_int, _VP, _VP, _VP, _VP]),
     "ncw_composite_fwd": (C.c_int, [C.POINTER(NcwCompositeIn), C.POINTER(NcwCompositeOut), _VP]),
diff --git a/neuralrecon-w_amd/rayops.py b/neuralrecon-w_amd/rayops.py
--- a/neuralrecon-w_amd/rayops.py
+++ b/neuralrecon-w_amd/rayops.py
@@ -40,17 +40,21 @@
     return out
 
 
-def sort_merge(a, b, pa=None, pb=None):
+def sort_merge(a, b, pa=None, pb=None, presorted=False):
     _chk_cuda(a, b)
     R, na = a.shape
     nb = b.shape[1]
     out = torch.empty(R, na + nb, device=a.device)
     pout = torch.empty(R, na + nb, device=a.device) if pa is not None else None
     lib = L.get_lib()
-    L.check(lib.ncw_sort_merge(L.ptr(_f(a)), na, L.ptr(_f(b)), nb, L.ptr(_f(pa) if pa is not None else None),
-                               L.ptr(_f(pb) if pb is not None else None), R, L.ptr(out), L.ptr(pout),
-                               L.stream_ptr(a.device)), "ncw_sort_merge")
+    fn, name = (lib.ncw_merge_sorted, "ncw_merge_sorted") if presorted else (lib.ncw_sort_merge, "ncw_sort_merge")
+    L.check(fn(L.ptr(_f(a)), na, L.ptr(_f(b)), nb, L.ptr(_f(pa) if pa is not None else None),
+               L.ptr(_f(pb) if pb is not None else None), R, L.ptr(out), L.ptr(pout), L.stream_ptr(a.device)), name)
     return out, pout
+
+
+def merge_sorted(a, b, pa=None, pb=None):
+    return sort_merge(a, b, pa, pb, presorted=True)
 
 
 def boundary(near, far, z, nb):
diff --git a/neuralrecon-w_amd/renderer.py b/neuralrecon-w_amd/renderer.py
--- a/neuralrecon-w_amd/renderer.py
+++ b/neuralrecon-w_amd/renderer.py
@@ -45,14 +45,14 @@
                 main = torch.cuda.current_stream(dev)
                 side.wait_stream(main)
                 with torch.cuda.stream(side):
-                    z_feed, _ = rayops.sort_merge(z, z_out)
+                    z_feed, _ = rayops.merge_sorted(z, z_out)
                     pts_bg = points_struct(rays_o=rays_o, rays_d=rays_d, z=z_feed, sample_dist=sample_dist, mode=2)
                     density, bg_rgb, nctx = nerf.fwd_stash(pts_bg, R * M, prec, a_det, select=select, train=train, refine=refine)
                 density.record_stream(main)
                 bg_rgb.record_stream(main)
                 z_feed.record_stream(main)
             else:
-                z_feed, _ = rayops.sort_merge(z, z_out)
+                z_feed, _ = rayops.merge_sorted(z, z_out)
                 pts_bg = points_struct(rays_o=rays_o, rays_d=rays_d, z=z_feed, sample_dist=sample_dist, mode=2)
                 density, bg_rgb, nctx = nerf.fwd_stash(pts_bg, R * M, prec, a_det, select=select, train=train, refine=refine)
             assert z_feed.shape[1] == M
@@ -109,13 +109,13 @@
         lib = L.get_lib()
         M = comp.S + comp.O
         side = rdr._bg_stream(dev) if (ctx.use_bg and rdr.use_bg_stream and not ordered) else None
-        d_a_bg = None
+        d_a = None
         if side is not None:
-            d_a_bg = torch.zeros(ctx.a_shape, device=dev, dtype=torch.float32)
+            d_a = torch.zeros(ctx.a_shape, device=dev, dtype=torch.float32)
             side.wait_stream(torch.cuda.current_stream(dev))
             with torch.cuda.stream(side):
-                nerf.bwd_stash(nctx, g["d_density"].view(R * M), g["d_bg_rgb"].view(R * M, 3), d_a_bg)
-            for t_ in (g["d_density"], g["d_bg_rgb"]):
+                nerf.bwd_stash(nctx, g["d_density"].view(R * M), g["d_bg_rgb"].view(R * M, 3), d_a)
+            for t_ in (g["d_density"], g["d_bg_rgb"], d_a):
                 t_.record_stream(side)
         try:
             if ordered:
@@ -124,7 +124,8 @@
                 neuconw.color_net.bwd_stash(cctx, g["d_rgb"].view(R * S, 3), d_grad, None, dfeat_ptr, d_a_rows=rows)
                 L.check(lib.ncw_ray_sum_rows(L.ptr(rows), R, S, n_a, L.ptr(d_a), 0, L.stream_ptr(dev)), "ncw_ray_sum_rows")
             else:
-                d_a = torch.zeros(ctx.a_shape, device=dev, dtype=torch.float32)
+                if d_a is None:
+                    d_a = torch.zeros(ctx.a_shape, device=dev, dtype=torch.float32)
                 neuconw.color_net.bwd_stash(cctx, g["d_rgb"].view(R * S, 3), d_grad, d_a, dfeat_ptr)
             neuconw.sdf_net.bwd_stash(sctx, g["d_sdf"].view(R * S), d_grad)
         finally:
@@ -132,7 +133,6 @@
                 torch.cuda.current_stream(dev).wait_stream(side)
         plans = [sctx["plan"], cctx["plan"]]
         if side is not None:
-            d_a.add_(d_a_bg)
             plans.append(nctx["plan"])
         elif ctx.use_bg:
             if ordered:
@@ -180,11 +180,11 @@
             keep = unpack_many(plans, tviews, grad_mul_dev=sc_inv)
         ctx._keep = (keep, batch)
         d_var = torch.empty(1, device=dev, dtype=torch.float32)
-        L.check(lib.ncw_inv_s_bwd(L.ptr(g["d_inv_s"]), R, L.ptr(ctx.inv_s), L.ptr(d_var), L.stream_ptr(dev)), "ncw_inv_s_bwd")
+        L.check(lib.ncw_inv_s_bwd_scaled(L.ptr(g["d_inv_s"]), R, L.ptr(ctx.inv_s), L.ptr(sc_inv), L.ptr(d_var), L.stream_ptr(dev)),
+                "ncw_inv_s_bwd_scaled")
         d_var = d_var.reshape(ctx.variance.shape)
         if sc_inv is not None:
             d_a.mul_(sc_inv)
-            d_var = d_var * sc_inv
         ctx.guard.release()
         return (None, None, None, None, None, None, None, None, None, d_a, d_var) + tuple(out)
 
@@ -369,9 +369,9 @@
 
     def cat_z_vals(self, rays_o, rays_d, z_vals, new_z_vals, sdf, last=False):
         if last:
-            return rayops.sort_merge(z_vals, new_z_vals)[0], sdf
+            return rayops.merge_sorted(z_vals, new_z_vals)[0], sdf
         new_sdf = self._sdf_rays(rays_o, rays_d, new_z_vals.contiguous())
-        return rayops.sort_merge(z_vals, new_z_vals, sdf, new_sdf)
+        return rayops.merge_sorted(z_vals, new_z_vals, sdf, new_sdf)
 
     @torch.no_grad()
     def sparse_sampler(self, rays_o, rays_d, near, far, perturb, _rand=None, far_override=None):
diff --git a/neuralrecon-w_amd/trainer.py b/neuralrecon-w_amd/trainer.py
--- a/neuralrecon-w_amd/trainer.py
+++ b/neuralrecon-w_amd/trainer.py
@@ -132,23 +132,27 @@
             raise L.NeuconwHipError("FlatAdam: parameters are not on a GPU; there is no CPU fallback")
         b1, b2 = self.betas
         need_norm = self.clip is not None or self.loss_scale is not None
-        norm = None
-        if need_norm:
-            lib = L.get_lib()
-            if self.__dict__.get("_norm_scratch") is None or self._norm_scratch.device != fp.flat_grad.device:
-                self._norm_scratch = torch.zeros(int(lib.ncw_grad_norm_scratch_floats()), device=fp.flat_grad.device, dtype=torch.float32)
-                self._norm = torch.empty(1, device=fp.flat_grad.device, dtype=torch.float32)
-            norm = self._norm
-            L.check(lib.ncw_grad_norm(L.ptr(fp.flat_grad), fp.flat_grad.numel(), L.ptr(self._norm_scratch), L.ptr(norm),
-                                      L.stream_ptr(fp.flat_grad.device)), "ncw_grad_norm")
-            norm = norm[0]
-        L.check(L.get_lib().ncw_adam_step_dev(
+        lib = L.get_lib()
+        clip = float(self.clip) if self.clip is not None else 0.0
+        if not need_norm:
+            L.check(lib.ncw_adam_step_dev(
+                L.ptr(fp.flat.data), L.ptr(fp.flat_grad), L.ptr(self.exp_avg), L.ptr(self.exp_avg_sq), fp.flat_grad.numel(),
+                L.ptr(self.state), None, self.lr, L.ptr(self.lr_dev), b1, b2, self.eps, clip, L.ptr(self.loss_scale),
+                self.growth_interval, self.scale_min, self.scale_max, L.stream_ptr(fp.flat_grad.device)), "ncw_adam_step_dev")
+            fp.mark_updated()
+            return None
+        if self.__dict__.get("_norm_scratch") is None or self._norm_scratch.device != fp.flat_grad.device:
+            self._norm_scratch = torch.zeros(int(lib.ncw_grad_norm_scratch_floats()), device=fp.flat_grad.device, dtype=torch.float32)
+            self._norms, self._norm_turn = torch.zeros(2, device=fp.flat_grad.device, dtype=torch.float32), 0
+        self._norm_turn ^= 1
+        norm = self._norms[self._norm_turn:self._norm_turn + 1]
+        L.check(lib.ncw_grad_norm_adam_step(
             L.ptr(fp.flat.data), L.ptr(fp.flat_grad), L.ptr(self.exp_avg), L.ptr(self.exp_avg_sq), fp.flat_grad.numel(),
-            L.ptr(self.state), L.ptr(norm), self.lr, L.ptr(self.lr_dev), b1, b2, self.eps,
-            float(self.clip) if self.clip is not None else 0.0, L.ptr(self.loss_scale), self.growth_interval,
-            self.scale_min, self.scale_max, L.stream_ptr(fp.flat_grad.device)), "ncw_adam_step_dev")
+            L.ptr(self._norm_scratch), L.ptr(norm), L.ptr(self.state), self.lr, L.ptr(self.lr_dev), b1, b2, self.eps, clip,
+            L.ptr(self.loss_scale), self.growth_interval, self.scale_min, self.scale_max, L.stream_ptr(fp.flat_grad.device)),
+            "ncw_grad_norm_adam_step")
         fp.mark_updated()
-        return norm.clone() if norm is not None else None
+        return norm[0]
 
     def state_dict(self):
         return {"step": self.step_count, "exp_avg": self.exp_avg, "exp_avg_sq": self.exp_avg_sq, "lr": self.lr,
```
